# rlangefe/pygemma

Hardware: AMD Instinct MI355X
Metric: SNPs/sec (whole node) at n=10,000 c=5; K-eigendecomp wallclock (higher is better)
Workload: dtype i8x3->i32 MFMA (genotype codes exact, integer accumulation exact; U as 24-bit fixed point per eigenvector in three int8 planes) rotation + f64 Gram/sweeps (f32 rounding points of the reference)

## Files before the change

### include/pygemma_hip.h

```cpp
#ifndef PYGEMMA_HIP_H
#define PYGEMMA_HIP_H
#include <stddef.h>
#include <stdint.h>
#ifdef __cplusplus
extern "C" {
#endif

#define PG_OK 0
#define PG_EINVAL (-22)
#define PG_ENOMEM (-12)
#define PG_EHIP (-5)
#define PG_ENOTSUP (-95)
#define PG_ENODEV (-19)

#define PG_MAX_COVARIATES 30

typedef struct pg_ctx pg_ctx;

const char *pg_last_error(void);
const char *pg_version(void);
int pg_device_count(void);
int pg_ctx_create(int device, pg_ctx **out);
int pg_ctx_create_on_stream(int device, void *hip_stream, pg_ctx **out);
void pg_ctx_destroy(pg_ctx *ctx);
int pg_ctx_sync(pg_ctx *ctx);
int pg_ctx_device(const pg_ctx *ctx);

int pg_malloc(pg_ctx *ctx, size_t bytes, void **dptr);
int pg_free(pg_ctx *ctx, void *dptr);
int pg_mem_info(pg_ctx *ctx, size_t *free_bytes, size_t *total_bytes);
int pg_memcpy_h2d(pg_ctx *ctx, void *dst, const void *src, size_t bytes);
int pg_memcpy_d2h(pg_ctx *ctx, void *dst, const void *src, size_t bytes);
int pg_memset(pg_ctx *ctx, void *dst, int value, size_t bytes);
int pg_memcpy2d_h2d(pg_ctx *ctx, void *dst, size_t dpitch, const void *src, size_t spitch, size_t width, size_t height);

int pg_host_alloc(pg_ctx *ctx, size_t bytes, void **hptr);
int pg_host_free(pg_ctx *ctx, void *hptr);
int pg_host_register(pg_ctx *ctx, void *hptr, size_t bytes);
int pg_host_unregister(pg_ctx *ctx, void *hptr);
int pg_memcpy_h2d_async(pg_ctx *ctx, void *dst, const void *src, size_t bytes);
int pg_memcpy_d2h_async(pg_ctx *ctx, void *dst, const void *src, size_t bytes);
int pg_memcpy_d2d_async(pg_ctx *ctx, void *dst, const void *src, size_t bytes);
int pg_memcpy2d_h2d_async(pg_ctx *ctx, void *dst, size_t dpitch, const void *src, size_t spitch, size_t width, size_t height);
int pg_stage_rows(void *dst, size_t dpitch, const void *src, size_t spitch, size_t width, size_t height, int nthreads);

int pg_event_create(pg_ctx *ctx, void **event);
int pg_event_destroy(pg_ctx *ctx, void *event);
int pg_event_record(pg_ctx *ctx, void *event);
int pg_event_elapsed_ms(pg_ctx *ctx, void *start, void *stop, float *ms);
int pg_event_sync(pg_ctx *ctx, void *event);
int pg_stream_wait_event(pg_ctx *ctx, void *event);

typedef struct pg_comm pg_comm;
#define PG_COMM_ID_BYTES 128
int pg_comm_unique_id(void *id128);
int pg_comm_init_rank(pg_ctx *ctx, int nranks, int rank, const void *id128, pg_comm **out);
int pg_comm_init_all(int ndev, pg_ctx *const *ctxs, pg_comm **out );
int pg_comm_destroy(pg_comm *comm);
int pg_comm_size(const pg_comm *comm);
int pg_comm_rank(const pg_comm *comm);
int pg_comm_broadcast_dev(pg_comm *comm, void *buf, size_t bytes, int root);
int pg_comm_allgather_dev(pg_comm *comm, const void *send, void *recv, size_t bytes_per_rank);
int pg_comm_allreduce_f64_dev(pg_comm *comm, double *buf, size_t count, int op_max);
int pg_comm_barrier(pg_comm *comm);
int pg_comm_group_start(void);
int pg_comm_group_end(void);

int pg_assoc_dev(pg_ctx *ctx, int64_t n, int c, int64_t p, const float *d, const float *Wr, const float *yr,
                 const float *Xr, int64_t ldx, int grid, float *beta, float *se, float *tau, float *lambda,
                 double *F, double *pval, unsigned long long *stats_dev);

int pg_assoc_set_eval_trace(pg_ctx *ctx, unsigned *trace_dev);
int pg_assoc_warm(pg_ctx *ctx, int64_t n, int c);

int pg_assoc_pheno_dev(pg_ctx *ctx, int64_t n, int c, int64_t p, int t, const float *d, const float *Wr,
                       const float *Yr, int64_t ldy, const float *Xr, int64_t ldx, int grid,
                       float *beta, float *se, float *tau, float *lambda, double *F, double *pval,
                       unsigned long long *stats_dev);
int pg_assoc_pheno_warm(pg_ctx *ctx, int64_t n, int c, int t, int64_t p);

int pg_assoc_lrt_dev(pg_ctx *ctx, int64_t n, int c, int64_t p, const float *d, const float *Wr, const float *yr,
                     const float *Xr, int64_t ldx, int grid, float *beta, float *se, float *tau, float *lambda,
                     double *F, double *pval, double *l_alt, double *l_null, double *D_lrt, double *p_lrt);

int pg_score_null_dev(pg_ctx *ctx, int64_t n, int c, const float *d, const float *Wr, const float *yr, float *lambda0_dev);
int pg_score_dev(pg_ctx *ctx, int64_t n, int c, int64_t p, const float *d, const float *Wr, const float *yr, float lambda0,
                 const float *Xr, int64_t ldx, float *beta, float *se, float *tau, float *lambda, double *F, double *pval);

int pg_assoc_gxe_dev(pg_ctx *ctx, int64_t n, int c, int64_t p, const float *d, const float *Wr, const float *yr,
                     const float *xr, int64_t ldx, const float *xer, int64_t ldxe, float *beta, float *se, float *tau,
                     float *lambda, double *F, double *pval, unsigned long long *stats_dev);
int pg_assoc_gxe_warm(pg_ctx *ctx, int64_t n, int c);
int pg_gxe_scale_u_dev(pg_ctx *ctx, int64_t n, const float *U, int64_t ldU, const float *e, float *Ue);

int pg_assoc(pg_ctx *ctx, int64_t n, int c, int64_t p, const float *d, const float *Wr, const float *yr,
             const float *X_n_by_p, int grid, float *beta, float *se, float *tau, float *lambda, double *F,
             double *pval, unsigned long long *stats2);

int pg_assoc_multi(int ngpu, int64_t n, int c, int64_t p, const float *d, const float *Wr, const float *yr,
                   const float *X_n_by_p, int grid, float *beta, float *se, float *tau, float *lambda, double *F, double *pval);

int pg_fdist_sf_dev(pg_ctx *ctx, int64_t count, const double *F, double dfd, double *pval);

int pg_transpose_dev(pg_ctx *ctx, int64_t n, int64_t p, const float *X_n_by_p, int64_t ldX, float *Xr, int64_t ldx);

int pg_rotate_dev(pg_ctx *ctx, int64_t n, int64_t p, const float *U, int64_t ldU, const float *X_n_by_p, int64_t ldX,
                  float *Xr, int64_t ldx);

size_t pg_geno_prep_bytes(int64_t n);
size_t pg_geno_work_bytes(int64_t n, int64_t p);
int pg_geno_prep_dev(pg_ctx *ctx, int64_t n, const float *U, int64_t ldU, void *Uprep);
int pg_rotate_geno_dev(pg_ctx *ctx, int64_t n, int64_t p, const void *Uprep, const float *X_n_by_p, int64_t ldX, float *Xr,
                       int64_t ldx, void *work, int *is_geno);
int pg_rotate_auto_dev(pg_ctx *ctx, int64_t n, int64_t p, const float *U, int64_t ldU, const void *Uprep, const float *X_n_by_p, int64_t ldX,
                       float *Xr, int64_t ldx, void *work, int *path_dev);
int pg_rotate_auto_i8_dev(pg_ctx *ctx, int64_t n, int64_t p, const void *Uprep, const void *X8_n_by_p, int is_unsigned, int64_t ldX,
                          float *Xr, int64_t ldx, void *work, int *path_dev);
int pg_rotate_geno_i8_dev(pg_ctx *ctx, int64_t n, int64_t p, const void *Uprep, const void *X8_n_by_p, int is_unsigned, int64_t ldX,
                          float *Xr, int64_t ldx, void *work, int *is_geno);
int pg_cast_i8_f32_dev(pg_ctx *ctx, int64_t n, int64_t p, const void *X8_n_by_p, int is_unsigned, int64_t ldX, float *Xf, int64_t ldXf);
int pg_rotate_geno_f64_dev(pg_ctx *ctx, int64_t n, int64_t p, const void *Uprep, const double *X_n_by_p, int64_t ldX, float *Xr,
                           int64_t ldx, void *work, int *is_geno);
int pg_cast_f64_f32_dev(pg_ctx *ctx, int64_t n, int64_t p, const double *X_n_by_p, int64_t ldX, float *Xf, int64_t ldXf);
int pg_rotate_bed_dev(pg_ctx *ctx, int64_t n, int64_t p, const void *Uprep, const unsigned char *bed, int64_t ldb, int count_a1,
                      float *Xr, int64_t ldx, void *work);

int pg_kinship_dev(pg_ctx *ctx, int64_t n, int64_t p_k, const float *Gt, int64_t ldg, float *K);
int pg_kinship_geno_dev(pg_ctx *ctx, int64_t n, int64_t p, const float *G, int64_t ldG, int standardize, float *K);

enum { PG_DTYPE_INT8 = 0, PG_DTYPE_UINT8 = 1, PG_DTYPE_FLOAT32 = 2, PG_DTYPE_FLOAT64 = 3 };
size_t pg_kinship_acc_bytes(int64_t n, int64_t pb);
int pg_kinship_bed_acc_dev(pg_ctx *ctx, int64_t n, int64_t pb, const unsigned char *bed, int64_t ldb, int count_a1, int standardize,
                           double *acc);
int pg_kinship_x_acc_dev(pg_ctx *ctx, int64_t n, int64_t pb, const void *X, int dtype, int64_t ldX, int snp_major, int standardize,
                         double *acc);
int pg_kinship_finish_dev(pg_ctx *ctx, int64_t n, int64_t p, const double *acc, float *K);

int pg_zkzt_dev(pg_ctx *ctx, int64_t n, int64_t q, const void *Z, int z_is_f64, int64_t ldz, const void *K, int k_is_f64, int64_t ldk,
                float *out, int64_t ldo);

int pg_syevd_dev(pg_ctx *ctx, int64_t n, const float *K, float *evals, float *U, double *evals64, double *U64);

int pg_precompute_mat_dev(pg_ctx *ctx, int64_t n, int ctot, float lam, const float *d, const float *Wx, const float *y,
                          int full, float *P3, float *Q3, float *R3, float *vecs, float *scal);
int pg_newton_dev(pg_ctx *ctx, int64_t n, int ctot, float lam, float lam_min, float lam_max, const float *d,
                  const float *Wx, const float *y, float *root);
int pg_reml_scalars_dev(pg_ctx *ctx, int64_t n, int ctot, const float *args8, float *out3);
int pg_ml_scalars_dev(pg_ctx *ctx, int64_t n, const float *args7, float *out3);

int pgx_dgemm_dev(pg_ctx *ctx, int transA, int64_t M, int64_t N, int64_t K, double alpha, const double *A, int64_t lda,
                  const double *B, int64_t ldb, double beta, double *C, int64_t ldc);
int pgx_dgemm_ex_dev(pg_ctx *ctx, int flags, int kxorB, int64_t M, int64_t N, int64_t K, double alpha, const double *A, int64_t lda,
                     const double *B, int64_t ldb, double beta, double *C, int64_t ldc);
int pgx_ring_stamps(long long *out64);
int pgx_sytrd_dev(pg_ctx *ctx, int64_t n, const float *K, double *d, double *e, double *tau, double *Vall);
int pgx_stedc_dev(pg_ctx *ctx, int64_t n, const double *d_host, const double *e_host, double *evals_host, double *Z_dev);
int pgx_sb2_stage1_dev(pg_ctx *ctx, int64_t n, const float *K, double *Aband, double *Z, int *flags);
int pgx_sb2_stage2_dev(pg_ctx *ctx, int64_t n, const double *Aband, double *d, double *e, double *Z, int *flags);
int pgx_sb2_set_debug(void *host_mapped);

#ifdef __cplusplus
}
#endif
#endif
```

### pygemma_amd/_lib.py

```python
import ctypes as C
import os

import numpy as np

_HERE = os.path.dirname(os.path.abspath(__file__))
LIB_PATH = os.environ.get("PYGEMMA_HIP_LIB") or os.path.join(_HERE, "lib", "libpygemma_hip.so")
_lib = None

SYMBOLS = [
    "pg_last_error", "pg_version", "pg_device_count", "pg_ctx_create", "pg_ctx_create_on_stream",
    "pg_ctx_destroy", "pg_ctx_sync", "pg_ctx_device", "pg_mem_info", "pg_malloc", "pg_free", "pg_memcpy_h2d", "pg_memcpy_d2h",
    "pg_memset", "pg_memcpy2d_h2d", "pg_event_create", "pg_event_destroy", "pg_event_record", "pg_event_elapsed_ms",
    "pg_kinship_dev", "pg_geno_prep_bytes", "pg_geno_work_bytes", "pg_geno_prep_dev", "pg_rotate_geno_dev", "pg_assoc_dev", "pg_assoc", "pg_fdist_sf_dev", "pg_transpose_dev", "pg_rotate_dev", "pg_syevd_dev",
    "pg_precompute_mat_dev", "pg_newton_dev", "pg_reml_scalars_dev", "pg_ml_scalars_dev", "pg_rotate_bed_dev", "pg_rotate_geno_i8_dev", "pg_cast_i8_f32_dev", "pg_assoc_multi", "pg_rotate_geno_f64_dev", "pg_cast_f64_f32_dev",
    "pg_host_alloc", "pg_host_free", "pg_host_register", "pg_host_unregister", "pg_memcpy_h2d_async", "pg_memcpy_d2h_async",
    "pg_memcpy_d2d_async", "pg_memcpy2d_h2d_async", "pg_stage_rows", "pg_event_sync", "pg_stream_wait_event",
    "pg_comm_unique_id", "pg_comm_init_rank", "pg_comm_init_all", "pg_comm_destroy", "pg_comm_size", "pg_comm_rank",
    "pg_comm_broadcast_dev", "pg_comm_allgather_dev", "pg_comm_allreduce_f64_dev", "pg_comm_barrier", "pg_comm_group_start",
    "pg_comm_group_end", "pgx_dgemm_dev", "pgx_sytrd_dev", "pgx_stedc_dev", "pgx_sb2_stage1_dev", "pgx_sb2_stage2_dev", "pgx_sb2_set_debug", "pg_kinship_geno_dev", "pg_assoc_lrt_dev", "pg_rotate_auto_dev", "pg_assoc_set_eval_trace", "pg_assoc_warm", "pg_rotate_auto_i8_dev",
    "pg_zkzt_dev", "pgx_dgemm_ex_dev", "pgx_ring_stamps", "pg_assoc_pheno_dev", "pg_assoc_pheno_warm", "pg_score_null_dev", "pg_score_dev",
    "pg_kinship_acc_bytes", "pg_kinship_bed_acc_dev", "pg_kinship_x_acc_dev", "pg_kinship_finish_dev",
    "pg_assoc_gxe_dev", "pg_assoc_gxe_warm", "pg_gxe_scale_u_dev",
]


class PgError(RuntimeError):
    pass


def load():
    global _lib
    if _lib is not None:
        return _lib
    if not os.path.exists(LIB_PATH):
        raise PgError(f"{LIB_PATH} not found: build the HIP extension (python -c 'import __graft_entry__ as g; g.build()'). "
                      "pygemma_amd has no CPU fallback.")
    L = C.CDLL(LIB_PATH)
    vp, i64, i32, sz = C.c_void_p, C.c_int64, C.c_int, C.c_size_t
    L.pg_last_error.restype = C.c_char_p
    L.pg_version.restype = C.c_char_p
    L.pg_device_count.restype = i32
    L.pg_ctx_create.argtypes = [i32, C.POINTER(vp)]
    L.pg_ctx_create_on_stream.argtypes = [i32, vp, C.POINTER(vp)]
    L.pg_ctx_destroy.argtypes = [vp]
    L.pg_ctx_destroy.restype = None
    L.pg_ctx_sync.argtypes = [vp]
    L.pg_ctx_device.argtypes = [vp]
    L.pg_mem_info.argtypes = [vp, C.POINTER(C.c_size_t), C.POINTER(C.c_size_t)]
    L.pg_malloc.argtypes = [vp, sz, C.POINTER(vp)]
    L.pg_free.argtypes = [vp, vp]
    L.pg_memcpy_h2d.argtypes = [vp, vp, vp, sz]
    L.pg_memcpy_d2h.argtypes = [vp, vp, vp, sz]
    L.pg_memset.argtypes = [vp, vp, i32, sz]
    L.pg_assoc_dev.argtypes = [vp, i64, i32, i64, vp, vp, vp, vp, i64, i32, vp, vp, vp, vp, vp, vp, vp]
    L.pg_assoc.argtypes = [vp, i64, i32, i64, vp, vp, vp, vp, i32, vp, vp, vp, vp, vp, vp, vp]
    L.pg_assoc_lrt_dev.argtypes = [vp, i64, i32, i64, vp, vp, vp, vp, i64, i32] + [vp] * 10
    L.pg_assoc_lrt_dev.restype = i32
    L.pg_fdist_sf_dev.argtypes = [vp, i64, vp, C.c_double, vp]
    L.pg_assoc_multi.argtypes = [i32, i64, i32, i64, vp, vp, vp, vp, i32, vp, vp, vp, vp, vp, vp]
    L.pg_assoc_multi.restype = i32
    L.pg_transpose_dev.argtypes = [vp, i64, i64, vp, i64, vp, i64]
    L.pg_rotate_dev.argtypes = [vp, i64, i64, vp, i64, vp, i64, vp, i64]
    L.pg_kinship_dev.argtypes = [vp, i64, i64, vp, i64, vp]
    L.pg_kinship_geno_dev.argtypes = [vp, i64, i64, vp, i64, i32, vp]
    L.pg_kinship_geno_dev.restype = i32
    L.pg_kinship_acc_bytes.argtypes = [i64, i64]
    L.pg_kinship_acc_bytes.restype = sz
    L.pg_kinship_bed_acc_dev.argtypes = [vp, i64, i64, vp, i64, i32, i32, vp]
    L.pg_kinship_bed_acc_dev.restype = i32
    L.pg_kinship_x_acc_dev.argtypes = [vp, i64, i64, vp, i32, i64, i32, i32, vp]
    L.pg_kinship_x_acc_dev.restype = i32
    L.pg_kinship_finish_dev.argtypes = [vp, i64, i64, vp, vp]
    L.pg_kinship_finish_dev.restype = i32
    L.pg_geno_prep_bytes.argtypes = [i64]
    L.pg_geno_prep_bytes.restype = sz
    L.pg_geno_work_bytes.argtypes = [i64, i64]
    L.pg_geno_work_bytes.restype = sz
    L.pg_geno_prep_dev.argtypes = [vp, i64, vp, i64, vp]
    L.pg_geno_prep_dev.restype = i32
    L.pg_rotate_geno_dev.argtypes = [vp, i64, i64, vp, vp, i64, vp, i64, vp, C.POINTER(i32)]
    L.pg_rotate_geno_dev.restype = i32
    L.pg_assoc_set_eval_trace.argtypes = [vp, vp]
    L.pg_assoc_set_eval_trace.restype = i32
    L.pg_assoc_warm.argtypes = [vp, i64, i32]
    L.pg_assoc_warm.restype = i32
    L.pg_assoc_pheno_dev.argtypes = [vp, i64, i32, i64, i32, vp, vp, vp, i64, vp, i64, i32, vp, vp, vp, vp, vp, vp, vp]
    L.pg_assoc_pheno_dev.restype = i32
    L.pg_assoc_pheno_warm.argtypes = [vp, i64, i32, i32, i64]
    L.pg_assoc_pheno_warm.restype = i32
    L.pg_score_null_dev.argtypes = [vp, i64, i32, vp, vp, vp, vp]
    L.pg_score_null_dev.restype = i32
    L.pg_score_dev.argtypes = [vp, i64, i32, i64, vp, vp, vp, C.c_float, vp, i64, vp, vp, vp, vp, vp, vp]
    L.pg_score_dev.restype = i32
    L.pg_assoc_gxe_dev.argtypes = [vp, i64, i32, i64, vp, vp, vp, vp, i64, vp, i64, vp, vp, vp, vp, vp, vp, vp]
    L.pg_assoc_gxe_dev.restype = i32
    L.pg_assoc_gxe_warm.argtypes = [vp, i64, i32]
    L.pg_assoc_gxe_warm.restype = i32
    L.pg_gxe_scale_u_dev.argtypes = [vp, i64, vp, i64, vp, vp]
    L.pg_gxe_scale_u_dev.restype = i32
    L.pg_rotate_auto_i8_dev.argtypes = [vp, i64, i64, vp, vp, i32, i64, vp, i64, vp, vp]
    L.pg_rotate_auto_i8_dev.restype = i32
    L.pg_rotate_auto_dev.argtypes = [vp, i64, i64, vp, i64, vp, vp, i64, vp, i64, vp, vp]
    L.pg_rotate_auto_dev.restype = i32
    L.pg_rotate_bed_dev.argtypes = [vp, i64, i64, vp, vp, i64, i32, vp, i64, vp]
    L.pg_rotate_bed_dev.restype = i32
    L.pg_rotate_geno_i8_dev.argtypes = [vp, i64, i64, vp, vp, i32, i64, vp, i64, vp, C.POINTER(i32)]
    L.pg_rotate_geno_i8_dev.restype = i32
    L.pg_cast_i8_f32_dev.argtypes = [vp, i64, i64, vp, i32, i64, vp, i64]
    L.pg_cast_i8_f32_dev.restype = i32
    L.pg_rotate_geno_f64_dev.argtypes = [vp, i64, i64, vp, vp, i64, vp, i64, vp, C.POINTER(i32)]
    L.pg_rotate_geno_f64_dev.restype = i32
    L.pg_cast_f64_f32_dev.argtypes = [vp, i64, i64, vp, i64, vp, i64]
    L.pg_cast_f64_f32_dev.restype = i32
    L.pg_memcpy2d_h2d.argtypes = [vp, vp, sz, vp, sz, sz, sz]
    L.pg_event_create.argtypes = [vp, C.POINTER(vp)]
    L.pg_event_destroy.argtypes = [vp, vp]
    L.pg_event_record.argtypes = [vp, vp]
    L.pg_event_elapsed_ms.argtypes = [vp, vp, vp, C.POINTER(C.c_float)]
    L.pg_syevd_dev.argtypes = [vp, i64, vp, vp, vp, vp, vp]
    f32 = C.c_float
    L.pg_precompute_mat_dev.argtypes = [vp, i64, i32, f32, vp, vp, vp, i32, vp, vp, vp, vp, vp]
    L.pg_newton_dev.argtypes = [vp, i64, i32, f32, f32, f32, vp, vp, vp, vp]
    L.pg_reml_scalars_dev.argtypes = [vp, i64, i32, vp, vp]
    L.pg_ml_scalars_dev.argtypes = [vp, i64, vp, vp]
    L.pg_ml_scalars_dev.restype = i32
    L.pg_host_alloc.argtypes = [vp, sz, C.POINTER(vp)]
    L.pg_host_free.argtypes = [vp, vp]
    L.pg_host_register.argtypes = [vp, vp, sz]
    L.pg_host_unregister.argtypes = [vp, vp]
    L.pg_memcpy_h2d_async.argtypes = [vp, vp, vp, sz]
    L.pg_memcpy_d2h_async.argtypes = [vp, vp, vp, sz]
    L.pg_memcpy_d2d_async.argtypes = [vp, vp, vp, sz]
    L.pg_memcpy2d_h2d_async.argtypes = [vp, vp, sz, vp, sz, sz, sz]
    L.pg_stage_rows.argtypes = [vp, sz, vp, sz, sz, sz, i32]
    L.pg_event_sync.argtypes = [vp, vp]
    L.pg_stream_wait_event.argtypes = [vp, vp]
    L.pg_comm_unique_id.argtypes = [vp]
    L.pg_comm_init_rank.argtypes = [vp, i32, i32, vp, C.POINTER(vp)]
    L.pg_comm_init_all.argtypes = [i32, C.POINTER(vp), C.POINTER(vp)]
    L.pg_comm_destroy.argtypes = [vp]
    L.pg_comm_size.argtypes = [vp]
    L.pg_comm_rank.argtypes = [vp]
    L.pg_comm_broadcast_dev.argtypes = [vp, vp, sz, i32]
    L.pg_comm_allgather_dev.argtypes = [vp, vp, vp, sz]
    L.pg_comm_allreduce_f64_dev.argtypes = [vp, vp, sz, i32]
    L.pg_comm_barrier.argtypes = [vp]
    L.pgx_dgemm_dev.argtypes = [vp, i32, i64, i64, i64, C.c_double, vp, i64, vp, i64, C.c_double, vp, i64]
    L.pgx_dgemm_ex_dev.argtypes = [vp, i32, i32, i64, i64, i64, C.c_double, vp, i64, vp, i64, C.c_double, vp, i64]
    L.pgx_dgemm_ex_dev.restype = i32
    L.pg_zkzt_dev.argtypes = [vp, i64, i64, vp, i32, i64, vp, i32, i64, vp, i64]
    L.pg_zkzt_dev.restype = i32
    L.pgx_sytrd_dev.argtypes = [vp, i64, vp, vp, vp, vp, vp]
    L.pgx_stedc_dev.argtypes = [vp, i64, vp, vp, vp, vp]
    L.pgx_sb2_stage1_dev.argtypes = [vp, i64, vp, vp, vp, vp]
    L.pgx_sb2_stage2_dev.argtypes = [vp, i64, vp, vp, vp, vp, vp]
    L.pgx_sb2_set_debug.argtypes = [vp]
    for name in ("pg_host_alloc", "pg_host_free", "pg_host_register", "pg_host_unregister", "pg_memcpy_h2d_async", "pg_memcpy_d2h_async",
                 "pg_memcpy_d2d_async", "pg_memcpy2d_h2d_async", "pg_stage_rows", "pg_event_sync", "pg_stream_wait_event", "pg_comm_unique_id",
                 "pg_comm_init_rank", "pg_comm_init_all", "pg_comm_destroy", "pg_comm_size", "pg_comm_rank", "pg_comm_broadcast_dev",
                 "pg_comm_allgather_dev", "pg_comm_allreduce_f64_dev", "pg_comm_barrier", "pg_comm_group_start", "pg_comm_group_end",
                 "pgx_dgemm_dev", "pgx_sytrd_dev", "pgx_stedc_dev", "pgx_sb2_stage1_dev", "pgx_sb2_stage2_dev", "pgx_sb2_set_debug"):
        getattr(L, name).restype = i32
    for name in ("pg_ctx_create", "pg_ctx_create_on_stream", "pg_ctx_sync", "pg_ctx_device", "pg_malloc", "pg_free",
                 "pg_memcpy_h2d", "pg_memcpy_d2h", "pg_memset", "pg_assoc_dev", "pg_assoc", "pg_fdist_sf_dev",
                 "pg_transpose_dev", "pg_rotate_dev", "pg_syevd_dev", "pg_memcpy2d_h2d", "pg_event_create", "pg_event_destroy",
                 "pg_event_record", "pg_event_elapsed_ms", "pg_kinship_dev", "pg_precompute_mat_dev", "pg_newton_dev",
                 "pg_reml_scalars_dev"):
        getattr(L, name).restype = i32
    _lib = L
    return L


def check(rc, what=""):
    if rc != 0:
        raise PgError(f"{what} failed (code {rc}): {load().pg_last_error().decode()}")


class DeviceBuffer:

    def __init__(self, ctx, nbytes):
        self.ctx, self.nbytes = ctx, int(nbytes)
        p = C.c_void_p()
        check(load().pg_malloc(ctx.handle, self.nbytes, C.byref(p)), "pg_malloc")
        self.ptr = p.value

    def free(self):
        if self.ptr:
            load().pg_free(self.ctx.handle, self.ptr)
            self.ptr = None

    def upload(self, arr):
        arr = np.ascontiguousarray(arr)
        assert arr.nbytes <= self.nbytes
        check(load().pg_memcpy_h2d(self.ctx.handle, self.ptr, arr.ctypes.data, arr.nbytes), "pg_memcpy_h2d")
        return self

    def download(self, shape, dtype, offset=0):
        out = np.empty(shape, dtype)
        check(load().pg_memcpy_d2h(self.ctx.handle, out.ctypes.data, self.ptr + offset, out.nbytes), "pg_memcpy_d2h")
        return out


class Context:

    def __init__(self, device=0, stream=None):
        L = load()
        h = C.c_void_p()
        if stream is None:
            check(L.pg_ctx_create(int(device), C.byref(h)), "pg_ctx_create")
        else:
            check(L.pg_ctx_create_on_stream(int(device), C.c_void_p(stream), C.byref(h)), "pg_ctx_create_on_stream")
        self.handle = h
        self.device = device
        self._bufs = []

    def alloc(self, nbytes):
        b = DeviceBuffer(self, nbytes)
        self._bufs.append(b)
        return b

    def to_device(self, arr):
        arr = np.ascontiguousarray(arr)
        return self.alloc(max(arr.nbytes, 4)).upload(arr)

    def sync(self):
        check(load().pg_ctx_sync(self.handle), "pg_ctx_sync")

    def mem_info(self):
        f, t = C.c_size_t(), C.c_size_t()
        check(load().pg_mem_info(self.handle, C.byref(f), C.byref(t)), "pg_mem_info")
        return int(f.value), int(t.value)

    def close(self):
        if self.handle:
            for b in self._bufs:
                b.free()
            self._bufs = []
            load().pg_ctx_destroy(self.handle)
            self.handle = None

    def __enter__(self):
        return self

    def __exit__(self, *a):
        self.close()

    def __del__(self):
        try:
            self.close()
        except Exception:
            pass


def device_count():
    return load().pg_device_count()


_pinned = {}


class _PinnedBlock:

    def __init__(self, nbytes, device=0):
        import weakref
        self.ctx = Context(device)
        p = C.c_void_p()
        check(load().pg_host_alloc(self.ctx.handle, max(int(nbytes), 1), C.byref(p)), "pg_host_alloc")
        self.ptr, self.nbytes = p.value, int(nbytes)
        _pinned[self.ptr] = self.nbytes
        self._fin = weakref.finalize(self, _PinnedBlock._release, self.ctx, self.ptr)

    @staticmethod
    def _release(ctx, ptr):
        _pinned.pop(ptr, None)
        try:
            load().pg_host_free(ctx.handle, ptr)
            ctx.close()
        except Exception:
            pass


def pinned_empty(shape, dtype=np.float32, device=0):
    dtype = np.dtype(dtype)
    nbytes = int(np.prod(shape, dtype=np.int64)) * dtype.itemsize
    blk = _PinnedBlock(nbytes, device)
    buf = (C.c_char * max(nbytes, 1)).from_address(blk.ptr)
    arr = np.frombuffer(buf, dtype=dtype, count=nbytes // dtype.itemsize).reshape(shape)
    arr.flags.writeable = True
    buf._pg_block = blk
    return arr


def pin(arr, device=0):
    assert arr.flags.c_contiguous or arr.flags.f_contiguous
    ctx = Context(device)
    check(load().pg_host_register(ctx.handle, arr.ctypes.data, arr.nbytes), "pg_host_register")
    _pinned[arr.ctypes.data] = arr.nbytes

    class _Pin:
        def close(self_inner):
            if _pinned.pop(arr.ctypes.data, None) is not None:
                load().pg_host_unregister(ctx.handle, arr.ctypes.data)
                ctx.close()
    return _Pin()


def is_pinned(arr):
    try:
        from numpy.lib.array_utils import byte_bounds
    except ImportError:
        byte_bounds = np.byte_bounds
    lo, hi = byte_bounds(arr)
    for base, nb in list(_pinned.items()):
        if base <= lo and hi <= base + nb:
            return True
    return False
```

### pygemma_amd/csrc/assoc.hip

```cpp
#include "common.hpp"

#include <cmath>

namespace pg {

constexpr int NLAM = 11;
#ifndef PG_ASSOC_WPB
#define PG_ASSOC_WPB 2
#endif
constexpr int WPB = PG_ASSOC_WPB;
#define PG_MINV 1e-35f
#ifndef PG_FUSE_PQ_MAX
#define PG_FUSE_PQ_MAX 36
#endif
#ifndef PG_FUSE_PQR_MAX
#define PG_FUSE_PQR_MAX 28
#endif
#ifndef PG_PFD
#define PG_PFD 2
#endif
#ifndef PG_CHUNK_MIN_NP
#define PG_CHUNK_MIN_NP 80
#endif
#ifndef PG_SCAN_NV
#define PG_SCAN_NV 96
#endif
#ifndef PG_SWEEP_LDS_MIN_SLOTS
#define PG_SWEEP_LDS_MIN_SLOTS 3
#endif
#ifndef PG_PHENO_SPLIT_XE
#define PG_PHENO_SPLIT_XE 26
#endif
#ifndef PG_WAVES
#define PG_WAVES 2
#endif

__host__ __device__ constexpr size_t assoc_per_wave_bytes(int M, bool sweep_lds, size_t evalout_bytes, int n_vals)
{
    return (((sweep_lds ? (size_t)3 * M * 8 : 0) + (size_t)NLAM * 2 * M * 8 + NLAM * evalout_bytes + 2 * NLAM * 4 + (size_t)n_vals * 4) + 15) & ~(size_t)15;
}

struct AssocParams {
    int n, npad, c, niter, nu, grid, rowf;
    long long p, ldx;
    const float *xr;
    const float *fixed;
    float *htab;
    double *fixg;
    double *t1tab;
    float *ldHtab;
    float lam11[NLAM];
    float logl_c;
    const int *leaf, *node, *level, *chunk;
    int n_leaf, n_level, n_chunk, n_vals;
    float *beta, *se, *tau, *lam;
    double *F;
    unsigned long long *stats;
    unsigned *trace;
    int lrt, nhalf;
    float ml_c;
    float *lalt, *lamalt;
    const double *xbuf;
    int xe, xcol;
};

struct EvalOut { float yPy, yPPy, yPPPy, trP, trPP, ld, Pxx_c, Pyx_c, sh, shh; };

__device__ __forceinline__ float hinv_f32(float lam, float d)
{
    const float x = __fadd_rn(__fmul_rn(lam, d), 1.0f);
    const float r0 = __builtin_amdgcn_rcpf(x);
    float r = __builtin_fmaf(__builtin_fmaf(-x, r0, 1.0f), r0, r0);
    if (__builtin_expect(!(x < 0x1p126f), 0)) r = __fdiv_rn(1.0f, x);
    return r;
}

__device__ __forceinline__ float np_logf(float x)
{
    const float p1 = 9.999999999999998702752e-01f, p2 = 2.112677543073053063722e+00f,
                p3 = 1.480000633576506585156e+00f, p4 = 3.808837741388407920751e-01f,
                p5 = 2.589979117907922693523e-02f;
    const float q1 = 2.612677543073109236779e+00f, q2 = 2.453006071784736363091e+00f,
                q3 = 9.864942958519418960339e-01f, q4 = 1.546476374983906719538e-01f,
                q5 = 5.875095403124574342950e-03f;
    if (__builtin_expect(!(x > 0.0f) || x == INFINITY, 0)) return (x != x) ? x : (x < 0.0f ? NAN : (x == 0.0f ? -INFINITY : x));
    unsigned u = __float_as_uint(x);
    int e = (int)((u >> 23) & 0xff) - 126;
    float m = __uint_as_float((u & 0x007fffffu) | 0x3f000000u);
    float ef = (float)e;
    if (m <= 0.70710678118f) { m = __fadd_rn(m, m); ef = __fsub_rn(ef, 1.0f); }
    float t = __fsub_rn(m, 1.0f);
    float den = fmaf(q5, t, q4);
    den = fmaf(den, t, q3); den = fmaf(den, t, q2); den = fmaf(den, t, q1); den = fmaf(den, t, 1.0f);
    float num = fmaf(p5, t, p4);
    num = fmaf(num, t, p3); num = fmaf(num, t, p2); num = fmaf(num, t, p1); num = fmaf(num, t, 0.0f);
    float poly = __fdiv_rn(num, den);
    return fmaf(ef, 0.693147180559945309417232121458176568f, poly);
}

__device__ __forceinline__ double bfly(double v)
{
#pragma unroll
    for (int s = 1; s < 64; s <<= 1) v += __shfl_xor(v, s, 64);
    return v;
}

__device__ float device_logdet_H(const AssocParams &pr, float lam, int lane, float *vals)
{
    const int sub = lane & 7, grp = lane >> 3;
    auto elem = [&](int i) -> float {
        float d = pr.fixed[(size_t)i * pr.rowf];
        return np_logf(__fadd_rn(__fmul_rn(lam, d), 1.0f));
    };
    for (int l0 = 0; l0 < pr.n_leaf; l0 += 8) {
        const int lf = l0 + grp;
        int start = 0, len = 0;
        if (lf < pr.n_leaf) { start = pr.leaf[2 * lf]; len = pr.leaf[2 * lf + 1]; }
        float res = 0.0f;
        if (len >= 8) {
            const int body = len - (len & 7);
            float r = elem(start + sub);
            for (int i = 8; i < body; i += 8) r = __fadd_rn(r, elem(start + i + sub));
            r = __fadd_rn(r, __shfl_xor(r, 1, 64));
            r = __fadd_rn(r, __shfl_xor(r, 2, 64));
            r = __fadd_rn(r, __shfl_xor(r, 4, 64));
            res = r;
            for (int i = body; i < len; i++) res = __fadd_rn(res, elem(start + i));
        } else {
            for (int i = 0; i < len; i++) res = __fadd_rn(res, elem(start + i));
        }
        if (lf < pr.n_leaf && sub == 0) vals[lf] = res;
    }
    __builtin_amdgcn_fence(__ATOMIC_RELEASE, "wavefront");
    __builtin_amdgcn_wave_barrier();
    __builtin_amdgcn_fence(__ATOMIC_ACQUIRE, "wavefront");
    for (int h = 0; h < pr.n_level; h++) {
        const int b = pr.level[h], e = pr.level[h + 1];
        for (int k = b + lane; k < e; k += 64) {
            float a = vals[pr.node[2 * k]], c = vals[pr.node[2 * k + 1]];
            vals[pr.n_leaf + k] = __fadd_rn(a, c);
        }
        __builtin_amdgcn_fence(__ATOMIC_RELEASE, "wavefront");
        __builtin_amdgcn_wave_barrier();
        __builtin_amdgcn_fence(__ATOMIC_ACQUIRE, "wavefront");
    }
    float tot = vals[pr.chunk[0]];
    for (int k = 1; k < pr.n_chunk; k++) tot = __fadd_rn(tot, vals[pr.chunk[k]]);
    return tot;
}

__device__ __forceinline__ float logl_f(const AssocParams &pr, float yPy, float ldH, float ld)
{
    float r = pr.logl_c;
    r = (float)((double)r + (0.5 * (double)0.0f));
    r = (float)((double)r - (0.5 * (double)ldH));
    r = (float)((double)r - (0.5 * (double)ld));
    r = (float)((double)r - ((0.5 * (double)pr.nu) * log((double)yPy)));
    return r;
}
__device__ __forceinline__ float d1_f(const AssocParams &pr, float lam, float yPy, float yPPy, float trP)
{
    float yT = (PG_MINV > yPy) ? PG_MINV : yPy;
    float nc_tr = __fsub_rn((float)pr.nu, trP);
    float r = (float)(-0.5 * (double)__fdiv_rn(nc_tr, lam));
    float t = (0.0f > yPPy) ? 0.0f : yPPy;
    float g = __fdiv_rn(__fsub_rn(yT, t), lam);
    r = (float)((double)r + ((0.5 * (double)pr.nu) * (double)g) / (double)yT);
    return r;
}
__device__ __forceinline__ float d2_f(const AssocParams &pr, float lam, float yPy, float yPPy, float yPPPy,
                                      float trP, float trPP)
{
    float a = (PG_MINV > yPy) ? PG_MINV : yPy;
    float b = (PG_MINV > yPPy) ? PG_MINV : yPPy;
    float e = (PG_MINV > yPPPy) ? PG_MINV : yPPPy;
    double lam2 = (double)lam * (double)lam;
    float ae = __fadd_rn(a, e);
    float G2 = (float)(((double)ae - 2.0 * (double)b) / lam2);
    float G1 = __fdiv_rn(__fsub_rn(a, b), lam);
    float nct = __fadd_rn((float)pr.nu, trPP);
    float r = (float)((0.5 * ((double)nct - 2.0 * (double)trP)) / lam2);
    float G2a = __fmul_rn(G2, a);
    r = (float)((double)r - ((double)pr.nu * ((double)G2a - (0.5 * (double)G1) * (double)G1)) / ((double)a * (double)a));
    return r;
}

__device__ __forceinline__ float ml_logl_f(const AssocParams &pr, float yPy, float ldH)
{
    float r = pr.ml_c;
    r = __fsub_rn(r, __fmul_rn(0.5f, ldH));
    const float t = (PG_MINV > yPy) ? PG_MINV : yPy;
    r = (float)((double)r - (double)pr.nhalf * log((double)t));
    return r;
}
__device__ __forceinline__ float ml_d1_f(const AssocParams &pr, float lam, float yPy, float yPPy, float sh)
{
    float r = __fmul_rn(-0.5f, __fdiv_rn(__fsub_rn((float)pr.n, sh), lam));
    const float num = (PG_MINV > yPPy) ? PG_MINV : yPPy, den = (PG_MINV > yPy) ? PG_MINV : yPy;
    r = (float)((double)r + ((double)pr.nhalf * (1.0 - (double)__fdiv_rn(num, den))) / (double)lam);
    return r;
}
__device__ __forceinline__ float ml_d2_f(const AssocParams &pr, float lam, float yPy, float yPPy, float yPPPy, float sh, float shh)
{
    const float a = (PG_MINV > yPy) ? PG_MINV : yPy, b = (PG_MINV > yPPy) ? PG_MINV : yPPy, e = (PG_MINV > yPPPy) ? PG_MINV : yPPPy;
    const float G2 = (float)(((double)__fadd_rn(a, e) - 2.0 * (double)b) / (double)__fmul_rn(lam, lam));
    const float G1 = __fdiv_rn(__fsub_rn(a, b), lam);
    const float t = __fmul_rn(0.5f, __fsub_rn(__fadd_rn((float)pr.n, shh), __fmul_rn(2.0f, sh)));
    float r = (float)((double)t / ((double)lam * (double)lam));
    r = (float)((double)r - ((0.5 * (double)pr.n) * ((2.0 * (double)G2) - (double)__fdiv_rn(__fmul_rn(G1, G1), a))) / (double)a);
    return r;
}

template <int C> struct Shape {
    static constexpr int M = C + 2;
    static constexpr int NP = M * (M + 1) / 2;
    static constexpr int SLOTS = (NP + 63) / 64;
    static constexpr int NV0 = NP < 64 ? NP : 64, NV1 = NP > 64 ? NP - 64 : 0;
    static constexpr int slot_nv(int sl) { return (NP - 64 * sl) < 64 ? (NP - 64 * sl) : 64; }
    static constexpr bool CHUNKED = NP > PG_CHUNK_MIN_NP;
    static constexpr bool SWEEP_LDS = SLOTS >= PG_SWEEP_LDS_MIN_SLOTS;
    static constexpr int SCAN_NV = (M <= 4 && PG_SCAN_NV > 64) ? 64 : PG_SCAN_NV;
    static constexpr int G = (SCAN_NV / (2 * M)) < 1 ? 1 : ((SCAN_NV / (2 * M)) > 11 ? 11 : (SCAN_NV / (2 * M)));
    static constexpr bool FUSE_PQ = NP <= PG_FUSE_PQ_MAX, FUSE_PQR = NP <= PG_FUSE_PQR_MAX;
};
__host__ __device__ constexpr int tri(int r, int c) { return r * (r + 1) / 2 + c; }
__host__ __device__ constexpr int next_pow2(int v) { int p = 1; while (p < v) p <<= 1; return p; }

__device__ __forceinline__ double dmaxf(double a, float b) { return ((double)b > a) ? (double)b : a; }

template <int NVP>
__device__ __forceinline__ double reduce_scatter(double (&v)[NVP], int lane)
{
    static_assert(NVP >= 1 && NVP <= 64 && (NVP & (NVP - 1)) == 0, "power of two");
#pragma unroll
    for (int s = 1; s < NVP; s <<= 1) {
        const bool b = (lane & s) != 0;
#pragma unroll
        for (int m = 0; m < NVP / (2 * s); m++) {
            const double keep = b ? v[2 * m + 1] : v[2 * m];
            const double send = b ? v[2 * m] : v[2 * m + 1];
            v[m] = keep + __shfl_xor(send, s, 64);
        }
    }
    double x = v[0];
#pragma unroll
    for (int s = NVP; s < 64; s <<= 1) x += __shfl_xor(x, s, 64);
    return x;
}

template <int C, int SL = 0>
__device__ __forceinline__ void scatter_entries(const double (&acc)[Shape<C>::NP], int lane, double (&out)[Shape<C>::SLOTS])
{
    constexpr int NV = Shape<C>::slot_nv(SL), NVP = next_pow2(NV);
    double t[NVP];
#pragma unroll
    for (int k = 0; k < NVP; k++) t[k] = (k < NV) ? acc[64 * SL + k] : 0.0;
    out[SL] = reduce_scatter<NVP>(t, lane);
    if constexpr (SL + 1 < Shape<C>::SLOTS) scatter_entries<C, SL + 1>(acc, lane, out);
}

template <int C> struct Own {
    int e[Shape<C>::SLOTS], r[Shape<C>::SLOTS], c[Shape<C>::SLOTS];
    bool valid[Shape<C>::SLOTS];
    __device__ __forceinline__ void init(int lane)
    {
#pragma unroll
        for (int sl = 0; sl < Shape<C>::SLOTS; sl++) {
            const int nv = Shape<C>::slot_nv(sl), k = lane % next_pow2(nv);
            valid[sl] = k < nv;
            e[sl] = valid[sl] ? 64 * sl + k : 0;
            int rr = 0;
            while ((rr + 1) * (rr + 2) / 2 <= e[sl]) rr++;
            r[sl] = rr; c[sl] = e[sl] - rr * (rr + 1) / 2;
        }
    }
};

template <int SLOTS>
__device__ __forceinline__ double gather(const double (&X)[SLOTS], int es)
{
    double v = __shfl(X[0], es & 63, 64);
#pragma unroll
    for (int sl = 1; sl < SLOTS; sl++) { const double w = __shfl(X[sl], es & 63, 64); v = ((es >> 6) == sl) ? w : v; }
    return v;
}

__device__ __forceinline__ void wave_lds_sync();

template <int C, bool FULL>
__device__ __forceinline__ void lane_sweeps(double (&P)[Shape<C>::SLOTS], double (&Q)[Shape<C>::SLOTS], double (&R)[Shape<C>::SLOTS],
                                            const Own<C> &own, double t1, double t2, int lane, EvalOut &o, double *piv)
{
    constexpr int M = Shape<C>::M, NP = Shape<C>::NP, SLOTS = Shape<C>::SLOTS;
    constexpr bool VIA_LDS = Shape<C>::SWEEP_LDS;
    if (own.valid[0] && own.e[0] == 0) P[0] = dmaxf(P[0], PG_MINV);
    double trP = t1, trPP = t2, apiv = 1.0;
    for (int i = 1; i < M; i++) {
        const int q = i - 1, eqq = tri(q, q);
        double a, b, e = 0.0;
        double ur[SLOTS], uc[SLOTS], vr[SLOTS], vc[SLOTS], wr[SLOTS], wc[SLOTS];
        bool act[SLOTS];
        if constexpr (VIA_LDS) {
#pragma unroll
            for (int sl = 0; sl < SLOTS; sl++)
                if (own.valid[sl] && own.c[sl] == q) {
                    piv[own.r[sl]] = P[sl]; piv[M + own.r[sl]] = Q[sl];
                    if (FULL) piv[2 * M + own.r[sl]] = R[sl];
                }
            wave_lds_sync();
            a = piv[q]; b = piv[M + q];
            if (FULL) e = piv[2 * M + q];
#pragma unroll
            for (int sl = 0; sl < SLOTS; sl++) {
                act[sl] = own.valid[sl] && own.c[sl] >= i;
                const int rr = act[sl] ? own.r[sl] : q, cc = act[sl] ? own.c[sl] : q;
                ur[sl] = piv[rr]; uc[sl] = piv[cc];
                vr[sl] = piv[M + rr]; vc[sl] = piv[M + cc];
                if (FULL) { wr[sl] = piv[2 * M + rr]; wc[sl] = piv[2 * M + cc]; }
            }
            wave_lds_sync();
        } else {
            a = gather<SLOTS>(P, eqq); b = gather<SLOTS>(Q, eqq);
            e = FULL ? gather<SLOTS>(R, eqq) : 0.0;
#pragma unroll
            for (int sl = 0; sl < SLOTS; sl++) {
                act[sl] = own.valid[sl] && own.c[sl] >= i;
                const int er = act[sl] ? tri(own.r[sl], q) : 0, ec = act[sl] ? tri(own.c[sl], q) : 0;
                ur[sl] = gather<SLOTS>(P, er); uc[sl] = gather<SLOTS>(P, ec);
                vr[sl] = gather<SLOTS>(Q, er); vc[sl] = gather<SLOTS>(Q, ec);
                if (FULL) { wr[sl] = gather<SLOTS>(R, er); wc[sl] = gather<SLOTS>(R, ec); }
            }
        }
        if (lane == q) apiv = a;
        const double a2 = a * a, ia = -1.0 / a, ba2 = b / a2;
        if (FULL) {
            const double ba = b / a;
            trPP = (trPP + ba * ba) - 2 * (e / a);
            const double a3 = a2 * a, b2 = b * b;
            const double cR = (e / a2) - (b2 / a3);
#pragma unroll
            for (int sl = 0; sl < SLOTS; sl++)
                if (act[sl]) {
                    double s1 = fma(cR * uc[sl], ur[sl], R[sl]);
                    double s2 = fma(ia * uc[sl], wr[sl], 0.0); s2 = fma(ia * wc[sl], ur[sl], s2);
                    double s3 = fma(ia * vc[sl], vr[sl], 0.0);
                    double s4 = fma(ba2 * uc[sl], vr[sl], 0.0); s4 = fma(ba2 * vc[sl], ur[sl], s4);
                    double rn = ((s1 + s2) + s3) + s4;
                    if (own.r[sl] == i && own.c[sl] == i) rn = dmaxf(rn, PG_MINV);
                    R[sl] = rn;
                }
        }
        trP = trP - b / a;
#pragma unroll
        for (int sl = 0; sl < SLOTS; sl++)
            if (act[sl]) {
                double s1 = fma(ba2 * uc[sl], ur[sl], Q[sl]);
                double s2 = fma(ia * uc[sl], vr[sl], 0.0); s2 = fma(ia * vc[sl], ur[sl], s2);
                double qn = s1 + s2;
                double pn = fma(ia * uc[sl], ur[sl], P[sl]);
                if (own.r[sl] == i && own.c[sl] == i) { qn = dmaxf(qn, PG_MINV); pn = dmaxf(pn, PG_MINV); }
                Q[sl] = qn; P[sl] = pn;
            }
        if (i == M - 2) { o.Pxx_c = (float)gather<SLOTS>(P, tri(M - 2, M - 2)); o.Pyx_c = (float)gather<SLOTS>(P, tri(M - 1, M - 2)); }
    }
    const double lg = log(apiv);
    float ld = 0.0f;
    for (int q = 0; q < M - 1; q++) ld = (float)((double)ld + __shfl(lg, q, 64));
    o.yPy = (float)gather<SLOTS>(P, NP - 1);
    o.yPPy = (float)gather<SLOTS>(Q, NP - 1);
    o.yPPPy = FULL ? (float)gather<SLOTS>(R, NP - 1) : 0.0f;
    o.trP = (float)trP;
    o.trPP = FULL ? (float)trPP : 0.0f;
    o.ld = ld;
    o.sh = (float)t1;
    o.shh = FULL ? (float)t2 : 0.0f;
}

template <int C> struct Elem {
    static constexpr int S4 = (C + 2 + 3) / 4;
    float4 row[S4];
    float x;
};
template <int C, bool HASX = true>
__device__ __forceinline__ void load_elem(const AssocParams &pr, const float *xrow, int i, Elem<C> &e)
{
    const float4 *src = reinterpret_cast<const float4 *>(pr.fixed + (size_t)i * pr.rowf);
#pragma unroll
    for (int k = 0; k < Elem<C>::S4; k++) e.row[k] = src[k];
    const int ic = min(i, pr.n - 1);
    e.x = HASX ? xrow[ic] : 0.0f;
}
constexpr int PFD = PG_PFD;
template <class E, int PF = PFD, class LoadF, class BodyF>
__device__ __forceinline__ void pipelined(int niter, LoadF &&ld, BodyF &&body)
{
    E buf[PF];
#pragma unroll
    for (int d = 0; d < PF; d++) ld(buf[d], d < niter ? d : niter - 1);
    for (int it = 0; it < niter; it += PF) {
#pragma unroll
        for (int d = 0; d < PF; d++) {
            if (it + d < niter) body(buf[d], it + d);
            const int nx = it + d + PF;
            ld(buf[d], nx < niter ? nx : niter - 1);
        }
    }
}
template <int C>
__device__ __forceinline__ void unpack_elem(const AssocParams &pr, const Elem<C> &e, int i, float &d, float (&col)[C + 2])
{
    float buf[4 * Elem<C>::S4];
#pragma unroll
    for (int k = 0; k < Elem<C>::S4; k++) {
        buf[4 * k] = e.row[k].x; buf[4 * k + 1] = e.row[k].y; buf[4 * k + 2] = e.row[k].z; buf[4 * k + 3] = e.row[k].w;
    }
    d = buf[0];
#pragma unroll
    for (int j = 0; j < C; j++) col[j] = buf[1 + j];
    col[C] = e.x;
    col[C + 1] = buf[C + 1];
}
template <int C> struct WaldElem {
    using E = Elem<C>;
    using Row = const float *;
    template <bool HASX>
    static __device__ __forceinline__ void load(const AssocParams &pr, Row xrow, int i, E &e) { load_elem<C, HASX>(pr, xrow, i, e); }
    static __device__ __forceinline__ void unpack(const AssocParams &pr, const E &e, int i, float &d, float (&col)[C + 2]) { unpack_elem<C>(pr, e, i, d, col); }
};

template <int C, int MASK, bool HASX, class EL = WaldElem<C>>
__device__ __forceinline__ void gram_pass(const AssocParams &pr, typename EL::Row xrow, float lam, int lane, float *htab_out,
                                          double (&Po)[Shape<C>::SLOTS], double (&Qo)[Shape<C>::SLOTS], double (&Ro)[Shape<C>::SLOTS],
                                          double &t1, double &t2)
{
    constexpr int M = Shape<C>::M, NP = Shape<C>::NP;
    constexpr bool DP = (MASK & 1) != 0, DQ = (MASK & 2) != 0, DR = (MASK & 4) != 0;
    double P[DP ? NP : 1], Q[DQ ? NP : 1], R[DR ? NP : 1];
#pragma unroll
    for (int k = 0; k < NP; k++) { if constexpr (DP) P[k] = 0.0; if constexpr (DQ) Q[k] = 0.0; if constexpr (DR) R[k] = 0.0; }
    double s1 = 0.0, s2 = 0.0;
    using E = typename EL::E;
    pipelined<E>(pr.niter, [&](E &e, int it) { EL::template load<HASX>(pr, xrow, it * 64 + lane, e); },
                       [&](const E &cur, int it) {
        const int i = it * 64 + lane;
        float d, colf[M];
        EL::unpack(pr, cur, i, d, colf);
        const float h = hinv_f32(lam, d);
        if (htab_out) htab_out[i] = h;
        const double hd = (double)h;
        double col[M], a[M];
#pragma unroll
        for (int j = 0; j < M; j++) { col[j] = (double)colf[j]; a[j] = hd * col[j]; }
        if (DP || DQ) {
#pragma unroll
            for (int j = 0; j < M; j++)
#pragma unroll
                for (int k = 0; k <= j; k++) {
                    if constexpr (DP) P[tri(j, k)] = fma(a[j], col[k], P[tri(j, k)]);
                    if constexpr (DQ) Q[tri(j, k)] = fma(a[j], a[k], Q[tri(j, k)]);
                }
        }
        if (DP) s1 += hd;
        if constexpr (DR) {
            const double h2 = hd * hd;
#pragma unroll
            for (int j = 0; j < M; j++) {
                const double gj = h2 * col[j];
#pragma unroll
                for (int k = 0; k <= j; k++) R[tri(j, k)] = fma(gj, a[k], R[tri(j, k)]);
            }
            s2 = fma(hd, hd, s2);
        }
    });
    if constexpr (DP) { scatter_entries<C>(P, lane, Po); t1 = bfly(s1); }
    if constexpr (DQ) scatter_entries<C>(Q, lane, Qo);
    if constexpr (DR) { scatter_entries<C>(R, lane, Ro); t2 = bfly(s2); }
}

template <int C, int PW, int SL, bool HASX, class EL = WaldElem<C>>
__device__ __forceinline__ void gram_pass_slot(const AssocParams &pr, typename EL::Row xrow, float lam, int lane, float *htab_out, double &out, double &tsum)
{
    constexpr int M = Shape<C>::M, E0 = 64 * SL, NV = Shape<C>::slot_nv(SL), NVP = next_pow2(NV);
    double acc[NVP];
#pragma unroll
    for (int k = 0; k < NVP; k++) acc[k] = 0.0;
    double s = 0.0;
    using E = typename EL::E;
    pipelined<E, (M > 22 ? 1 : PFD)>(pr.niter, [&](E &e, int it) { EL::template load<HASX>(pr, xrow, it * 64 + lane, e); },
                       [&](const E &cur, int it) {
        const int i = it * 64 + lane;
        float d, colf[M];
        EL::unpack(pr, cur, i, d, colf);
        const float h = hinv_f32(lam, d);
        if (htab_out) htab_out[i] = h;
        const double hd = (double)h, h2 = hd * hd;
        double col[M], a[M], g[PW == 3 ? M : 1];
#pragma unroll
        for (int j = 0; j < M; j++) { col[j] = (double)colf[j]; a[j] = hd * col[j]; if constexpr (PW == 3) g[j] = h2 * col[j]; }
#pragma unroll
        for (int j = 0; j < M; j++)
#pragma unroll
            for (int k = 0; k <= j; k++) {
                const int e = tri(j, k);
                if (e >= E0 && e < E0 + NV) {
                    if constexpr (PW == 1) acc[e - E0] = fma(a[j], col[k], acc[e - E0]);
                    else if constexpr (PW == 2) acc[e - E0] = fma(a[j], a[k], acc[e - E0]);
                    else acc[e - E0] = fma(g[j], a[k], acc[e - E0]);
                }
            }
        if constexpr (SL == 0 && PW == 1) s += hd;
        if constexpr (SL == 0 && PW == 3) s = fma(hd, hd, s);
    });
    out = reduce_scatter<NVP>(acc, lane);
    if constexpr (SL == 0 && (PW == 1 || PW == 3)) tsum = bfly(s);
}
template <int C, int PW, bool HASX, int SL = 0, class EL = WaldElem<C>>
__device__ __forceinline__ void slot_passes(const AssocParams &pr, typename EL::Row xrow, float lam, int lane, float *htab_out,
                                            double (&X)[Shape<C>::SLOTS], double &tsum)
{
    gram_pass_slot<C, PW, SL, HASX, EL>(pr, xrow, lam, lane, SL == 0 ? htab_out : nullptr, X[SL], tsum);
    if constexpr (SL + 1 < Shape<C>::SLOTS) slot_passes<C, PW, HASX, SL + 1, EL>(pr, xrow, lam, lane, htab_out, X, tsum);
}

template <int C, bool FULL, class EL = WaldElem<C>>
__device__ __forceinline__ void eval_specific(const AssocParams &pr, typename EL::Row xrow, float lam, int lane, const Own<C> &own, EvalOut &o,
                                              double *piv)
{
    constexpr int SLOTS = Shape<C>::SLOTS;
    double P[SLOTS], Q[SLOTS], R[SLOTS], t1 = 0.0, t2 = 0.0;
#pragma unroll
    for (int sl = 0; sl < SLOTS; sl++) R[sl] = 0.0;
    if constexpr (Shape<C>::CHUNKED) {
        double tq = 0.0;
        slot_passes<C, 1, true, 0, EL>(pr, xrow, lam, lane, nullptr, P, t1);
        slot_passes<C, 2, true, 0, EL>(pr, xrow, lam, lane, nullptr, Q, tq);
        if (FULL) slot_passes<C, 3, true, 0, EL>(pr, xrow, lam, lane, nullptr, R, t2);
    } else if constexpr (FULL && Shape<C>::FUSE_PQR) {
        gram_pass<C, 7, true, EL>(pr, xrow, lam, lane, nullptr, P, Q, R, t1, t2);
    } else if constexpr (Shape<C>::FUSE_PQ) {
        gram_pass<C, 3, true, EL>(pr, xrow, lam, lane, nullptr, P, Q, R, t1, t2);
        if (FULL) gram_pass<C, 4, true, EL>(pr, xrow, lam, lane, nullptr, P, Q, R, t1, t2);
    } else {
        gram_pass<C, 1, true, EL>(pr, xrow, lam, lane, nullptr, P, Q, R, t1, t2);
        gram_pass<C, 2, true, EL>(pr, xrow, lam, lane, nullptr, P, Q, R, t1, t2);
        if (FULL) gram_pass<C, 4, true, EL>(pr, xrow, lam, lane, nullptr, P, Q, R, t1, t2);
    }
    lane_sweeps<C, FULL>(P, Q, R, own, t1, t2, lane, o, piv);
}

template <int C>
__global__ __launch_bounds__(64) void setup_tabs_kernel(AssocParams pr)
{
    constexpr int NP = Shape<C>::NP, SLOTS = Shape<C>::SLOTS;
    extern __shared__ float smem_f[];
    const int t = blockIdx.x, lane = threadIdx.x;
    const float lam = pr.lam11[t];
    Own<C> own;
    own.init(lane);
    double P[SLOTS], Q[SLOTS], R[SLOTS], t1 = 0.0, t2 = 0.0;
    if constexpr (Shape<C>::CHUNKED) {
        double tq = 0.0;
        slot_passes<C, 1, false>(pr, nullptr, lam, lane, pr.htab + (size_t)t * pr.npad, P, t1);
        slot_passes<C, 2, false>(pr, nullptr, lam, lane, nullptr, Q, tq);
    } else if constexpr (Shape<C>::FUSE_PQ) {
        gram_pass<C, 3, false>(pr, nullptr, lam, lane, pr.htab + (size_t)t * pr.npad, P, Q, R, t1, t2);
    } else {
        gram_pass<C, 1, false>(pr, nullptr, lam, lane, pr.htab + (size_t)t * pr.npad, P, Q, R, t1, t2);
        gram_pass<C, 2, false>(pr, nullptr, lam, lane, nullptr, P, Q, R, t1, t2);
    }
#pragma unroll
    for (int sl = 0; sl < SLOTS; sl++)
        if (own.valid[sl]) {
            pr.fixg[((size_t)t * 2 + 0) * NP + own.e[sl]] = P[sl];
            pr.fixg[((size_t)t * 2 + 1) * NP + own.e[sl]] = Q[sl];
        }
    float ldH = device_logdet_H(pr, lam, lane, smem_f);
    if (lane == 0) { pr.t1tab[t] = t1; pr.ldHtab[t] = ldH; }
}

template <int C, int GG>
__device__ __forceinline__ void scan_accumulate(const AssocParams &pr, const float *xrow, int t0, int lane, double *xent)
{
    constexpr int M = Shape<C>::M, NV = GG * 2 * M;
    constexpr int NV0 = NV < 64 ? NV : 64, NV1 = NV > 64 ? NV - 64 : 0;
    constexpr int NVP0 = next_pow2(NV0), NVP1 = next_pow2(NV1 > 0 ? NV1 : 1);
    static_assert(NV <= 128, "scan group too large");
    double acc[NV0 == 64 ? 64 + NVP1 : NVP0];
#pragma unroll
    for (int k = 0; k < (NV0 == 64 ? 64 + NVP1 : NVP0); k++) acc[k] = 0.0;
    struct SE { Elem<C> e; float h[GG]; };
    pipelined<SE>(pr.niter, [&](SE &q, int it) {
        const int i = it * 64 + lane;
        load_elem<C>(pr, xrow, i, q.e);
#pragma unroll
        for (int g = 0; g < GG; g++) q.h[g] = pr.htab[(size_t)(t0 + g) * pr.npad + i];
    }, [&](const SE &q, int it) {
        const int i = it * 64 + lane;
        float d, colf[M];
        unpack_elem<C>(pr, q.e, i, d, colf);
        const double xd = (double)colf[C];
        double z[M];
#pragma unroll
        for (int k = 0; k <= C; k++) z[k] = xd * (double)colf[k];
        z[C + 1] = (double)colf[C + 1] * xd;
#pragma unroll
        for (int g = 0; g < GG; g++) {
            const double hd = (double)q.h[g];
            const double h2 = hd * hd;
#pragma unroll
            for (int k = 0; k <= C + 1; k++) {
                acc[g * 2 * M + k] = fma(hd, z[k], acc[g * 2 * M + k]);
                acc[g * 2 * M + M + k] = fma(h2, z[k], acc[g * 2 * M + M + k]);
            }
        }
    });
    {
        double t[NVP0];
#pragma unroll
        for (int k = 0; k < NVP0; k++) t[k] = acc[k];
        const double tot = reduce_scatter<NVP0>(t, lane);
        const int idx = lane % NVP0;
        if (idx < NV0 && lane < NVP0) xent[t0 * 2 * M + idx] = tot;
    }
    if constexpr (NV1 > 0) {
        double t[NVP1];
#pragma unroll
        for (int k = 0; k < NVP1; k++) t[k] = acc[64 + k];
        const double tot = reduce_scatter<NVP1>(t, lane);
        const int idx = lane % NVP1;
        if (idx < NV1 && lane < NVP1) xent[t0 * 2 * M + 64 + idx] = tot;
    }
}
template <int C, int T0>
__device__ __forceinline__ void scan_all(const AssocParams &pr, const float *xrow, int lane, double *xent)
{
    constexpr int G = Shape<C>::G;
    if constexpr (T0 < NLAM) {
        constexpr int GG = (NLAM - T0) < G ? (NLAM - T0) : G;
        scan_accumulate<C, GG>(pr, xrow, T0, lane, xent);
        scan_all<C, T0 + GG>(pr, xrow, lane, xent);
    }
}

template <int C, int TC, int GG, int PWS, int PW0>
__device__ __forceinline__ void scan_pheno_accumulate(const AssocParams &pr, const float *xrow, const float *Y, long long ldy, int tcn,
                                                      int t0, int lane, double *out)
{
    constexpr int M = Shape<C>::M, XE = C + 1 + TC, NV = GG * PWS * XE;
    auto dest = [&](int v) { const int gg = v / (PWS * XE), r = v - gg * PWS * XE; return (t0 + gg) * 2 * XE + PW0 * XE + r; };
    constexpr int NV0 = NV < 64 ? NV : 64, NV1 = NV > 64 ? NV - 64 : 0;
    constexpr int NVP0 = next_pow2(NV0), NVP1 = next_pow2(NV1 > 0 ? NV1 : 1);
    static_assert(NV <= 128, "scan group too large");
    double acc[NV0 == 64 ? 64 + NVP1 : NVP0];
#pragma unroll
    for (int k = 0; k < (NV0 == 64 ? 64 + NVP1 : NVP0); k++) acc[k] = 0.0;
    struct SE { Elem<C> e; float y[TC]; float h[GG]; };
    pipelined<SE>(pr.niter, [&](SE &q, int it) {
        const int i = it * 64 + lane;
        load_elem<C>(pr, xrow, i, q.e);
#pragma unroll
        for (int j = 0; j < TC; j++) q.y[j] = (i < pr.n && j < tcn) ? Y[(size_t)j * ldy + i] : 0.0f;
#pragma unroll
        for (int g = 0; g < GG; g++) q.h[g] = pr.htab[(size_t)(t0 + g) * pr.npad + i];
    }, [&](const SE &q, int it) {
        const int i = it * 64 + lane;
        float d, colf[M];
        unpack_elem<C>(pr, q.e, i, d, colf);
        const double xd = (double)colf[C];
        double z[XE];
#pragma unroll
        for (int k = 0; k <= C; k++) z[k] = xd * (double)colf[k];
#pragma unroll
        for (int j = 0; j < TC; j++) z[C + 1 + j] = (double)q.y[j] * xd;
#pragma unroll
        for (int g = 0; g < GG; g++) {
            const double hd = (double)q.h[g];
            const double h2 = hd * hd;
#pragma unroll
            for (int k = 0; k < XE; k++) {
                if constexpr (PWS == 2) {
                    acc[g * 2 * XE + k] = fma(hd, z[k], acc[g * 2 * XE + k]);
                    acc[g * 2 * XE + XE + k] = fma(h2, z[k], acc[g * 2 * XE + XE + k]);
                } else {
                    acc[g * XE + k] = fma(PW0 == 0 ? hd : h2, z[k], acc[g * XE + k]);
                }
            }
        }
    });
    {
        double t[NVP0];
#pragma unroll
        for (int k = 0; k < NVP0; k++) t[k] = acc[k];
        const double tot = reduce_scatter<NVP0>(t, lane);
        const int idx = lane % NVP0;
        if (idx < NV0 && lane < NVP0) out[dest(idx)] = tot;
    }
    if constexpr (NV1 > 0) {
        double t[NVP1];
#pragma unroll
        for (int k = 0; k < NVP1; k++) t[k] = acc[64 + k];
        const double tot = reduce_scatter<NVP1>(t, lane);
        const int idx = lane % NVP1;
        if (idx < NV1 && lane < NVP1) out[dest(64 + idx)] = tot;
    }
}
template <int C, int TC, int T0>
__device__ __forceinline__ void scan_pheno_all(const AssocParams &pr, const float *xrow, const float *Y, long long ldy, int tcn, int lane,
                                               double *out)
{
    constexpr int XE = C + 1 + TC, PWS = XE > PG_PHENO_SPLIT_XE ? 1 : 2;
    constexpr int G0 = PWS == 1 ? 1 : (Shape<C>::SCAN_NV - XE) / (PWS * XE), G = G0 < 1 ? 1 : (G0 > NLAM ? NLAM : G0);
    if constexpr (T0 < NLAM) {
        constexpr int GG = (NLAM - T0) < G ? (NLAM - T0) : G;
        if constexpr (PWS == 2) {
            scan_pheno_accumulate<C, TC, GG, 2, 0>(pr, xrow, Y, ldy, tcn, T0, lane, out);
        } else {
            scan_pheno_accumulate<C, TC, GG, 1, 0>(pr, xrow, Y, ldy, tcn, T0, lane, out);
            scan_pheno_accumulate<C, TC, GG, 1, 1>(pr, xrow, Y, ldy, tcn, T0, lane, out);
        }
        scan_pheno_all<C, TC, T0 + GG>(pr, xrow, Y, ldy, tcn, lane, out);
    }
}
constexpr int SCAN_WPB = 4;
template <int C, int TC>
__global__ __launch_bounds__(64 * SCAN_WPB, PG_WAVES) void scan_pheno_kernel(AssocParams pr, const float *Y, long long ldy, int tcn, double *xbuf)
{
    const int wave = threadIdx.x >> 6, lane = threadIdx.x & 63;
    const long long g = (long long)blockIdx.x * SCAN_WPB + wave;
    if (g >= pr.p) return;
    scan_pheno_all<C, TC, 0>(pr, pr.xr + (size_t)g * pr.ldx, Y, ldy, tcn, lane, xbuf + (size_t)g * NLAM * 2 * (C + 1 + TC));
}

__device__ __forceinline__ void wave_lds_sync()
{
    __builtin_amdgcn_fence(__ATOMIC_RELEASE, "wavefront");
    __builtin_amdgcn_wave_barrier();
    __builtin_amdgcn_fence(__ATOMIC_ACQUIRE, "wavefront");
}

template <class Fn>
__device__ __forceinline__ double brentq_dev(Fn &&f, double xa, double xb, double fa, double fb, int maxiter = 100)
{
    const double xtol = 2e-12, rtol = 0.1;
    double xpre = xa, xcur = xb, xblk = 0., fpre = fa, fcur = fb, fblk = 0., spre = 0., scur = 0., sbis, delta, stry, dpre, dblk;
    if (fpre == 0) return xpre;
    if (fcur == 0) return xcur;
    for (int i = 0; i < maxiter; i++) {
        if (fpre != 0 && fcur != 0 && (__builtin_signbit(fpre) != __builtin_signbit(fcur))) {
            xblk = xpre; fblk = fpre; spre = scur = xcur - xpre;
        }
        if (fabs(fblk) < fabs(fcur)) {
            xpre = xcur; xcur = xblk; xblk = xpre;
            fpre = fcur; fcur = fblk; fblk = fpre;
        }
        delta = (xtol + rtol * fabs(xcur)) / 2;
        sbis = (xblk - xcur) / 2;
        if (fcur == 0 || fabs(sbis) < delta) return xcur;
        if (fabs(spre) > delta && fabs(fcur) < fabs(fpre)) {
            if (xpre == xblk) {
                stry = -fcur * (xcur - xpre) / (fcur - fpre);
            } else {
                dpre = (fpre - fcur) / (xpre - xcur);
                dblk = (fblk - fcur) / (xblk - xcur);
                stry = -fcur * (fblk * dblk - fpre * dpre) / (dblk * dpre * (fblk - fpre));
            }
            double lim = 3 * fabs(sbis) - delta;
            double mn = fabs(spre) < lim ? fabs(spre) : lim;
            if (2 * fabs(stry) < mn) { spre = scur; scur = stry; }
            else { spre = sbis; scur = sbis; }
        } else { spre = sbis; scur = sbis; }
        xpre = xcur; fpre = fcur;
        if (fabs(scur) > delta) xcur += scur;
        else xcur += (sbis > 0 ? delta : -delta);
        fcur = f(xcur);
    }
    return xcur;
}

template <class Eval>
__device__ __forceinline__ float newton_dev(const AssocParams &pr, float lroot, float l0, float l1, Eval &&eval)
{
    int iteration = 0;
    for (;;) {
        EvalOut e;
        eval(lroot, e);
        const float d1 = d1_f(pr, lroot, e.yPy, e.yPPy, e.trP);
        const float d2 = d2_f(pr, lroot, e.yPy, e.yPPy, e.yPPPy, e.trP, e.trPP);
        const float ratio = __fdiv_rn(d1, d2);
        const bool any_nan = (ratio != ratio) || (d1 != d1) || (d2 != d2);
        const float sr = (float)((ratio > 0) - (ratio < 0)), s1 = (float)((d1 > 0) - (d1 < 0)), s2 = (float)((d2 > 0) - (d2 < 0));
        if (!any_nan && sr * s1 * s2 <= 0.0f) break;
        const float lnew = __fsub_rn(lroot, ratio);
        const float r_eps = (float)(fabs((double)__fsub_rn(lnew, lroot)) / fabs((double)lroot));
        if (lnew < l0) break;
        if (lnew > l1) break;
        if (isnan(lnew) || isinf(lnew)) break;
        lroot = lnew;
        if ((double)r_eps < 1e-5 || iteration > 100) break;
        iteration++;
    }
    return lroot;
}

template <int C, bool LRT, bool PHENO = false>
__global__ __launch_bounds__(64 * WPB, PG_WAVES) void assoc_kernel(AssocParams pr)
{
    constexpr int M = Shape<C>::M, NP = Shape<C>::NP, SLOTS = Shape<C>::SLOTS;
    extern __shared__ unsigned char smem[];
    const int wave = threadIdx.x >> 6, lane = threadIdx.x & 63;
    static_assert(!(PHENO && LRT), "the multi-phenotype search has no LRT");
    const long long g = (long long)blockIdx.x * WPB + wave;
    if (g >= pr.p) return;
    constexpr size_t piv_bytes = Shape<C>::SWEEP_LDS ? (size_t)3 * M * 8 : 0;
    unsigned char *base = smem + (size_t)wave * assoc_per_wave_bytes(M, Shape<C>::SWEEP_LDS, sizeof(EvalOut), pr.n_vals);
    double *piv = reinterpret_cast<double *>(base);
    base += piv_bytes;
    double *xent = reinterpret_cast<double *>(base);
    EvalOut *evs = reinterpret_cast<EvalOut *>(base + (size_t)NLAM * 2 * M * 8);
    float *d1s = reinterpret_cast<float *>(evs + NLAM);
    float *lls = d1s + NLAM;
    float *vals = lls + NLAM;
    const float *xrow = pr.xr + (size_t)g * pr.ldx;

    Own<C> own;
    own.init(lane);
    if constexpr (PHENO) {
        const double *src = pr.xbuf + (size_t)g * NLAM * 2 * pr.xe;
        for (int j = lane; j < NLAM * 2 * M; j += 64) {
            const int tp = j / M, k = j - tp * M;
            xent[j] = src[(size_t)tp * pr.xe + (k <= C ? k : pr.xcol)];
        }
    } else {
        scan_all<C, 0>(pr, xrow, lane, xent);
    }
    wave_lds_sync();
    for (int t = 0; t < NLAM; t++) {
        double P[SLOTS], Q[SLOTS], R[SLOTS];
        const double *fp = pr.fixg + ((size_t)t * 2 + 0) * NP, *fq = pr.fixg + ((size_t)t * 2 + 1) * NP;
        const double *xe = xent + t * 2 * M;
#pragma unroll
        for (int sl = 0; sl < SLOTS; sl++) {
            const int r = own.r[sl], c = own.c[sl];
            const bool isx = (r == C) || (r == C + 1 && c == C);
            const int k = (r == C) ? c : C + 1;
            P[sl] = isx ? xe[k] : fp[own.e[sl]];
            Q[sl] = isx ? xe[M + k] : fq[own.e[sl]];
            R[sl] = 0.0;
        }
        EvalOut e;
        lane_sweeps<C, false>(P, Q, R, own, pr.t1tab[t], 0.0, lane, e, piv);
        if (lane == 0) {
            evs[t] = e;
            d1s[t] = d1_f(pr, pr.lam11[t], e.yPy, e.yPPy, e.trP);
            lls[t] = logl_f(pr, e.yPy, pr.ldHtab[t], e.ld);
        }
    }
    wave_lds_sync();
    float best_l = lls[0], best_lambda;
    EvalOut best_e;
    if (best_l < lls[NLAM - 1]) { best_l = lls[NLAM - 1]; best_lambda = pr.lam11[NLAM - 1]; best_e = evs[NLAM - 1]; }
    else { best_lambda = pr.lam11[0]; best_e = evs[0]; }
    unsigned n_fast = 0, n_full = 0;
    if (pr.grid) {
        for (int t = 0; t < NLAM - 1; t++)
            if (lls[t] > best_l) { best_l = lls[t]; best_lambda = pr.lam11[t]; best_e = evs[t]; }
    } else {
        for (int k = 0; k < NLAM - 1; k++) {
            const float f0 = d1s[k], f1 = d1s[k + 1];
            if (__builtin_signbit(f0) == __builtin_signbit(f1)) continue;
            const float l0 = pr.lam11[k], l1 = pr.lam11[k + 1];
            double root = brentq_dev(
                [&](double x) -> double {
                    EvalOut e;
                    const float lf = (float)x;
                    eval_specific<C, false>(pr, xrow, lf, lane, own, e, piv);
                    n_fast++;
                    return (double)d1_f(pr, lf, e.yPy, e.yPPy, e.trP);
                },
                (double)l0, (double)l1, (double)f0, (double)f1);
            const float lroot = newton_dev(pr, (float)root, l0, l1, [&](float lf, EvalOut &e) {
                eval_specific<C, true>(pr, xrow, lf, lane, own, e, piv);
                n_full++;
            });
            EvalOut e;
            eval_specific<C, false>(pr, xrow, lroot, lane, own, e, piv);
            n_fast++;
            const float ldH = device_logdet_H(pr, lroot, lane, vals);
            const float ll = logl_f(pr, e.yPy, ldH, e.ld);
            if (ll > best_l) { best_l = ll; best_lambda = lroot; best_e = e; }
        }
    }
    if constexpr (LRT) {
        float ml_l = ml_logl_f(pr, evs[0].yPy, pr.ldHtab[0]), ml_lam = pr.lam11[0];
        {
            const float l1 = ml_logl_f(pr, evs[NLAM - 1].yPy, pr.ldHtab[NLAM - 1]);
            if (ml_l == ml_l && (l1 != l1 || l1 > ml_l)) { ml_l = l1; ml_lam = pr.lam11[NLAM - 1]; }
        }
        for (int k = 0; k < NLAM - 1; k++) {
            const float f0 = ml_d1_f(pr, pr.lam11[k], evs[k].yPy, evs[k].yPPy, evs[k].sh);
            const float f1 = ml_d1_f(pr, pr.lam11[k + 1], evs[k + 1].yPy, evs[k + 1].yPPy, evs[k + 1].sh);
            if (f0 != f0 || f1 != f1) continue;
            const float s0 = (float)((f0 > 0) - (f0 < 0)), s1 = (float)((f1 > 0) - (f1 < 0));
            if (!(s0 * s1 < 0.0f)) continue;
            double p0 = brentq_dev(
                [&](double x) -> double {
                    EvalOut e;
                    const float lf = (float)x;
                    eval_specific<C, false>(pr, xrow, lf, lane, own, e, piv);
                    n_fast++;
                    return (double)ml_d1_f(pr, lf, e.yPy, e.yPPy, e.sh);
                },
                (double)pr.lam11[k], (double)pr.lam11[k + 1], (double)f0, (double)f1, 5000);
            double pn = p0;
            for (int itr = 0; itr < 10; itr++) {
                EvalOut e;
                const float lf = (float)p0;
                eval_specific<C, true>(pr, xrow, lf, lane, own, e, piv);
                n_full++;
                const float fval = ml_d1_f(pr, lf, e.yPy, e.yPPy, e.sh);
                if (fval == 0.0f) { pn = p0; break; }
                const float fder = ml_d2_f(pr, lf, e.yPy, e.yPPy, e.yPPPy, e.sh, e.shh);
                if (fder == 0.0f) { pn = p0; break; }
                pn = p0 - (double)__fdiv_rn(fval, fder);
                if (fabs(pn - p0) <= 1.48e-8 + 1e-5 * fabs(p0)) break;
                p0 = pn;
            }
            if (ml_l == ml_l) {
                EvalOut e;
                const float lf = (float)pn;
                eval_specific<C, false>(pr, xrow, lf, lane, own, e, piv);
                n_fast++;
                const float l = ml_logl_f(pr, e.yPy, device_logdet_H(pr, lf, lane, vals));
                if (l != l || l > ml_l) { ml_l = l; ml_lam = lf; }
            }
        }
        if (lane == 0) { pr.lalt[g] = ml_l; pr.lamalt[g] = ml_lam; }
    }
    if (lane == 0) {
        const float b = __fdiv_rn(best_e.Pyx_c, best_e.Pxx_c);
        const float pxx = (PG_MINV > best_e.Pxx_c) ? PG_MINV : best_e.Pxx_c;
        const float sb = (float)(__dsqrt_rn((double)best_e.yPy) / ((double)sqrtf(pxx) * __dsqrt_rn((double)(pr.nu))));
        const float ta = __fdiv_rn((float)pr.nu, best_e.yPy);
        const double t = (double)__fdiv_rn(b, sb);
        pr.beta[g] = b; pr.se[g] = sb; pr.tau[g] = ta; pr.lam[g] = best_lambda; pr.F[g] = t * t;
        if (pr.stats) { atomicAdd(&pr.stats[0], (unsigned long long)n_fast); atomicAdd(&pr.stats[1], (unsigned long long)n_full); }
        if (pr.trace) pr.trace[g] = n_fast | (n_full << 16);
    }
}

#if defined(PG_ASSOC_PART) && (PG_ASSOC_PART == 6 || PG_ASSOC_PART == 7)
struct GxeRows { const float *x, *xe; };
template <int CS> struct GxeVals {
    static constexpr int S4 = (CS + 2 + 3) / 4;
    float4 row[S4];
    float x, xe;
};
template <int C> struct GxeElem {
    static constexpr int CS = C - 1;
    using E = GxeVals<CS>;
    using Row = GxeRows;
    template <bool HASX>
    static __device__ __forceinline__ void load(const AssocParams &pr, Row r, int i, E &e)
    {
        const float4 *src = reinterpret_cast<const float4 *>(pr.fixed + (size_t)i * pr.rowf);
#pragma unroll
        for (int k = 0; k < E::S4; k++) e.row[k] = src[k];
        const int ic = min(i, pr.n - 1);
        e.x = r.x[ic];
        e.xe = r.xe[ic];
    }
    static __device__ __forceinline__ void unpack(const AssocParams &pr, const E &e, int i, float &d, float (&col)[C + 2])
    {
        float buf[4 * E::S4];
#pragma unroll
        for (int k = 0; k < E::S4; k++) {
            buf[4 * k] = e.row[k].x; buf[4 * k + 1] = e.row[k].y; buf[4 * k + 2] = e.row[k].z; buf[4 * k + 3] = e.row[k].w;
        }
        d = buf[0];
#pragma unroll
        for (int j = 0; j < CS; j++) col[j] = buf[1 + j];
        col[CS] = e.x;
        col[CS + 1] = e.xe;
        col[CS + 2] = buf[CS + 1];
    }
};
template <int CS> struct GxeShape {
    static constexpr int C = CS + 1, NE = 2 * CS + 5;
    static constexpr int PWS = NE > PG_PHENO_SPLIT_XE ? 1 : 2;
    static constexpr int G0 = (Shape<C>::SCAN_NV - NE) / (PWS * NE), G = G0 < 1 ? 1 : (G0 > NLAM ? NLAM : G0);
};
__host__ __device__ constexpr size_t gxe_per_wave_bytes(int M, bool sweep_lds, int NE, size_t evalout_bytes, int n_vals)
{
    return (((sweep_lds ? (size_t)3 * M * 8 : 0) + (size_t)NLAM * 2 * NE * 8 + NLAM * evalout_bytes + 2 * NLAM * 4 + (size_t)n_vals * 4) + 15) & ~(size_t)15;
}

template <int CS, int GG, int PWS, int PW0>
__device__ __forceinline__ void gxe_scan_accumulate(const AssocParams &pr, GxeRows xr, int t0, int lane, double *out)
{
    using EL = GxeElem<CS + 1>;
    constexpr int M = CS + 3, NE = GxeShape<CS>::NE, NV = GG * PWS * NE;
    auto dest = [&](int v) { const int gg = v / (PWS * NE), r = v - gg * PWS * NE; return (t0 + gg) * 2 * NE + PW0 * NE + r; };
    constexpr int NV0 = NV < 64 ? NV : 64, NV1 = NV > 64 ? NV - 64 : 0;
    constexpr int NVP0 = next_pow2(NV0), NVP1 = next_pow2(NV1 > 0 ? NV1 : 1);
    static_assert(NV <= 128, "scan group too large");
    double acc[NV0 == 64 ? 64 + NVP1 : NVP0];
#pragma unroll
    for (int k = 0; k < (NV0 == 64 ? 64 + NVP1 : NVP0); k++) acc[k] = 0.0;
    struct SE { typename EL::E e; float h[GG]; };
    pipelined<SE>(pr.niter, [&](SE &q, int it) {
        const int i = it * 64 + lane;
        EL::template load<true>(pr, xr, i, q.e);
#pragma unroll
        for (int g = 0; g < GG; g++) q.h[g] = pr.htab[(size_t)(t0 + g) * pr.npad + i];
    }, [&](const SE &q, int it) {
        const int i = it * 64 + lane;
        float d, colf[M];
        EL::unpack(pr, q.e, i, d, colf);
        const double xd = (double)colf[CS], ed = (double)colf[CS + 1], yd = (double)colf[CS + 2];
        double z[NE];
#pragma unroll
        for (int k = 0; k < CS; k++) { z[k] = xd * (double)colf[k]; z[CS + 1 + k] = ed * (double)colf[k]; }
        z[CS] = xd * xd;
        z[2 * CS + 1] = ed * xd;
        z[2 * CS + 2] = ed * ed;
        z[2 * CS + 3] = yd * xd;
        z[2 * CS + 4] = yd * ed;
#pragma unroll
        for (int g = 0; g < GG; g++) {
            const double hd = (double)q.h[g];
            const double h2 = hd * hd;
#pragma unroll
            for (int k = 0; k < NE; k++) {
                if constexpr (PWS == 2) {
                    acc[g * 2 * NE + k] = fma(hd, z[k], acc[g * 2 * NE + k]);
                    acc[g * 2 * NE + NE + k] = fma(h2, z[k], acc[g * 2 * NE + NE + k]);
                } else {
                    acc[g * NE + k] = fma(PW0 == 0 ? hd : h2, z[k], acc[g * NE + k]);
                }
            }
        }
    });
    {
        double t[NVP0];
#pragma unroll
        for (int k = 0; k < NVP0; k++) t[k] = acc[k];
        const double tot = reduce_scatter<NVP0>(t, lane);
        const int idx = lane % NVP0;
        if (idx < NV0 && lane < NVP0) out[dest(idx)] = tot;
    }
    if constexpr (NV1 > 0) {
        double t[NVP1];
#pragma unroll
        for (int k = 0; k < NVP1; k++) t[k] = acc[64 + k];
        const double tot = reduce_scatter<NVP1>(t, lane);
        const int idx = lane % NVP1;
        if (idx < NV1 && lane < NVP1) out[dest(64 + idx)] = tot;
    }
}
template <int CS, int T0>
__device__ __forceinline__ void gxe_scan_all(const AssocParams &pr, GxeRows xr, int lane, double *xent)
{
    constexpr int G = GxeShape<CS>::G;
    if constexpr (T0 < NLAM) {
        constexpr int GG = (NLAM - T0) < G ? (NLAM - T0) : G;
        if constexpr (GxeShape<CS>::PWS == 2) {
            gxe_scan_accumulate<CS, GG, 2, 0>(pr, xr, T0, lane, xent);
        } else {
            gxe_scan_accumulate<CS, GG, 1, 0>(pr, xr, T0, lane, xent);
            gxe_scan_accumulate<CS, GG, 1, 1>(pr, xr, T0, lane, xent);
        }
        gxe_scan_all<CS, T0 + GG>(pr, xr, lane, xent);
    }
}

template <int CS>
__global__ __launch_bounds__(64 * WPB, PG_WAVES) void assoc_gxe_kernel(AssocParams pr, const float *xer, long long ldxe)
{
    constexpr int C = CS + 1, M = Shape<C>::M, SLOTS = Shape<C>::SLOTS, NE = GxeShape<CS>::NE, NPS = Shape<CS>::NP;
    using EL = GxeElem<C>;
    extern __shared__ unsigned char smem[];
    const int wave = threadIdx.x >> 6, lane = threadIdx.x & 63;
    const long long g = (long long)blockIdx.x * WPB + wave;
    if (g >= pr.p) return;
    constexpr size_t piv_bytes = Shape<C>::SWEEP_LDS ? (size_t)3 * M * 8 : 0;
    unsigned char *base = smem + (size_t)wave * gxe_per_wave_bytes(M, Shape<C>::SWEEP_LDS, NE, sizeof(EvalOut), pr.n_vals);
    double *piv = reinterpret_cast<double *>(base);
    base += piv_bytes;
    double *xent = reinterpret_cast<double *>(base);
    EvalOut *evs = reinterpret_cast<EvalOut *>(base + (size_t)NLAM * 2 * NE * 8);
    float *d1s = reinterpret_cast<float *>(evs + NLAM);
    float *lls = d1s + NLAM;
    float *vals = lls + NLAM;
    const GxeRows xr{pr.xr + (size_t)g * pr.ldx, xer + (size_t)g * ldxe};

    Own<C> own;
    own.init(lane);
    gxe_scan_all<CS, 0>(pr, xr, lane, xent);
    wave_lds_sync();
    for (int t = 0; t < NLAM; t++) {
        double P[SLOTS], Q[SLOTS], R[SLOTS];
        const double *fp = pr.fixg + ((size_t)t * 2 + 0) * NPS, *fq = pr.fixg + ((size_t)t * 2 + 1) * NPS;
        const double *xe = xent + t * 2 * NE;
#pragma unroll
        for (int sl = 0; sl < SLOTS; sl++) {
            const int r = own.r[sl], c = own.c[sl];
            const int k = (r == CS) ? c : (r == CS + 1) ? CS + 1 + c : (r == CS + 2 && c == CS) ? 2 * CS + 3 : (r == CS + 2 && c == CS + 1) ? 2 * CS + 4 : -1;
            const int f = (r < CS) ? tri(r, c) : tri(CS + 1, c < CS ? c : CS + 1);
            const int kk = k >= 0 ? k : 0;
            P[sl] = k >= 0 ? xe[kk] : fp[f];
            Q[sl] = k >= 0 ? xe[NE + kk] : fq[f];
            R[sl] = 0.0;
        }
        EvalOut e;
        lane_sweeps<C, false>(P, Q, R, own, pr.t1tab[t], 0.0, lane, e, piv);
        if (lane == 0) {
            evs[t] = e;
            d1s[t] = d1_f(pr, pr.lam11[t], e.yPy, e.yPPy, e.trP);
            lls[t] = logl_f(pr, e.yPy, pr.ldHtab[t], e.ld);
        }
    }
    wave_lds_sync();
    float best_l = lls[0], best_lambda;
    EvalOut best_e;
    if (best_l < lls[NLAM - 1]) { best_l = lls[NLAM - 1]; best_lambda = pr.lam11[NLAM - 1]; best_e = evs[NLAM - 1]; }
    else { best_lambda = pr.lam11[0]; best_e = evs[0]; }
    unsigned n_fast = 0, n_full = 0;
    for (int k = 0; k < NLAM - 1; k++) {
        const float f0 = d1s[k], f1 = d1s[k + 1];
        if (__builtin_signbit(f0) == __builtin_signbit(f1)) continue;
        const float l0 = pr.lam11[k], l1 = pr.lam11[k + 1];
        double root = brentq_dev(
            [&](double x) -> double {
                EvalOut e;
                const float lf = (float)x;
                eval_specific<C, false, EL>(pr, xr, lf, lane, own, e, piv);
                n_fast++;
                return (double)d1_f(pr, lf, e.yPy, e.yPPy, e.trP);
            },
            (double)l0, (double)l1, (double)f0, (double)f1);
        const float lroot = newton_dev(pr, (float)root, l0, l1, [&](float lf, EvalOut &e) {
            eval_specific<C, true, EL>(pr, xr, lf, lane, own, e, piv);
            n_full++;
        });
        EvalOut e;
        eval_specific<C, false, EL>(pr, xr, lroot, lane, own, e, piv);
        n_fast++;
        const float ldH = device_logdet_H(pr, lroot, lane, vals);
        const float ll = logl_f(pr, e.yPy, ldH, e.ld);
        if (ll > best_l) { best_l = ll; best_lambda = lroot; best_e = e; }
    }
    if (lane == 0) {
        const float b = __fdiv_rn(best_e.Pyx_c, best_e.Pxx_c);
        const float pxx = (PG_MINV > best_e.Pxx_c) ? PG_MINV : best_e.Pxx_c;
        const float sb = (float)(__dsqrt_rn((double)best_e.yPy) / ((double)sqrtf(pxx) * __dsqrt_rn((double)(pr.nu))));
        const float ta = __fdiv_rn((float)pr.nu, best_e.yPy);
        const double t = (double)__fdiv_rn(b, sb);
        pr.beta[g] = b; pr.se[g] = sb; pr.tau[g] = ta; pr.lam[g] = best_lambda; pr.F[g] = t * t;
        if (pr.stats) { atomicAdd(&pr.stats[0], (unsigned long long)n_fast); atomicAdd(&pr.stats[1], (unsigned long long)n_full); }
    }
}

template <int CS>
static int launch_gxe(pg_ctx *ctx, AssocParams &pr, const float *xer, long long ldxe)
{
    constexpr int C = CS + 1;
    const size_t lds = (size_t)WPB * gxe_per_wave_bytes(Shape<C>::M, Shape<C>::SWEEP_LDS, GxeShape<CS>::NE, sizeof(EvalOut), pr.n_vals);
    PG_REQUIRE(pr.n_vals >= 0 && lds <= 160 * 1024, "assoc_gxe: c = %d, n_vals = %d need %zu bytes of LDS per workgroup", CS, pr.n_vals, lds);
    setup_tabs_kernel<CS><<<NLAM, 64, (size_t)pr.n_vals * 4 + 16, ctx->stream>>>(pr);
    PG_HIP(hipGetLastError());
    if (lds > 64 * 1024)
        PG_HIP(hipFuncSetAttribute(reinterpret_cast<const void *>(&assoc_gxe_kernel<CS>), hipFuncAttributeMaxDynamicSharedMemorySize, (int)lds));
    const long long nblk = (pr.p + WPB - 1) / WPB;
    assoc_gxe_kernel<CS><<<dim3((unsigned)nblk), 64 * WPB, lds, ctx->stream>>>(pr, xer, ldxe);
    PG_HIP(hipGetLastError());
    return PG_OK;
}
#endif

template <int C, bool LRT = false>
static int launch_assoc(pg_ctx *ctx, AssocParams &pr)
{
    const size_t lds = (size_t)WPB * assoc_per_wave_bytes(Shape<C>::M, Shape<C>::SWEEP_LDS, sizeof(EvalOut), pr.n_vals);
    static_assert(Shape<C>::M == C + 2, "Shape<C>::M");
    PG_REQUIRE(pr.n_vals >= 0 && lds <= 160 * 1024, "assoc: c = %d, n_vals = %d need %zu bytes of LDS per workgroup", C, pr.n_vals, lds);
    setup_tabs_kernel<C><<<NLAM, 64, (size_t)pr.n_vals * 4 + 16, ctx->stream>>>(pr);
    PG_HIP(hipGetLastError());
    if (lds > 64 * 1024)
        PG_HIP(hipFuncSetAttribute(reinterpret_cast<const void *>(&assoc_kernel<C, LRT>), hipFuncAttributeMaxDynamicSharedMemorySize, (int)lds));
    const long long nblk = (pr.p + WPB - 1) / WPB;
    assoc_kernel<C, LRT><<<dim3((unsigned)nblk), 64 * WPB, lds, ctx->stream>>>(pr);
    PG_HIP(hipGetLastError());
    return PG_OK;
}

struct PhenoLaunch {
    enum { SETUP, SCAN, SEARCH } phase;
    const float *Y; long long ldy;
    int tcn, tpad;
    double *xbuf;
};
constexpr int PHENO_CHUNK = 8;
template <int C>
static int launch_pheno(pg_ctx *ctx, AssocParams &pr, const PhenoLaunch &pl)
{
    if (pl.phase == PhenoLaunch::SETUP) {
        setup_tabs_kernel<C><<<NLAM, 64, (size_t)pr.n_vals * 4 + 16, ctx->stream>>>(pr);
    } else if (pl.phase == PhenoLaunch::SCAN) {
        const unsigned nblk = (unsigned)((pr.p + SCAN_WPB - 1) / SCAN_WPB);
        switch (pl.tpad) {
            case 1: scan_pheno_kernel<C, 1><<<nblk, 64 * SCAN_WPB, 0, ctx->stream>>>(pr, pl.Y, pl.ldy, pl.tcn, pl.xbuf); break;
            case 2: scan_pheno_kernel<C, 2><<<nblk, 64 * SCAN_WPB, 0, ctx->stream>>>(pr, pl.Y, pl.ldy, pl.tcn, pl.xbuf); break;
            case 4: scan_pheno_kernel<C, 4><<<nblk, 64 * SCAN_WPB, 0, ctx->stream>>>(pr, pl.Y, pl.ldy, pl.tcn, pl.xbuf); break;
            case 8: scan_pheno_kernel<C, 8><<<nblk, 64 * SCAN_WPB, 0, ctx->stream>>>(pr, pl.Y, pl.ldy, pl.tcn, pl.xbuf); break;
            default: set_error("assoc_pheno: chunk width %d", pl.tpad); return PG_EINVAL;
        }
    } else {
        const size_t lds = (size_t)WPB * assoc_per_wave_bytes(Shape<C>::M, Shape<C>::SWEEP_LDS, sizeof(EvalOut), pr.n_vals);
        PG_REQUIRE(pr.n_vals >= 0 && lds <= 160 * 1024, "assoc_pheno: c = %d, n_vals = %d need %zu bytes of LDS per workgroup", C, pr.n_vals, lds);
        if (lds > 64 * 1024)
            PG_HIP(hipFuncSetAttribute(reinterpret_cast<const void *>(&assoc_kernel<C, false, true>), hipFuncAttributeMaxDynamicSharedMemorySize, (int)lds));
        const long long nblk = (pr.p + WPB - 1) / WPB;
        assoc_kernel<C, false, true><<<dim3((unsigned)nblk), 64 * WPB, lds, ctx->stream>>>(pr);
    }
    PG_HIP(hipGetLastError());
    return PG_OK;
}


int launch_assoc_hi(pg_ctx *ctx, AssocParams &pr);
int launch_assoc_lrt(pg_ctx *ctx, AssocParams &pr);
int launch_assoc_lrt_hi(pg_ctx *ctx, AssocParams &pr);
int launch_assoc_pheno(pg_ctx *ctx, AssocParams &pr, const PhenoLaunch &pl);
int launch_assoc_pheno_hi(pg_ctx *ctx, AssocParams &pr, const PhenoLaunch &pl);
int launch_assoc_gxe(pg_ctx *ctx, AssocParams &pr, const float *xer, long long ldxe);
int launch_assoc_gxe_hi(pg_ctx *ctx, AssocParams &pr, const float *xer, long long ldxe);
#define PG_CASE(CC) case CC: return launch_assoc<CC, PG_CASE_LRT>(ctx, pr);
#define PG_PCASE(CC) case CC: return launch_pheno<CC>(ctx, pr, pl);
#define PG_GCASE(CC) case CC: return launch_gxe<CC>(ctx, pr, xer, ldxe);
#if defined(PG_ASSOC_PART) && PG_ASSOC_PART == 6
int launch_assoc_gxe(pg_ctx *ctx, AssocParams &pr, const float *xer, long long ldxe)
{
    switch (pr.c) {
        PG_GCASE(1) PG_GCASE(2) PG_GCASE(3) PG_GCASE(4) PG_GCASE(5) PG_GCASE(6) PG_GCASE(7) PG_GCASE(8) PG_GCASE(9) PG_GCASE(10)
        PG_GCASE(11) PG_GCASE(12) PG_GCASE(13) PG_GCASE(14) PG_GCASE(15)
        default: return launch_assoc_gxe_hi(ctx, pr, xer, ldxe);
    }
}
__global__ __launch_bounds__(256) void gxe_scale_u_kernel(long long n, const float *U, long long ldU, const float *e, float *Ue)
{
    const long long i = blockIdx.y, k = (long long)blockIdx.x * 256 + threadIdx.x;
    if (i < n && k < n) Ue[i * n + k] = __fmul_rn(e[i], U[i * ldU + k]);
}
extern "C" int pg_gxe_scale_u_dev(pg_ctx *ctx, int64_t n, const float *U, int64_t ldU, const float *e, float *Ue)
{
    PG_REQUIRE(ctx && U && e && Ue, "pg_gxe_scale_u_dev: NULL argument");
    PG_REQUIRE(n >= 1 && n < (1LL << 30) && ldU >= n, "pg_gxe_scale_u_dev: bad shape n=%lld ldU=%lld", (long long)n, (long long)ldU);
    PG_HIP(hipSetDevice(ctx->device));
    gxe_scale_u_kernel<<<dim3((unsigned)((n + 255) / 256), (unsigned)n), 256, 0, ctx->stream>>>(n, U, ldU, e, Ue);
    PG_HIP(hipGetLastError());
    return PG_OK;
}
#elif defined(PG_ASSOC_PART) && PG_ASSOC_PART == 7
int launch_assoc_gxe_hi(pg_ctx *ctx, AssocParams &pr, const float *xer, long long ldxe)
{
    switch (pr.c) {
        PG_GCASE(16) PG_GCASE(17) PG_GCASE(18) PG_GCASE(19) PG_GCASE(20) PG_GCASE(21) PG_GCASE(22) PG_GCASE(23) PG_GCASE(24) PG_GCASE(25)
        PG_GCASE(26) PG_GCASE(27) PG_GCASE(28) PG_GCASE(29)
        default: return PG_ENOTSUP;
    }
}
#elif defined(PG_ASSOC_PART) && PG_ASSOC_PART == 4
int launch_assoc_pheno(pg_ctx *ctx, AssocParams &pr, const PhenoLaunch &pl)
{
    switch (pr.c) {
        PG_PCASE(1) PG_PCASE(2) PG_PCASE(3) PG_PCASE(4) PG_PCASE(5) PG_PCASE(6) PG_PCASE(7) PG_PCASE(8) PG_PCASE(9) PG_PCASE(10)
        PG_PCASE(11) PG_PCASE(12) PG_PCASE(13) PG_PCASE(14) PG_PCASE(15)
        default: return launch_assoc_pheno_hi(ctx, pr, pl);
    }
}
#elif defined(PG_ASSOC_PART) && PG_ASSOC_PART == 5
int launch_assoc_pheno_hi(pg_ctx *ctx, AssocParams &pr, const PhenoLaunch &pl)
{
    switch (pr.c) {
        PG_PCASE(16) PG_PCASE(17) PG_PCASE(18) PG_PCASE(19) PG_PCASE(20) PG_PCASE(21) PG_PCASE(22) PG_PCASE(23) PG_PCASE(24) PG_PCASE(25)
        PG_PCASE(26) PG_PCASE(27) PG_PCASE(28) PG_PCASE(29) PG_PCASE(30)
        default: return PG_ENOTSUP;
    }
}
#elif defined(PG_ASSOC_PART) && PG_ASSOC_PART == 1
#define PG_CASE_LRT false
int launch_assoc_hi(pg_ctx *ctx, AssocParams &pr)
{
    switch (pr.c) {
        PG_CASE(16) PG_CASE(17) PG_CASE(18) PG_CASE(19) PG_CASE(20) PG_CASE(21) PG_CASE(22) PG_CASE(23) PG_CASE(24) PG_CASE(25)
        PG_CASE(26) PG_CASE(27) PG_CASE(28) PG_CASE(29) PG_CASE(30)
        default: return PG_ENOTSUP;
    }
}
#elif defined(PG_ASSOC_PART) && PG_ASSOC_PART == 2
#define PG_CASE_LRT true
int launch_assoc_lrt(pg_ctx *ctx, AssocParams &pr)
{
    switch (pr.c) {
        PG_CASE(0) PG_CASE(1) PG_CASE(2) PG_CASE(3) PG_CASE(4) PG_CASE(5) PG_CASE(6) PG_CASE(7) PG_CASE(8) PG_CASE(9) PG_CASE(10)
        PG_CASE(11) PG_CASE(12) PG_CASE(13) PG_CASE(14) PG_CASE(15)
        default: return launch_assoc_lrt_hi(ctx, pr);
    }
}
#elif defined(PG_ASSOC_PART) && PG_ASSOC_PART == 3
#define PG_CASE_LRT true
int launch_assoc_lrt_hi(pg_ctx *ctx, AssocParams &pr)
{
    switch (pr.c) {
        PG_CASE(16) PG_CASE(17) PG_CASE(18) PG_CASE(19) PG_CASE(20) PG_CASE(21) PG_CASE(22) PG_CASE(23) PG_CASE(24) PG_CASE(25)
        PG_CASE(26) PG_CASE(27) PG_CASE(28) PG_CASE(29) PG_CASE(30)
        default: return PG_ENOTSUP;
    }
}
#else
#define PG_CASE_LRT false
static int launch_assoc_any(pg_ctx *ctx, AssocParams &pr)
{
    if (pr.lrt) return launch_assoc_lrt(ctx, pr);
    switch (pr.c) {
#ifdef PG_ONLY_C
        PG_CASE(PG_ONLY_C)
#else
        PG_CASE(1) PG_CASE(2) PG_CASE(3) PG_CASE(4) PG_CASE(5) PG_CASE(6) PG_CASE(7) PG_CASE(8) PG_CASE(9) PG_CASE(10)
        PG_CASE(11) PG_CASE(12) PG_CASE(13) PG_CASE(14) PG_CASE(15)
#endif
        default: return launch_assoc_hi(ctx, pr);
    }
}
#ifdef PG_ONLY_C
#undef PG_CASE_LRT
#define PG_CASE_LRT true
int launch_assoc_lrt(pg_ctx *ctx, AssocParams &pr)
{
    switch (pr.c) { PG_CASE(PG_ONLY_C) case PG_ONLY_C - 1: return launch_assoc<PG_ONLY_C - 1, true>(ctx, pr); default: return PG_ENOTSUP; }
}
int launch_assoc_hi(pg_ctx *, AssocParams &) { return PG_ENOTSUP; }
int launch_assoc_pheno(pg_ctx *, AssocParams &, const PhenoLaunch &) { return PG_ENOTSUP; }
#endif
#endif
#undef PG_CASE
#undef PG_PCASE
#undef PG_GCASE

#ifndef PG_ASSOC_PART
__device__ double betacf_dev(double a, double b, double x)
{
    const double FPMIN = 1e-300, EPS = 1e-16;
    double qab = a + b, qap = a + 1.0, qam = a - 1.0, c = 1.0, dd = 1.0 - qab * x / qap, h;
    if (fabs(dd) < FPMIN) dd = FPMIN;
    dd = 1.0 / dd; h = dd;
    for (int m = 1; m <= 2000; m++) {
        int m2 = 2 * m;
        double aa = m * (b - m) * x / ((qam + m2) * (a + m2));
        dd = 1.0 + aa * dd; if (fabs(dd) < FPMIN) dd = FPMIN;
        c = 1.0 + aa / c; if (fabs(c) < FPMIN) c = FPMIN;
        dd = 1.0 / dd; h *= dd * c;
        aa = -(a + m) * (qab + m) * x / ((a + m2) * (qap + m2));
        dd = 1.0 + aa * dd; if (fabs(dd) < FPMIN) dd = FPMIN;
        c = 1.0 + aa / c; if (fabs(c) < FPMIN) c = FPMIN;
        dd = 1.0 / dd;
        double del = dd * c;
        h *= del;
        if (fabs(del - 1.0) < EPS) break;
    }
    return h;
}
__global__ void fdist_sf_kernel(long long count, const double *F, double dfd, double *pval)
{
    long long g = (long long)blockIdx.x * blockDim.x + threadIdx.x;
    if (g >= count) return;
    double f = F[g], r;
    if (f != f) r = f;
    else if (f <= 0.0) r = 1.0;
    else if (isinf(f)) r = 0.0;
    else {
        double a = 0.5 * dfd, b = 0.5;
        double x = dfd / (dfd + f), omx = 1.0 - x;
        double lbeta = lgamma(a) + lgamma(b) - lgamma(a + b);
        double lbt = a * log(x) + b * log(omx) - lbeta;
        if (x < (a + 1.0) / (a + b + 2.0)) r = exp(lbt) * betacf_dev(a, b, x) / a;
        else r = 1.0 - exp(lbt) * betacf_dev(b, a, omx) / b;
    }
    pval[g] = r;
}

__global__ void build_fixed_kernel(int n, int npad, int c, int ldw, int rowf, const float *d, const float *Wr, const float *yr, float *fixed)
{
    int i = blockIdx.x * blockDim.x + threadIdx.x;
    if (i >= npad) return;
    float *row = fixed + (size_t)i * rowf;
    for (int k = 0; k < rowf; k++) row[k] = 0.0f;
    if (i >= n) row[0] = INFINITY;
    if (i < n) {
        row[0] = d[i];
        for (int j = 0; j < c; j++) row[1 + j] = Wr[(size_t)i * ldw + j];
        row[c + 1] = yr[i];
    }
}

__global__ __launch_bounds__(256) void transpose_kernel(long long n, long long p, const float *X, long long ldX, float *Xr, long long ldx)
{
    __shared__ float tile[32][33];
    const long long g0 = (long long)blockIdx.x * 32, i0 = (long long)blockIdx.y * 32;
    const int tx = threadIdx.x & 31, ty = threadIdx.x >> 5;
    for (int r = ty; r < 32; r += 8) {
        long long i = i0 + r, g = g0 + tx;
        tile[r][tx] = (i < n && g < p) ? X[(size_t)i * ldX + g] : 0.0f;
    }
    __syncthreads();
    for (int r = ty; r < 32; r += 8) {
        long long g = g0 + r, i = i0 + tx;
        if (g < p && i < ldx) Xr[(size_t)g * ldx + i] = tile[tx][r];
    }
}

constexpr int IM = PG_MAX_COVARIATES + 2;

struct InspectParams {
    AssocParams pr;
    int ctot, m, full;
    float lam, lam_min, lam_max;
    const float *d, *Wx, *y;
    float *P3, *Q3, *R3;
    float *vecs;
    float *scal;
    float *out;
};

__device__ __forceinline__ float inspect_col(const InspectParams &ip, int j, int i)
{
    return (j < ip.ctot) ? ip.Wx[(size_t)i * ip.ctot + j] : ip.y[i];
}

__device__ void inspect_gram0(const InspectParams &ip, float lam, bool full, int lane, double (*G)[IM][IM], double *tr)
{
    const int n = ip.pr.n, m = ip.m;
    for (int j = 0; j < m; j++)
        for (int k = 0; k <= j; k++) {
            double P = 0.0, Q = 0.0, R = 0.0;
            for (int i = lane; i < n; i += 64) {
                const double hd = (double)hinv_f32(lam, ip.d[i]);
                const double cj = (double)inspect_col(ip, j, i), ck = (double)inspect_col(ip, k, i);
                const double aj = hd * cj, ak = hd * ck;
                P = fma(aj, ck, P);
                Q = fma(aj, ak, Q);
                if (full) { const double gj = (hd * hd) * cj; R = fma(gj, ak, R); }
            }
            P = bfly(P); Q = bfly(Q); R = bfly(R);
            if (lane == 0) { G[0][j][k] = P; G[1][j][k] = Q; G[2][j][k] = full ? R : 0.0; }
        }
    double s1 = 0.0, s2 = 0.0;
    for (int i = lane; i < n; i += 64) {
        const double hd = (double)hinv_f32(lam, ip.d[i]);
        s1 += hd;
        s2 = fma(hd, hd, s2);
    }
    s1 = bfly(s1); s2 = bfly(s2);
    if (lane == 0) { tr[0] = s1; tr[1] = full ? s2 : 0.0; }
    wave_lds_sync();
}

__device__ void inspect_sweeps(const InspectParams &ip, bool full, double (*G)[IM][IM], const double *tr, bool exp, EvalOut &o)
{
    const int m = ip.m;
    double (*P)[IM] = G[0], (*Q)[IM] = G[1], (*R)[IM] = G[2];
    double trP = tr[0], trPP = tr[1];
    float ld = 0.0f;
    P[0][0] = dmaxf(P[0][0], PG_MINV);
    auto level_out = [&](int lv) {
        if (!exp) return;
        for (int r = lv; r < m; r++)
            for (int c = lv; c <= r; c++) {
                const size_t idx = ((size_t)r * m + lv) * m + c;
                ip.P3[idx] = (float)P[r][c]; ip.Q3[idx] = (float)Q[r][c];
                if (full) ip.R3[idx] = (float)R[r][c];
            }
        ip.vecs[0 * m + lv] = (float)P[m - 1][m - 1];
        ip.vecs[1 * m + lv] = (float)Q[m - 1][m - 1];
        if (full) ip.vecs[2 * m + lv] = (float)R[m - 1][m - 1];
        ip.vecs[3 * m + lv] = (float)trP;
        ip.vecs[4 * m + lv] = (float)trPP;
    };
    level_out(0);
    for (int i = 1; i < m; i++) {
        const int q = i - 1;
        const double a = P[q][q], b = Q[q][q], e = R[q][q];
        double u[IM], v[IM], w[IM];
        for (int r = i; r < m; r++) { u[r] = P[r][q]; v[r] = Q[r][q]; w[r] = R[r][q]; }
        if (full) {
            const double ba = b / a;
            trPP = trPP + ba * ba - 2 * (e / a);
            const double a2 = a * a, a3 = a2 * a, b2 = b * b;
            const double cR = (e / a2) - (b2 / a3), ia = -1.0 / a, ba2 = b / a2;
            for (int r = i; r < m; r++)
                for (int c = i; c <= r; c++) {
                    const double t1 = fma(cR * u[c], u[r], R[r][c]);
                    double t2 = fma(ia * u[c], w[r], 0.0); t2 = fma(ia * w[c], u[r], t2);
                    const double t3 = fma(ia * v[c], v[r], 0.0);
                    double t4 = fma(ba2 * u[c], v[r], 0.0); t4 = fma(ba2 * v[c], u[r], t4);
                    R[r][c] = ((t1 + t2) + t3) + t4;
                }
            R[i][i] = dmaxf(R[i][i], PG_MINV);
        }
        trP = trP - b / a;
        {
            const double a2 = a * a, al1 = b / a2, ia = -1.0 / a;
            for (int r = i; r < m; r++)
                for (int c = i; c <= r; c++) {
                    const double t1 = fma(al1 * u[c], u[r], Q[r][c]);
                    double t2 = fma(ia * u[c], v[r], 0.0); t2 = fma(ia * v[c], u[r], t2);
                    Q[r][c] = t1 + t2;
                }
            Q[i][i] = dmaxf(Q[i][i], PG_MINV);
        }
        ld = (float)((double)ld + log(a));
        {
            const double ia = -1.0 / a;
            for (int r = i; r < m; r++)
                for (int c = i; c <= r; c++) P[r][c] = fma(ia * u[c], u[r], P[r][c]);
            P[i][i] = dmaxf(P[i][i], PG_MINV);
        }
        if (!full) trPP = 0.0;
        level_out(i);
    }
    o.yPy = (float)P[m - 1][m - 1]; o.yPPy = (float)Q[m - 1][m - 1]; o.yPPPy = (float)R[m - 1][m - 1];
    o.trP = (float)trP; o.trPP = (float)trPP; o.ld = ld;
    o.Pxx_c = (m >= 2) ? (float)P[m - 2][m - 2] : 0.0f; o.Pyx_c = (m >= 2) ? (float)P[m - 1][m - 2] : 0.0f;
}

__global__ __launch_bounds__(64) void precompute_kernel(InspectParams ip)
{
    __shared__ double G[3][IM][IM];
    __shared__ double tr[2];
    __shared__ EvalOut eo;
    extern __shared__ float vals_dyn[];
    const int lane = threadIdx.x, m = ip.m;
    for (int idx = lane; idx < m * m * m; idx += 64) { ip.P3[idx] = NAN; ip.Q3[idx] = NAN; ip.R3[idx] = NAN; }
    for (int idx = lane; idx < 5 * m; idx += 64) ip.vecs[idx] = NAN;
    for (int idx = lane; idx < 3 * IM * IM; idx += 64) (&G[0][0][0])[idx] = 0.0;
    wave_lds_sync();
    inspect_gram0(ip, ip.lam, ip.full != 0, lane, G, tr);
    if (lane == 0) inspect_sweeps(ip, ip.full != 0, G, tr, true, eo);
    wave_lds_sync();
    const float ldH = device_logdet_H(ip.pr, ip.lam, lane, vals_dyn);
    if (lane == 0) {
        ip.scal[0] = eo.ld; ip.scal[1] = ldH;
        ip.scal[2] = d1_f(ip.pr, ip.lam, eo.yPy, eo.yPPy, eo.trP);
        ip.scal[3] = ip.full ? d2_f(ip.pr, ip.lam, eo.yPy, eo.yPPy, eo.yPPPy, eo.trP, eo.trPP) : NAN;
        ip.scal[4] = logl_f(ip.pr, eo.yPy, ldH, eo.ld);
        ip.scal[5] = (float)tr[0];
        ip.scal[6] = ip.full ? (float)tr[1] : NAN;
    }
}

__global__ __launch_bounds__(64) void newton_kernel(InspectParams ip)
{
    __shared__ double G[3][IM][IM];
    __shared__ double tr[2];
    __shared__ EvalOut eo;
    const int lane = threadIdx.x;
    const float root = newton_dev(ip.pr, ip.lam, ip.lam_min, ip.lam_max, [&](float lf, EvalOut &e) {
        for (int idx = lane; idx < 3 * IM * IM; idx += 64) (&G[0][0][0])[idx] = 0.0;
        wave_lds_sync();
        inspect_gram0(ip, lf, true, lane, G, tr);
        if (lane == 0) inspect_sweeps(ip, true, G, tr, false, eo);
        wave_lds_sync();
        e = eo;
        wave_lds_sync();
    });
    if (lane == 0) ip.out[0] = root;
}

__global__ void reml_scalars_kernel(AssocParams pr, const float *a, float *out)
{
    if (threadIdx.x != 0 || blockIdx.x != 0) return;
    out[0] = logl_f(pr, a[1], a[6], a[7]);
    out[1] = d1_f(pr, a[0], a[1], a[2], a[4]);
    out[2] = d2_f(pr, a[0], a[1], a[2], a[3], a[4], a[5]);
}

}

using namespace pg;

extern "C" int pg_fdist_sf_dev(pg_ctx *ctx, int64_t count, const double *F, double dfd, double *pval)
{
    PG_REQUIRE(ctx && F && pval && count >= 0, "pg_fdist_sf_dev: bad arguments");
    if (count == 0) return PG_OK;
    PG_HIP(hipSetDevice(ctx->device));
    fdist_sf_kernel<<<(unsigned)((count + 255) / 256), 256, 0, ctx->stream>>>(count, F, dfd, pval);
    PG_HIP(hipGetLastError());
    return PG_OK;
}

extern "C" int pg_transpose_dev(pg_ctx *ctx, int64_t n, int64_t p, const float *X, int64_t ldX, float *Xr, int64_t ldx)
{
    PG_REQUIRE(ctx && X && Xr && n > 0 && p > 0 && ldx >= n && ldX >= p, "pg_transpose_dev: bad arguments");
    PG_HIP(hipSetDevice(ctx->device));
    dim3 grid((unsigned)((p + 31) / 32), (unsigned)((ldx + 31) / 32));
    transpose_kernel<<<grid, 256, 0, ctx->stream>>>(n, p, X, ldX, Xr, ldx);
    PG_HIP(hipGetLastError());
    return PG_OK;
}

static void fill_params(pg_ctx *ctx, int64_t n, int c, int grid, AssocParams &pr)
{
    pr.n = (int)n; pr.npad = (int)((n + 63) / 64 * 64); pr.c = c; pr.niter = pr.npad / 64;
    pr.nu = (int)(n - c - 1); pr.grid = grid ? 1 : 0; pr.rowf = ((c + 2 + 3) / 4) * 4;
    for (int k = -5; k <= 5; k++) pr.lam11[k + 5] = (float)pow(10.0, (double)(float)k);
    {
        const int ctot = c + 1;
        float r = (float)((0.5 * (double)(n - ctot)) * std::log(0.5 * (double)(n - ctot) / M_PI));
        r = (float)((double)r - (0.5 * (double)(n - ctot)));
        pr.logl_c = r;
    }
    pr.nhalf = (int)(n / 2);
    {
        float r = (float)((double)(n / 2) * std::log((double)n / (2.0 * M_PI)));
        pr.ml_c = r - (float)(n / 2);
    }
    pr.leaf = ctx->plan.d_leaf; pr.node = ctx->plan.d_node; pr.level = ctx->plan.d_level; pr.chunk = ctx->plan.d_chunk;
    pr.n_leaf = ctx->plan.n_leaf; pr.n_level = ctx->plan.n_level; pr.n_chunk = ctx->plan.n_chunk;
    pr.n_vals = ctx->plan.n_leaf + ctx->plan.n_node;
}

static int assoc_run(pg_ctx *ctx, int64_t n, int c, int64_t p, const float *d, const float *Wr, int64_t ldw, const float *yr,
                     const float *Xr, int64_t ldx, int grid, float *beta, float *se, float *tau, float *lambda, double *F,
                     unsigned long long *stats_dev, bool lrt, float *lalt, float *lamalt)
{
    PG_HIP(hipSetDevice(ctx->device));
    int rc = build_npsum_plan(ctx, n);
    if (rc) return rc;

    AssocParams pr{};
    fill_params(ctx, n, c, grid, pr);
    pr.p = p; pr.ldx = ldx; pr.xr = Xr;
    const int M = c + 2, NP = M * (M + 1) / 2;
    rc = ensure(ctx, &ctx->fixed, &ctx->fixed_bytes, (size_t)pr.npad * pr.rowf * 4);
    if (rc) return rc;
    const size_t off_fixg = ((size_t)NLAM * pr.npad * 4 + 255) & ~(size_t)255;
    const size_t off_t1 = off_fixg + (size_t)NLAM * 2 * NP * 8;
    const size_t off_ldh = off_t1 + NLAM * 8;
    rc = ensure(ctx, &ctx->tabs, &ctx->tabs_bytes, off_ldh + NLAM * 4 + 256);
    if (rc) return rc;
    if (!ctx->stats) PG_HIP(hipMalloc(&ctx->stats, 16));
    pr.fixed = (const float *)ctx->fixed;
    pr.htab = (float *)ctx->tabs;
    pr.fixg = (double *)((char *)ctx->tabs + off_fixg);
    pr.t1tab = (double *)((char *)ctx->tabs + off_t1);
    pr.ldHtab = (float *)((char *)ctx->tabs + off_ldh);
    pr.lrt = lrt ? 1 : 0;
    pr.lalt = lalt; pr.lamalt = lamalt;
    pr.beta = beta; pr.se = se; pr.tau = tau; pr.lam = lambda; pr.F = F;
    pr.stats = stats_dev;
    pr.trace = lrt ? nullptr : ctx->eval_trace;

    build_fixed_kernel<<<(pr.npad + 255) / 256, 256, 0, ctx->stream>>>(pr.n, pr.npad, c, (int)ldw, pr.rowf, d, Wr, yr, (float *)ctx->fixed);
    PG_HIP(hipGetLastError());
    return launch_assoc_any(ctx, pr);
}

extern "C" int pg_assoc_dev(pg_ctx *ctx, int64_t n, int c, int64_t p, const float *d, const float *Wr, const float *yr,
                            const float *Xr, int64_t ldx, int grid, float *beta, float *se, float *tau, float *lambda,
                            double *F, double *pval, unsigned long long *stats_dev)
{
    PG_REQUIRE(ctx && d && Wr && yr && Xr && beta && se && tau && lambda && F, "pg_assoc_dev: NULL argument");
    PG_REQUIRE(n >= 2 && n < (1LL << 30) && p >= 0 && ldx >= n, "pg_assoc_dev: bad shape n=%lld p=%lld ldx=%lld", (long long)n, (long long)p, (long long)ldx);
    if (c < 1 || c > PG_MAX_COVARIATES) {
        set_error("pg_assoc_dev: c=%d covariates not supported by this build (1..%d)", c, PG_MAX_COVARIATES);
        return PG_ENOTSUP;
    }
    PG_REQUIRE(n - c - 1 > 0, "pg_assoc_dev: n - c - 1 must be positive");
    if (p == 0) return PG_OK;
    int rc = assoc_run(ctx, n, c, p, d, Wr, c, yr, Xr, ldx, grid, beta, se, tau, lambda, F, stats_dev, false, nullptr, nullptr);
    if (rc) return rc;
    if (pval) return pg_fdist_sf_dev(ctx, p, F, (double)(n - c - 1), pval);
    return PG_OK;
}

extern "C" int pg_assoc_warm(pg_ctx *ctx, int64_t n, int c)
{
    PG_REQUIRE(ctx && n >= 2 && n < (1LL << 30), "pg_assoc_warm: bad arguments");
    if (c < 1 || c > PG_MAX_COVARIATES) {
        set_error("pg_assoc_warm: c=%d covariates not supported by this build (1..%d)", c, PG_MAX_COVARIATES);
        return PG_ENOTSUP;
    }
    PG_HIP(hipSetDevice(ctx->device));
    int rc = build_npsum_plan(ctx, n);
    if (rc) return rc;
    const int npad = (int)((n + 63) / 64 * 64), rowf = ((c + 2 + 3) / 4) * 4, M = c + 2, NP = M * (M + 1) / 2;
    rc = ensure(ctx, &ctx->fixed, &ctx->fixed_bytes, (size_t)npad * rowf * 4);
    if (rc) return rc;
    const size_t off_fixg = ((size_t)NLAM * npad * 4 + 255) & ~(size_t)255;
    rc = ensure(ctx, &ctx->tabs, &ctx->tabs_bytes, off_fixg + (size_t)NLAM * 2 * NP * 8 + NLAM * 8 + NLAM * 4 + 256);
    if (rc) return rc;
    if (!ctx->stats) PG_HIP(hipMalloc(&ctx->stats, 16));
    return PG_OK;
}

extern "C" int pg_assoc_set_eval_trace(pg_ctx *ctx, unsigned *trace_dev)
{
    PG_REQUIRE(ctx, "pg_assoc_set_eval_trace: NULL ctx");
    ctx->eval_trace = trace_dev;
    return PG_OK;
}

struct PhenoLayout {
    int npad, rowf, NP, tpad_max;
    long long ptile;
    size_t off_htab, off_fixg, off_t1, off_ldh, off_xbuf, bytes;
};
static PhenoLayout pheno_layout(int64_t n, int c, int t, int64_t p)
{
    PhenoLayout L{};
    auto up = [](size_t v) { return (v + 255) & ~(size_t)255; };
    L.npad = (int)((n + 63) / 64 * 64); L.rowf = ((c + 2 + 3) / 4) * 4; L.NP = (c + 2) * (c + 3) / 2;
    const int tc = t < PHENO_CHUNK ? t : PHENO_CHUNK;
    L.tpad_max = 1;
    while (L.tpad_max < tc) L.tpad_max <<= 1;
    const size_t per_snp = (size_t)NLAM * 2 * (c + 1 + L.tpad_max) * 8;
    const long long cap = (long long)((256u << 20) / per_snp);
    L.ptile = p < cap ? p : (cap < 1024 ? 1024 : cap);
    if (L.ptile > p) L.ptile = p;
    L.off_htab = up((size_t)PHENO_CHUNK * L.npad * L.rowf * 4);
    L.off_fixg = L.off_htab + up((size_t)NLAM * L.npad * 4);
    L.off_t1 = L.off_fixg + up((size_t)PHENO_CHUNK * NLAM * 2 * L.NP * 8);
    L.off_ldh = L.off_t1 + up(NLAM * 8);
    L.off_xbuf = L.off_ldh + up(NLAM * 4);
    L.bytes = L.off_xbuf + up((size_t)L.ptile * per_snp);
    return L;
}

extern "C" int pg_assoc_pheno_dev(pg_ctx *ctx, int64_t n, int c, int64_t p, int t, const float *d, const float *Wr,
                                  const float *Yr, int64_t ldy, const float *Xr, int64_t ldx, int grid,
                                  float *beta, float *se, float *tau, float *lambda, double *F, double *pval,
                                  unsigned long long *stats_dev)
{
    PG_REQUIRE(ctx && d && Wr && Yr && Xr && beta && se && tau && lambda && F, "pg_assoc_pheno_dev: NULL argument");
    PG_REQUIRE(n >= 2 && n < (1LL << 30) && p >= 0 && ldx >= n, "pg_assoc_pheno_dev: bad shape n=%lld p=%lld ldx=%lld",
               (long long)n, (long long)p, (long long)ldx);
    if (c < 1 || c > PG_MAX_COVARIATES) {
        set_error("pg_assoc_pheno_dev: c=%d covariates not supported by this build (1..%d)", c, PG_MAX_COVARIATES);
        return PG_ENOTSUP;
    }
    PG_REQUIRE(n - c - 1 > 0, "pg_assoc_pheno_dev: n - c - 1 must be positive");
    PG_REQUIRE(t >= 1 && ldy >= n, "pg_assoc_pheno_dev: bad phenotypes t=%d ldy=%lld (n=%lld)", t, (long long)ldy, (long long)n);
    if (p == 0) return PG_OK;
    PG_HIP(hipSetDevice(ctx->device));
    int rc = build_npsum_plan(ctx, n);
    if (rc) return rc;
    const PhenoLayout L = pheno_layout(n, c, t, p);
    rc = ensure(ctx, &ctx->pheno, &ctx->pheno_bytes, L.bytes);
    if (rc) return rc;
    char *base = (char *)ctx->pheno;
    float *fixed = (float *)base;
    double *fixg = (double *)(base + L.off_fixg), *xbuf = (double *)(base + L.off_xbuf);

    AssocParams pr{};
    fill_params(ctx, n, c, grid, pr);
    pr.ldx = ldx;
    pr.htab = (float *)(base + L.off_htab);
    pr.t1tab = (double *)(base + L.off_t1);
    pr.ldHtab = (float *)(base + L.off_ldh);
    pr.stats = stats_dev;
    const size_t fixed_stride = (size_t)L.npad * L.rowf, fixg_stride = (size_t)NLAM * 2 * L.NP;
    for (int k0 = 0; k0 < t; k0 += PHENO_CHUNK) {
        const int tcn = (t - k0) < PHENO_CHUNK ? (t - k0) : PHENO_CHUNK;
        int tpad = 1;
        while (tpad < tcn) tpad <<= 1;
        for (int j = 0; j < tcn; j++) {
            pr.fixed = fixed + j * fixed_stride;
            pr.fixg = fixg + j * fixg_stride;
            build_fixed_kernel<<<(L.npad + 255) / 256, 256, 0, ctx->stream>>>(pr.n, L.npad, c, c, L.rowf, d, Wr, Yr + (size_t)(k0 + j) * ldy,
                                                                             (float *)pr.fixed);
            PG_HIP(hipGetLastError());
            rc = launch_assoc_pheno(ctx, pr, PhenoLaunch{PhenoLaunch::SETUP, nullptr, 0, 0, 0, nullptr});
            if (rc) return rc;
        }
        pr.xe = c + 1 + tpad; pr.xbuf = xbuf;
        for (int64_t s0 = 0; s0 < p; s0 += L.ptile) {
            pr.p = (p - s0) < L.ptile ? (p - s0) : L.ptile;
            pr.xr = Xr + (size_t)s0 * ldx;
            rc = launch_assoc_pheno(ctx, pr, PhenoLaunch{PhenoLaunch::SCAN, Yr + (size_t)k0 * ldy, ldy, tcn, tpad, xbuf});
            if (rc) return rc;
            for (int j = 0; j < tcn; j++) {
                const size_t o = (size_t)(k0 + j) * p + s0;
                pr.fixed = fixed + j * fixed_stride; pr.fixg = fixg + j * fixg_stride; pr.xcol = c + 1 + j;
                pr.beta = beta + o; pr.se = se + o; pr.tau = tau + o; pr.lam = lambda + o; pr.F = F + o;
                rc = launch_assoc_pheno(ctx, pr, PhenoLaunch{PhenoLaunch::SEARCH, nullptr, 0, tcn, tpad, xbuf});
                if (rc) return rc;
            }
        }
    }
    if (pval) return pg_fdist_sf_dev(ctx, (int64_t)t * p, F, (double)(n - c - 1), pval);
    return PG_OK;
}

extern "C" int pg_assoc_pheno_warm(pg_ctx *ctx, int64_t n, int c, int t, int64_t p)
{
    PG_REQUIRE(ctx && n >= 2 && n < (1LL << 30) && t >= 1 && p >= 1, "pg_assoc_pheno_warm: bad arguments");
    if (c < 1 || c > PG_MAX_COVARIATES) {
        set_error("pg_assoc_pheno_warm: c=%d covariates not supported by this build (1..%d)", c, PG_MAX_COVARIATES);
        return PG_ENOTSUP;
    }
    PG_HIP(hipSetDevice(ctx->device));
    int rc = build_npsum_plan(ctx, n);
    if (rc) return rc;
    return ensure(ctx, &ctx->pheno, &ctx->pheno_bytes, pheno_layout(n, c, t, p).bytes);
}

extern "C" int pg_assoc_gxe_dev(pg_ctx *ctx, int64_t n, int c, int64_t p, const float *d, const float *Wr, const float *yr,
                                const float *xr, int64_t ldx, const float *xer, int64_t ldxe, float *beta, float *se, float *tau,
                                float *lambda, double *F, double *pval, unsigned long long *stats_dev)
{
    PG_REQUIRE(ctx && d && Wr && yr && xr && xer && beta && se && tau && lambda && F, "pg_assoc_gxe_dev: NULL argument");
    PG_REQUIRE(n >= 2 && n < (1LL << 30) && p >= 0 && ldx >= n && ldxe >= n, "pg_assoc_gxe_dev: bad shape n=%lld p=%lld ldx=%lld ldxe=%lld",
               (long long)n, (long long)p, (long long)ldx, (long long)ldxe);
    if (c < 1 || c + 1 > PG_MAX_COVARIATES) {
        set_error("pg_assoc_gxe_dev: c=%d shared covariates not supported by this build (1..%d)", c, PG_MAX_COVARIATES - 1);
        return PG_ENOTSUP;
    }
    PG_REQUIRE(n - c - 2 > 0, "pg_assoc_gxe_dev: n - c - 2 must be positive");
    if (p == 0) return PG_OK;
    PG_HIP(hipSetDevice(ctx->device));
    int rc = build_npsum_plan(ctx, n);
    if (rc) return rc;
    AssocParams pr{};
    fill_params(ctx, n, c + 1, 0, pr);
    pr.c = c; pr.rowf = ((c + 2 + 3) / 4) * 4;
    pr.p = p; pr.ldx = ldx; pr.xr = xr;
    const int NP = (c + 2) * (c + 3) / 2;
    rc = ensure(ctx, &ctx->fixed, &ctx->fixed_bytes, (size_t)pr.npad * pr.rowf * 4);
    if (rc) return rc;
    const size_t off_fixg = ((size_t)NLAM * pr.npad * 4 + 255) & ~(size_t)255;
    const size_t off_t1 = off_fixg + (size_t)NLAM * 2 * NP * 8;
    const size_t off_ldh = off_t1 + NLAM * 8;
    rc = ensure(ctx, &ctx->tabs, &ctx->tabs_bytes, off_ldh + NLAM * 4 + 256);
    if (rc) return rc;
    pr.fixed = (const float *)ctx->fixed;
    pr.htab = (float *)ctx->tabs;
    pr.fixg = (double *)((char *)ctx->tabs + off_fixg);
    pr.t1tab = (double *)((char *)ctx->tabs + off_t1);
    pr.ldHtab = (float *)((char *)ctx->tabs + off_ldh);
    pr.beta = beta; pr.se = se; pr.tau = tau; pr.lam = lambda; pr.F = F;
    pr.stats = stats_dev;
    build_fixed_kernel<<<(pr.npad + 255) / 256, 256, 0, ctx->stream>>>(pr.n, pr.npad, c, c, pr.rowf, d, Wr, yr, (float *)ctx->fixed);
    PG_HIP(hipGetLastError());
    rc = launch_assoc_gxe(ctx, pr, xer, ldxe);
    if (rc) return rc;
    if (pval) return pg_fdist_sf_dev(ctx, p, F, (double)(n - c - 2), pval);
    return PG_OK;
}

extern "C" int pg_assoc_gxe_warm(pg_ctx *ctx, int64_t n, int c)
{
    PG_REQUIRE(ctx && n >= 2 && n < (1LL << 30), "pg_assoc_gxe_warm: bad arguments");
    if (c < 1 || c + 1 > PG_MAX_COVARIATES) {
        set_error("pg_assoc_gxe_warm: c=%d shared covariates not supported by this build (1..%d)", c, PG_MAX_COVARIATES - 1);
        return PG_ENOTSUP;
    }
    return pg_assoc_warm(ctx, n, c);
}

namespace pg {
__global__ void gather_col_kernel(int n, int npad, const float *W, int ldw, int col, float *out)
{
    const int i = blockIdx.x * blockDim.x + threadIdx.x;
    if (i < npad) out[i] = (i < n) ? W[(size_t)i * ldw + col] : 0.0f;
}
__global__ void lrt_finish_kernel(long long p, const float *lalt, const float *lnull, double *o_lalt, double *o_lnull, double *o_D, double *o_p)
{
    const long long g = (long long)blockIdx.x * blockDim.x + threadIdx.x;
    if (g >= p) return;
    const float la = lalt[g], ln = lnull[0];
    const float D = __fmul_rn(2.0f, __fsub_rn(la, ln));
    const double Dd = (double)D;
    o_lalt[g] = (double)la; o_lnull[g] = (double)ln; o_D[g] = Dd;
    o_p[g] = (Dd != Dd) ? Dd : (Dd <= 0.0 ? 1.0 : erfc(sqrt(0.5 * Dd)));
}
}

extern "C" int pg_assoc_lrt_dev(pg_ctx *ctx, int64_t n, int c, int64_t p, const float *d, const float *Wr, const float *yr,
                                const float *Xr, int64_t ldx, int grid, float *beta, float *se, float *tau, float *lambda,
                                double *F, double *pval, double *l_alt, double *l_null, double *D_lrt, double *p_lrt)
{
    PG_REQUIRE(ctx && d && Wr && yr && Xr && beta && se && tau && lambda && F && l_alt && l_null && D_lrt && p_lrt, "pg_assoc_lrt_dev: NULL argument");
    PG_REQUIRE(n >= 2 && n < (1LL << 30) && p >= 0 && ldx >= n, "pg_assoc_lrt_dev: bad shape");
    if (c < 1 || c > PG_MAX_COVARIATES) {
        set_error("pg_assoc_lrt_dev: c=%d covariates not supported by this build (1..%d)", c, PG_MAX_COVARIATES);
        return PG_ENOTSUP;
    }
    PG_REQUIRE(n - c - 1 > 0, "pg_assoc_lrt_dev: n - c - 1 must be positive");
    if (p == 0) return PG_OK;
    PG_HIP(hipSetDevice(ctx->device));
    const int64_t npad = (n + 63) / 64 * 64;
    const size_t off_out = (size_t)npad * 4, off_la = off_out + 64, need = off_la + (size_t)p * 8 + 64;
    int rc = ensure(ctx, &ctx->scratch, &ctx->scratch_bytes, need);
    if (rc) return rc;
    char *sc = (char *)ctx->scratch;
    float *xnull = (float *)sc, *nb = (float *)(sc + off_out), *lnull = nb + 8, *lamnull = nb + 9;
    double *nF = (double *)(sc + off_out + 16);
    float *lalt = (float *)(sc + off_la), *lamalt = lalt + p;
    gather_col_kernel<<<(unsigned)((npad + 255) / 256), 256, 0, ctx->stream>>>((int)n, (int)npad, Wr, c, c - 1, xnull);
    PG_HIP(hipGetLastError());
    rc = assoc_run(ctx, n, c - 1, 1, d, Wr, c, yr, xnull, npad, grid, nb, nb + 1, nb + 2, nb + 3, nF, nullptr, true, lnull, lamnull);
    if (rc) return rc;
    rc = assoc_run(ctx, n, c, p, d, Wr, c, yr, Xr, ldx, grid, beta, se, tau, lambda, F, nullptr, true, lalt, lamalt);
    if (rc) return rc;
    lrt_finish_kernel<<<(unsigned)((p + 255) / 256), 256, 0, ctx->stream>>>(p, lalt, lnull, l_alt, l_null, D_lrt, p_lrt);
    PG_HIP(hipGetLastError());
    if (pval) return pg_fdist_sf_dev(ctx, p, F, (double)(n - c - 1), pval);
    return PG_OK;
}

extern "C" int pg_score_null_dev(pg_ctx *ctx, int64_t n, int c, const float *d, const float *Wr, const float *yr, float *lambda0_dev)
{
    PG_REQUIRE(ctx && d && Wr && yr && lambda0_dev, "pg_score_null_dev: NULL argument");
    PG_REQUIRE(n >= 2 && n < (1LL << 30), "pg_score_null_dev: bad shape n=%lld", (long long)n);
    if (c < 1 || c > PG_MAX_COVARIATES) {
        set_error("pg_score_null_dev: c=%d covariates not supported by this build (1..%d)", c, PG_MAX_COVARIATES);
        return PG_ENOTSUP;
    }
    PG_REQUIRE(n - c - 1 > 0, "pg_score_null_dev: n - c - 1 must be positive");
    PG_HIP(hipSetDevice(ctx->device));
    const int64_t npad = (n + 63) / 64 * 64;
    const size_t off_out = (size_t)npad * 4;
    int rc = ensure(ctx, &ctx->scratch, &ctx->scratch_bytes, off_out + 64);
    if (rc) return rc;
    char *sc = (char *)ctx->scratch;
    float *xnull = (float *)sc, *nb = (float *)(sc + off_out), *lnull = nb + 8;
    double *nF = (double *)(sc + off_out + 16);
    gather_col_kernel<<<(unsigned)((npad + 255) / 256), 256, 0, ctx->stream>>>((int)n, (int)npad, Wr, c, c - 1, xnull);
    PG_HIP(hipGetLastError());
    return assoc_run(ctx, n, c - 1, 1, d, Wr, c, yr, xnull, npad, 0, nb, nb + 1, nb + 2, nb + 3, nF, nullptr, true, lnull, lambda0_dev);
}

static int inspect_params(pg_ctx *ctx, int64_t n, int ctot, InspectParams &ip, const float *d)
{
    PG_REQUIRE(n >= 2 && n < (1LL << 30), "inspect: bad n");
    if (ctot < 1 || ctot > PG_MAX_COVARIATES + 1) {
        set_error("inspect: %d columns not supported by this build (1..%d)", ctot, PG_MAX_COVARIATES + 1);
        return PG_ENOTSUP;
    }
    PG_REQUIRE(n - ctot > 0, "inspect: n - c must be positive");
    PG_HIP(hipSetDevice(ctx->device));
    int rc = build_npsum_plan(ctx, n);
    if (rc) return rc;
    AssocParams &pr = ip.pr;
    pr.n = (int)n; pr.npad = (int)((n + 63) / 64 * 64); pr.c = ctot - 1; pr.niter = pr.npad / 64;
    pr.nu = (int)(n - ctot); pr.rowf = 1; pr.fixed = d;
    {
        float r = (float)((0.5 * (double)(n - ctot)) * std::log(0.5 * (double)(n - ctot) / M_PI));
        r = (float)((double)r - (0.5 * (double)(n - ctot)));
        pr.logl_c = r;
    }
    pr.leaf = ctx->plan.d_leaf; pr.node = ctx->plan.d_node; pr.level = ctx->plan.d_level; pr.chunk = ctx->plan.d_chunk;
    pr.n_leaf = ctx->plan.n_leaf; pr.n_level = ctx->plan.n_level; pr.n_chunk = ctx->plan.n_chunk;
    pr.n_vals = ctx->plan.n_leaf + ctx->plan.n_node;
    ip.ctot = ctot; ip.m = ctot + 1; ip.d = d;
    return PG_OK;
}

extern "C" int pg_precompute_mat_dev(pg_ctx *ctx, int64_t n, int ctot, float lam, const float *d, const float *Wx, const float *y,
                                     int full, float *P3, float *Q3, float *R3, float *vecs, float *scal)
{
    PG_REQUIRE(ctx && d && Wx && y && P3 && Q3 && R3 && vecs && scal, "pg_precompute_mat_dev: NULL argument");
    InspectParams ip{};
    int rc = inspect_params(ctx, n, ctot, ip, d);
    if (rc) return rc;
    ip.full = full ? 1 : 0; ip.lam = lam; ip.Wx = Wx; ip.y = y;
    ip.P3 = P3; ip.Q3 = Q3; ip.R3 = R3; ip.vecs = vecs; ip.scal = scal;
    precompute_kernel<<<1, 64, (size_t)ip.pr.n_vals * 4 + 16, ctx->stream>>>(ip);
    PG_HIP(hipGetLastError());
    return PG_OK;
}

extern "C" int pg_newton_dev(pg_ctx *ctx, int64_t n, int ctot, float lam, float lam_min, float lam_max, const float *d,
                             const float *Wx, const float *y, float *root)
{
    PG_REQUIRE(ctx && d && Wx && y && root, "pg_newton_dev: NULL argument");
    InspectParams ip{};
    int rc = inspect_params(ctx, n, ctot, ip, d);
    if (rc) return rc;
    ip.full = 1; ip.lam = lam; ip.lam_min = lam_min; ip.lam_max = lam_max; ip.Wx = Wx; ip.y = y; ip.out = root;
    newton_kernel<<<1, 64, 0, ctx->stream>>>(ip);
    PG_HIP(hipGetLastError());
    return PG_OK;
}

extern "C" int pg_reml_scalars_dev(pg_ctx *ctx, int64_t n, int ctot, const float *args8, float *out3)
{
    PG_REQUIRE(ctx && args8 && out3 && n - ctot > 0, "pg_reml_scalars_dev: bad arguments");
    PG_HIP(hipSetDevice(ctx->device));
    AssocParams pr{};
    pr.n = (int)n; pr.nu = (int)(n - ctot);
    {
        float r = (float)((0.5 * (double)(n - ctot)) * std::log(0.5 * (double)(n - ctot) / M_PI));
        r = (float)((double)r - (0.5 * (double)(n - ctot)));
        pr.logl_c = r;
    }
    reml_scalars_kernel<<<1, 1, 0, ctx->stream>>>(pr, args8, out3);
    PG_HIP(hipGetLastError());
    return PG_OK;
}

__global__ void ml_scalars_kernel(AssocParams pr, const float *a, float *out)
{
    if (threadIdx.x != 0 || blockIdx.x != 0) return;
    out[0] = ml_logl_f(pr, a[1], a[6]);
    out[1] = ml_d1_f(pr, a[0], a[1], a[2], a[4]);
    out[2] = ml_d2_f(pr, a[0], a[1], a[2], a[3], a[4], a[5]);
}
extern "C" int pg_ml_scalars_dev(pg_ctx *ctx, int64_t n, const float *args7, float *out3)
{
    PG_REQUIRE(ctx && args7 && out3 && n >= 2 && n < (1LL << 30), "pg_ml_scalars_dev: bad arguments");
    PG_HIP(hipSetDevice(ctx->device));
    AssocParams pr{};
    pr.n = (int)n;
    pr.nhalf = (int)(n / 2);
    {
        float r = (float)((double)(n / 2) * std::log((double)n / (2.0 * M_PI)));
        pr.ml_c = r - (float)(n / 2);
    }
    ml_scalars_kernel<<<1, 1, 0, ctx->stream>>>(pr, args7, out3);
    PG_HIP(hipGetLastError());
    return PG_OK;
}
#else
}
#endif
```

### pygemma_amd/csrc/common.hpp

```cpp
#pragma once
#include <hip/hip_runtime.h>
#include <cstdarg>
#include <cstdint>
#include <cstdio>
#include <cstring>
#include <vector>

#include "../../include/pygemma_hip.h"

namespace pg {

void set_error(const char *fmt, ...);

#define PG_HIP(call)                                                                             \
    do {                                                                                         \
        hipError_t _e = (call);                                                                  \
        if (_e != hipSuccess) {                                                                  \
            pg::set_error("%s failed: %s (%s:%d)", #call, hipGetErrorString(_e), __FILE__, __LINE__); \
            return PG_EHIP;                                                                      \
        }                                                                                        \
    } while (0)

#define PG_REQUIRE(cond, ...)            \
    do {                                 \
        if (!(cond)) {                   \
            pg::set_error(__VA_ARGS__);  \
            return PG_EINVAL;            \
        }                                \
    } while (0)

struct NpSumPlan {
    int64_t n = -1;
    int n_leaf = 0, n_node = 0, n_level = 0, n_chunk = 0;
    int *d_leaf = nullptr;
    int *d_node = nullptr;
    int *d_level = nullptr;
    int *d_chunk = nullptr;
};

}

struct pg_ctx {
    int device = 0;
    hipStream_t stream = nullptr;
    bool own_stream = true;
    int num_cu = 256;
    void *fixed = nullptr; size_t fixed_bytes = 0;
    void *tabs = nullptr;  size_t tabs_bytes = 0;
    unsigned long long *stats = nullptr;
    unsigned *eval_trace = nullptr;
    pg::NpSumPlan plan;
    void *pheno = nullptr; size_t pheno_bytes = 0;
    void *score = nullptr; size_t score_bytes = 0;
    void *scratch = nullptr; size_t scratch_bytes = 0;
    void *arena = nullptr; size_t arena_bytes = 0;
    void *hpin = nullptr; size_t hpin_bytes = 0;
};

namespace pg {
int ensure(pg_ctx *ctx, void **ptr, size_t *have, size_t need);
int build_npsum_plan(pg_ctx *ctx, int64_t n);
}
```

### pygemma_amd/ops.py

```python
import ctypes as C

import numpy as np

from . import _lib


def _f32(a):
    return np.ascontiguousarray(a, dtype=np.float32)


def assoc(d, Wr, yr, Xr, grid=False, ctx=None, want_p=True, return_stats=False):
    L = _lib.load()
    own = ctx is None
    ctx = ctx or _lib.Context(0)
    try:
        d, Wr, yr, Xr = _f32(d), _f32(Wr), _f32(np.asarray(yr).reshape(-1)), _f32(Xr)
        n, c = Wr.shape
        p = Xr.shape[1]
        assert d.shape == (n,) and yr.shape == (n,) and Xr.shape[0] == n
        beta, se, tau, lam = (np.empty(p, np.float32) for _ in range(4))
        F, pv = np.empty(p, np.float64), np.empty(p, np.float64)
        stats = np.zeros(2, np.uint64)
        vp = lambda a: a.ctypes.data_as(C.c_void_p)
        _lib.check(L.pg_assoc(ctx.handle, n, c, p, vp(d), vp(Wr), vp(yr), vp(Xr), int(bool(grid)), vp(beta), vp(se),
                              vp(tau), vp(lam), vp(F), vp(pv) if want_p else None, vp(stats)), "pg_assoc")
        out = {"beta": beta, "se_beta": se, "tau": tau, "lambda": lam.astype(np.float64), "F_wald": F,
               "p_wald": pv if want_p else None}
        if return_stats:
            out["n_evals"] = stats.astype(np.int64)
        return out
    finally:
        if own:
            ctx.close()


def score(d, Wr, yr, Xr, lam0=None, ctx=None):
    L = _lib.load()
    own = ctx is None
    ctx = ctx or _lib.Context(0)
    try:
        d, Wr, yr, Xr = _f32(d), _f32(Wr), _f32(np.asarray(yr).reshape(-1)), _f32(Xr)
        n, c = Wr.shape
        p = Xr.shape[1]
        assert d.shape == (n,) and yr.shape == (n,) and Xr.shape[0] == n
        dd, dW, dy = ctx.to_device(d), ctx.to_device(Wr), ctx.to_device(yr)
        if lam0 is None:
            dl = ctx.alloc(4)
            _lib.check(L.pg_score_null_dev(ctx.handle, n, c, dd.ptr, dW.ptr, dy.ptr, dl.ptr), "pg_score_null_dev")
            ctx.sync()
            lam0 = dl.download((1,), np.float32)[0]
            dl.free()
        lam0 = np.float32(lam0)
        dX = ctx.to_device(Xr)
        dXr = ctx.alloc(max(p, 1) * n * 4)
        out = [ctx.alloc(max(p, 1) * 4) for _ in range(4)] + [ctx.alloc(max(p, 1) * 8) for _ in range(2)]
        if p:
            _lib.check(L.pg_transpose_dev(ctx.handle, n, p, dX.ptr, p, dXr.ptr, n), "pg_transpose_dev")
        _lib.check(L.pg_score_dev(ctx.handle, n, c, p, dd.ptr, dW.ptr, dy.ptr, float(lam0), dXr.ptr, n, *[b.ptr for b in out]),
                   "pg_score_dev")
        ctx.sync()
        res = {col: b.download((p,), np.float32 if k < 4 else np.float64)
               for k, (col, b) in enumerate(zip(("beta", "se_beta", "tau", "lambda", "F_score", "p_score"), out))}
        res["lambda"] = res["lambda"].astype(np.float64)
        res["lambda_null"] = float(lam0)
        for b in (dd, dW, dy, dX, dXr, *out):
            b.free()
        return res
    finally:
        if own:
            ctx.close()


def gxe(d, Wr, yr, Xr, XEr, ctx=None, want_p=True, return_stats=False):
    L = _lib.load()
    own = ctx is None
    ctx = ctx or _lib.Context(0)
    try:
        d, Wr, yr, Xr, XEr = _f32(d), _f32(Wr), _f32(np.asarray(yr).reshape(-1)), _f32(Xr), _f32(XEr)
        n, c = Wr.shape
        p = Xr.shape[1]
        assert d.shape == (n,) and yr.shape == (n,) and Xr.shape == (n, p) and XEr.shape == (n, p)
        dd, dW, dy = ctx.to_device(d), ctx.to_device(Wr), ctx.to_device(yr)
        dX, dXE = ctx.to_device(Xr), ctx.to_device(XEr)
        dXr, dXEr = ctx.alloc(max(p, 1) * n * 4), ctx.alloc(max(p, 1) * n * 4)
        out = [ctx.alloc(max(p, 1) * 4) for _ in range(4)] + [ctx.alloc(max(p, 1) * 8) for _ in range(2)]
        dst = ctx.alloc(16)
        _lib.check(L.pg_memset(ctx.handle, dst.ptr, 0, 16), "pg_memset")
        if p:
            _lib.check(L.pg_transpose_dev(ctx.handle, n, p, dX.ptr, p, dXr.ptr, n), "pg_transpose_dev")
            _lib.check(L.pg_transpose_dev(ctx.handle, n, p, dXE.ptr, p, dXEr.ptr, n), "pg_transpose_dev")
        _lib.check(L.pg_assoc_gxe_dev(ctx.handle, n, c, p, dd.ptr, dW.ptr, dy.ptr, dXr.ptr, n, dXEr.ptr, n,
                                      *[b.ptr for b in out[:5]], out[5].ptr if want_p else None, dst.ptr), "pg_assoc_gxe_dev")
        ctx.sync()
        res = {col: b.download((p,), np.float32 if k < 4 else np.float64)
               for k, (col, b) in enumerate(zip(("beta", "se_beta", "tau", "lambda", "F_wald", "p_wald"), out))}
        res["lambda"] = res["lambda"].astype(np.float64)
        if not want_p:
            res["p_wald"] = None
        if return_stats:
            res["n_evals"] = dst.download((2,), np.uint64).astype(np.int64)
        for b in (dd, dW, dy, dX, dXE, dXr, dXEr, dst, *out):
            b.free()
        return res
    finally:
        if own:
            ctx.close()


def fdist_sf(F, dfd, ctx=None):
    L = _lib.load()
    own = ctx is None
    ctx = ctx or _lib.Context(0)
    try:
        F = np.ascontiguousarray(F, np.float64).ravel()
        dF = ctx.to_device(F)
        dP = ctx.alloc(F.nbytes)
        _lib.check(L.pg_fdist_sf_dev(ctx.handle, F.size, dF.ptr, float(dfd), dP.ptr), "pg_fdist_sf_dev")
        ctx.sync()
        return dP.download(F.shape, np.float64)
    finally:
        if own:
            ctx.close()


def rotate(U, X, ctx=None, ldx=None):
    L = _lib.load()
    own = ctx is None
    ctx = ctx or _lib.Context(0)
    try:
        U, X = _f32(U), _f32(X)
        n, p = X.shape
        ldx = ldx or (n + 63) // 64 * 64
        dU, dX = ctx.to_device(U), ctx.to_device(X)
        dXr = ctx.alloc(p * ldx * 4)
        _lib.check(L.pg_rotate_dev(ctx.handle, n, p, dU.ptr, n, dX.ptr, p, dXr.ptr, ldx), "pg_rotate_dev")
        ctx.sync()
        out = dXr.download((p, ldx), np.float32)
        for b in (dU, dX, dXr):
            b.free()
        return out
    finally:
        if own:
            ctx.close()


def syevd(K, ctx=None, want64=False):
    L = _lib.load()
    own = ctx is None
    ctx = ctx or _lib.Context(0)
    try:
        K = _f32(K)
        n = K.shape[0]
        assert K.shape == (n, n)
        dK = ctx.to_device(K)
        dev, dU = ctx.alloc(n * 4), ctx.alloc(n * n * 4)
        d64 = ctx.alloc(n * 8) if want64 else None
        U64 = ctx.alloc(n * n * 8) if want64 else None
        _lib.check(L.pg_syevd_dev(ctx.handle, n, dK.ptr, dev.ptr, dU.ptr, d64.ptr if want64 else None,
                                  U64.ptr if want64 else None), "pg_syevd_dev")
        ctx.sync()
        out = [dev.download((n,), np.float32), dU.download((n, n), np.float32)]
        if want64:
            out += [d64.download((n,), np.float64), U64.download((n, n), np.float64)]
        for b in (dK, dev, dU, d64, U64):
            if b is not None:
                b.free()
        return tuple(out)
    finally:
        if own:
            ctx.close()


def rotate_geno(U, X, ctx=None, ldx=None):
    L = _lib.load()
    own = ctx is None
    ctx = ctx or _lib.Context(0)
    try:
        U, X = _f32(U), _f32(X)
        n, p = X.shape
        ldx = ldx or (n + 63) // 64 * 64
        dU, dX = ctx.to_device(U), ctx.to_device(X)
        dprep = ctx.alloc(L.pg_geno_prep_bytes(n))
        dwork = ctx.alloc(L.pg_geno_work_bytes(n, p))
        dXr = ctx.alloc(p * ldx * 4)
        _lib.check(L.pg_geno_prep_dev(ctx.handle, n, dU.ptr, n, dprep.ptr), "pg_geno_prep_dev")
        ok = C.c_int(0)
        _lib.check(L.pg_rotate_geno_dev(ctx.handle, n, p, dprep.ptr, dX.ptr, p, dXr.ptr, ldx, dwork.ptr, C.byref(ok)), "pg_rotate_geno_dev")
        ctx.sync()
        out = dXr.download((p, ldx), np.float32) if ok.value else None
        for b in (dU, dX, dprep, dwork, dXr):
            b.free()
        return out, int(ok.value)
    finally:
        if own:
            ctx.close()


def rotate_auto(U, X, ctx=None):
    L = _lib.load()
    own = ctx is None
    ctx = ctx or _lib.Context(0)
    try:
        U, X = _f32(U), _f32(X)
        n, p = X.shape
        ldx = (n + 63) // 64 * 64
        dU, dX = ctx.to_device(U), ctx.to_device(X)
        dprep, dwork = ctx.alloc(L.pg_geno_prep_bytes(n)), ctx.alloc(L.pg_geno_work_bytes(n, p))
        dXr, dpath = ctx.alloc(p * ldx * 4), ctx.alloc(4)
        _lib.check(L.pg_geno_prep_dev(ctx.handle, n, dU.ptr, n, dprep.ptr), "pg_geno_prep_dev")
        _lib.check(L.pg_rotate_auto_dev(ctx.handle, n, p, dU.ptr, n, dprep.ptr, dX.ptr, p, dXr.ptr, ldx, dwork.ptr, dpath.ptr),
                   "pg_rotate_auto_dev")
        ctx.sync()
        out = dXr.download((p, ldx), np.float32), int(dpath.download((1,), np.int32)[0])
        for b in (dU, dX, dprep, dwork, dXr, dpath):
            b.free()
        return out
    finally:
        if own:
            ctx.close()
```

Before: 1.763 million.

## Reuse cached Gram P/Q passes across Brent, Newton and final evaluations

Adds a small per-wave LDS ring that stores the P/Q Gram pass results (and t1) for recent lambda evaluations from the Brent root search. The first Newton step and the final evaluation can then reuse cached results, the level-0 endpoint results, or the last full evaluation instead of recomputing the Gram passes. This targets redundant per-SNP Gram work but uses more LDS per wave, which may lower occupancy, and adds LDS syncs and best-value tracking through LDS. It also adds an optional pass-trace counter exposed to Python.

```diff
diff --git a/include/pygemma_hip.h b/include/pygemma_hip.h
--- a/include/pygemma_hip.h
+++ b/include/pygemma_hip.h
@@ -71,6 +71,7 @@
                  double *F, double *pval, unsigned long long *stats_dev);
 
 int pg_assoc_set_eval_trace(pg_ctx *ctx, unsigned *trace_dev);
+int pg_assoc_set_pass_trace(pg_ctx *ctx, unsigned *trace_dev);
 int pg_assoc_warm(pg_ctx *ctx, int64_t n, int c);
 
 int pg_assoc_pheno_dev(pg_ctx *ctx, int64_t n, int c, int64_t p, int t, const float *d, const float *Wr,
diff --git a/pygemma_amd/_lib.py b/pygemma_amd/_lib.py
--- a/pygemma_amd/_lib.py
+++ b/pygemma_amd/_lib.py
@@ -20,7 +20,7 @@
     "pg_comm_group_end", "pgx_dgemm_dev", "pgx_sytrd_dev", "pgx_stedc_dev", "pgx_sb2_stage1_dev", "pgx_sb2_stage2_dev", "pgx_sb2_set_debug", "pg_kinship_geno_dev", "pg_assoc_lrt_dev", "pg_rotate_auto_dev", "pg_assoc_set_eval_trace", "pg_assoc_warm", "pg_rotate_auto_i8_dev",
     "pg_zkzt_dev", "pgx_dgemm_ex_dev", "pgx_ring_stamps", "pg_assoc_pheno_dev", "pg_assoc_pheno_warm", "pg_score_null_dev", "pg_score_dev",
     "pg_kinship_acc_bytes", "pg_kinship_bed_acc_dev", "pg_kinship_x_acc_dev", "pg_kinship_finish_dev",
-    "pg_assoc_gxe_dev", "pg_assoc_gxe_warm", "pg_gxe_scale_u_dev",
+    "pg_assoc_gxe_dev", "pg_assoc_gxe_warm", "pg_gxe_scale_u_dev", "pg_assoc_set_pass_trace",
 ]
 
 
@@ -82,6 +82,8 @@
     L.pg_rotate_geno_dev.restype = i32
     L.pg_assoc_set_eval_trace.argtypes = [vp, vp]
     L.pg_assoc_set_eval_trace.restype = i32
+    L.pg_assoc_set_pass_trace.argtypes = [vp, vp]
+    L.pg_assoc_set_pass_trace.restype = i32
     L.pg_assoc_warm.argtypes = [vp, i64, i32]
     L.pg_assoc_warm.restype = i32
     L.pg_assoc_pheno_dev.argtypes = [vp, i64, i32, i64, i32, vp, vp, vp, i64, vp, i64, i32, vp, vp, vp, vp, vp, vp, vp]
diff --git a/pygemma_amd/csrc/assoc.hip b/pygemma_amd/csrc/assoc.hip
--- a/pygemma_amd/csrc/assoc.hip
+++ b/pygemma_amd/csrc/assoc.hip
@@ -1,6 +1,7 @@
 #include "common.hpp"
 
 #include <cmath>
+#include <cstdlib>
 
 namespace pg {
 
@@ -35,9 +36,21 @@
 #define PG_WAVES 2
 #endif
 
-__host__ __device__ constexpr size_t assoc_per_wave_bytes(int M, bool sweep_lds, size_t evalout_bytes, int n_vals)
-{
-    return (((sweep_lds ? (size_t)3 * M * 8 : 0) + (size_t)NLAM * 2 * M * 8 + NLAM * evalout_bytes + 2 * NLAM * 4 + (size_t)n_vals * 4) + 15) & ~(size_t)15;
+constexpr int REUSE_MAX_DEPTH = 4;
+constexpr size_t REUSE_HDR_BYTES = 144;
+constexpr size_t REUSE_WAVE_BUDGET = 160 * 1024 / 8;
+__host__ __device__ constexpr size_t reuse_entry_bytes(int slots) { return (size_t)2 * slots * 64 * 8; }
+__host__ __device__ constexpr size_t reuse_bytes(int slots, int depth) { return REUSE_HDR_BYTES + (size_t)depth * reuse_entry_bytes(slots); }
+
+__host__ __device__ constexpr size_t assoc_per_wave_bytes(int M, bool sweep_lds, size_t evalout_bytes, int n_vals, size_t reuse_b)
+{
+    return ((reuse_b + (sweep_lds ? (size_t)3 * M * 8 : 0) + (size_t)NLAM * 2 * M * 8 + NLAM * evalout_bytes + 2 * NLAM * 4 + (size_t)n_vals * 4) + 15) & ~(size_t)15;
+}
+inline int reuse_fit_depth(int req, int slots, size_t base_bytes)
+{
+    int d = req < 0 ? 0 : (req > REUSE_MAX_DEPTH ? REUSE_MAX_DEPTH : req);
+    while (d > 0 && base_bytes + (size_t)d * reuse_entry_bytes(slots) > REUSE_WAVE_BUDGET) d--;
+    return d;
 }
 
 struct AssocParams {
@@ -57,6 +70,8 @@
     double *F;
     unsigned long long *stats;
     unsigned *trace;
+    int reuse, reuse_req, reuse_depth;
+    unsigned *ptrace;
     int lrt, nhalf;
     float ml_c;
     float *lalt, *lamalt;
@@ -522,9 +537,74 @@
     if constexpr (SL + 1 < Shape<C>::SLOTS) slot_passes<C, PW, HASX, SL + 1, EL>(pr, xrow, lam, lane, htab_out, X, tsum);
 }
 
-template <int C, bool FULL, class EL = WaldElem<C>>
+__device__ __forceinline__ double *reuse_t1(unsigned *rw) { return reinterpret_cast<double *>(rw + 8); }
+__device__ __forceinline__ EvalOut *reuse_last(unsigned *rw) { return reinterpret_cast<EvalOut *>(rw + 16); }
+__device__ __forceinline__ float *reuse_best(unsigned *rw) { return reinterpret_cast<float *>(rw + 26); }
+__device__ __forceinline__ void reuse_set_best(unsigned *rw, float lam, const EvalOut &e, float l, int lane)
+{
+    if (lane == 0) { float *b = reuse_best(rw); b[0] = e.Pyx_c; b[1] = e.Pxx_c; b[2] = e.yPy; b[3] = lam; b[4] = l; }
+    wave_lds_sync();
+}
+__device__ __forceinline__ double *reuse_pq(unsigned *rw) { return reinterpret_cast<double *>(rw + REUSE_HDR_BYTES / 4); }
+enum { REUSE_MISS = 0, REUSE_RING = 1, REUSE_END = 2, REUSE_SKIP = 3 };
+__device__ __forceinline__ void reuse_count(unsigned *rw, int how, int lane)
+{
+    if (lane == 0) rw[1] += 1u << (how == REUSE_RING ? 0 : how == REUSE_END ? 8 : how == REUSE_MISS ? 16 : 24);
+}
+__device__ __forceinline__ void reuse_bump(unsigned *rw, int word, int lane) { if (lane == 0) rw[word] += 1u; }
+__device__ __forceinline__ void reuse_init(unsigned *rw, int lane)
+{
+    if (lane < 8) rw[lane] = (lane < 2) ? 0u : 0xffffffffu;
+    if (lane >= 32 && lane < 34) rw[lane] = 0u;
+    wave_lds_sync();
+}
+template <int C>
+__device__ __forceinline__ void reuse_put(const AssocParams &pr, unsigned *rw, float lam, double t1, const double (&P)[Shape<C>::SLOTS],
+                                          const double (&Q)[Shape<C>::SLOTS], int lane)
+{
+    constexpr int SLOTS = Shape<C>::SLOTS;
+    if (pr.reuse_depth == 0) return;
+    const unsigned pos = (unsigned)__builtin_amdgcn_readfirstlane((int)rw[0]);
+    double *e = reuse_pq(rw) + (size_t)pos * 2 * SLOTS * 64;
+#pragma unroll
+    for (int sl = 0; sl < SLOTS; sl++) { e[sl * 64 + lane] = P[sl]; e[(SLOTS + sl) * 64 + lane] = Q[sl]; }
+    if (lane == 0) {
+        rw[4 + pos] = __float_as_uint(lam);
+        reuse_t1(rw)[pos] = t1;
+        rw[0] = (pos + 1 == (unsigned)pr.reuse_depth) ? 0u : pos + 1;
+    }
+    wave_lds_sync();
+}
+template <int C, class EndF>
+__device__ __forceinline__ int reuse_get(const AssocParams &pr, unsigned *rw, float lam, int k, double (&P)[Shape<C>::SLOTS],
+                                         double (&Q)[Shape<C>::SLOTS], double &t1, int lane, EndF &&endpoint)
+{
+    constexpr int SLOTS = Shape<C>::SLOTS;
+    if (!pr.reuse) return REUSE_MISS;
+    const unsigned lb = __float_as_uint(lam);
+    int hit = -1;
+#pragma unroll
+    for (int j = 0; j < REUSE_MAX_DEPTH; j++) if (j < pr.reuse_depth && rw[4 + j] == lb) hit = j;
+    hit = __builtin_amdgcn_readfirstlane(hit);
+    if (hit >= 0) {
+        const double *e = reuse_pq(rw) + (size_t)hit * 2 * SLOTS * 64;
+#pragma unroll
+        for (int sl = 0; sl < SLOTS; sl++) { P[sl] = e[sl * 64 + lane]; Q[sl] = e[(SLOTS + sl) * 64 + lane]; }
+        t1 = reuse_t1(rw)[hit];
+        return REUSE_RING;
+    }
+    const int t = (lb == __float_as_uint(pr.lam11[k])) ? k : (lb == __float_as_uint(pr.lam11[k + 1])) ? k + 1 : -1;
+    if (t >= 0) {
+        endpoint(t, P, Q);
+        t1 = pr.t1tab[t];
+        return REUSE_END;
+    }
+    return REUSE_MISS;
+}
+
+template <int C, bool FULL, class EL = WaldElem<C>, bool KEEP = false>
 __device__ __forceinline__ void eval_specific(const AssocParams &pr, typename EL::Row xrow, float lam, int lane, const Own<C> &own, EvalOut &o,
-                                              double *piv)
+                                              double *piv, unsigned *rw = nullptr)
 {
     constexpr int SLOTS = Shape<C>::SLOTS;
     double P[SLOTS], Q[SLOTS], R[SLOTS], t1 = 0.0, t2 = 0.0;
@@ -545,7 +625,60 @@
         gram_pass<C, 2, true, EL>(pr, xrow, lam, lane, nullptr, P, Q, R, t1, t2);
         if (FULL) gram_pass<C, 4, true, EL>(pr, xrow, lam, lane, nullptr, P, Q, R, t1, t2);
     }
+    if constexpr (!FULL && KEEP) reuse_put<C>(pr, rw, lam, t1, P, Q, lane);
     lane_sweeps<C, FULL>(P, Q, R, own, t1, t2, lane, o, piv);
+}
+
+template <int C, class EL = WaldElem<C>, class EndF>
+__device__ __forceinline__ void eval_specific_full_reusing(const AssocParams &pr, typename EL::Row xrow, float lam, int lane, const Own<C> &own,
+                                                           EvalOut &o, double *piv, unsigned *rw, bool try_reuse, int k, EndF &&endpoint)
+{
+    constexpr int SLOTS = Shape<C>::SLOTS;
+    constexpr bool FUSED = !Shape<C>::CHUNKED && Shape<C>::FUSE_PQR;
+    double P[SLOTS], Q[SLOTS], R[SLOTS], t1 = 0.0, t2 = 0.0;
+#pragma unroll
+    for (int sl = 0; sl < SLOTS; sl++) R[sl] = 0.0;
+    int how = REUSE_MISS;
+    if (try_reuse) {
+        how = reuse_get<C>(pr, rw, lam, k, P, Q, t1, lane, endpoint);
+        reuse_count(rw, how, lane);
+    }
+    if (how == REUSE_MISS) {
+        if constexpr (Shape<C>::CHUNKED) {
+            double tq = 0.0;
+            slot_passes<C, 1, true, 0, EL>(pr, xrow, lam, lane, nullptr, P, t1);
+            slot_passes<C, 2, true, 0, EL>(pr, xrow, lam, lane, nullptr, Q, tq);
+        } else if constexpr (FUSED) {
+            gram_pass<C, 7, true, EL>(pr, xrow, lam, lane, nullptr, P, Q, R, t1, t2);
+        } else if constexpr (Shape<C>::FUSE_PQ) {
+            gram_pass<C, 3, true, EL>(pr, xrow, lam, lane, nullptr, P, Q, R, t1, t2);
+        } else {
+            gram_pass<C, 1, true, EL>(pr, xrow, lam, lane, nullptr, P, Q, R, t1, t2);
+            gram_pass<C, 2, true, EL>(pr, xrow, lam, lane, nullptr, P, Q, R, t1, t2);
+        }
+    }
+    if (!FUSED || how != REUSE_MISS) {
+        if constexpr (Shape<C>::CHUNKED) slot_passes<C, 3, true, 0, EL>(pr, xrow, lam, lane, nullptr, R, t2);
+        else gram_pass<C, 4, true, EL>(pr, xrow, lam, lane, nullptr, P, Q, R, t1, t2);
+    }
+    lane_sweeps<C, true>(P, Q, R, own, t1, t2, lane, o, piv);
+    if (pr.reuse) {
+        if (lane == 0) { *reuse_last(rw) = o; rw[2] = __float_as_uint(lam); }
+        wave_lds_sync();
+    }
+}
+template <int C, class EL = WaldElem<C>>
+__device__ __forceinline__ void reuse_final(const AssocParams &pr, typename EL::Row xrow, float lroot, int lane, const Own<C> &own, EvalOut &o,
+                                            double *piv, unsigned *rw)
+{
+    if (pr.reuse && __builtin_amdgcn_readfirstlane((int)rw[2]) == (int)__float_as_uint(lroot)) {
+        o = *reuse_last(rw);
+        o.yPPPy = 0.0f; o.trPP = 0.0f; o.shh = 0.0f;
+        reuse_count(rw, REUSE_SKIP, lane);
+        wave_lds_sync();
+        return;
+    }
+    eval_specific<C, false, EL>(pr, xrow, lroot, lane, own, o, piv);
 }
 
 template <int C>
@@ -783,7 +916,7 @@
     int iteration = 0;
     for (;;) {
         EvalOut e;
-        eval(lroot, e);
+        eval(lroot, e, iteration == 0);
         const float d1 = d1_f(pr, lroot, e.yPy, e.yPPy, e.trP);
         const float d2 = d2_f(pr, lroot, e.yPy, e.yPPy, e.yPPPy, e.trP, e.trPP);
         const float ratio = __fdiv_rn(d1, d2);
@@ -802,17 +935,37 @@
     return lroot;
 }
 
+template <int C>
+__device__ __forceinline__ void scan_level0(const AssocParams &pr, const Own<C> &own, const double *xent, int t,
+                                            double (&P)[Shape<C>::SLOTS], double (&Q)[Shape<C>::SLOTS])
+{
+    constexpr int M = Shape<C>::M, NP = Shape<C>::NP, SLOTS = Shape<C>::SLOTS;
+    const double *fp = pr.fixg + ((size_t)t * 2 + 0) * NP, *fq = pr.fixg + ((size_t)t * 2 + 1) * NP;
+    const double *xe = xent + t * 2 * M;
+#pragma unroll
+    for (int sl = 0; sl < SLOTS; sl++) {
+        const int r = own.r[sl], c = own.c[sl];
+        const bool isx = (r == C) || (r == C + 1 && c == C);
+        const int k = (r == C) ? c : C + 1;
+        P[sl] = isx ? xe[k] : fp[own.e[sl]];
+        Q[sl] = isx ? xe[M + k] : fq[own.e[sl]];
+    }
+}
+
 template <int C, bool LRT, bool PHENO = false>
 __global__ __launch_bounds__(64 * WPB, PG_WAVES) void assoc_kernel(AssocParams pr)
 {
     constexpr int M = Shape<C>::M, NP = Shape<C>::NP, SLOTS = Shape<C>::SLOTS;
     extern __shared__ unsigned char smem[];
-    const int wave = threadIdx.x >> 6, lane = threadIdx.x & 63;
+    const int wave = __builtin_amdgcn_readfirstlane((int)(threadIdx.x >> 6)), lane = threadIdx.x & 63;
     static_assert(!(PHENO && LRT), "the multi-phenotype search has no LRT");
     const long long g = (long long)blockIdx.x * WPB + wave;
     if (g >= pr.p) return;
     constexpr size_t piv_bytes = Shape<C>::SWEEP_LDS ? (size_t)3 * M * 8 : 0;
-    unsigned char *base = smem + (size_t)wave * assoc_per_wave_bytes(M, Shape<C>::SWEEP_LDS, sizeof(EvalOut), pr.n_vals);
+    const size_t reuse_b = reuse_bytes(SLOTS, pr.reuse_depth);
+    unsigned char *base = smem + (size_t)wave * assoc_per_wave_bytes(M, Shape<C>::SWEEP_LDS, sizeof(EvalOut), pr.n_vals, reuse_b);
+    unsigned *rw = reinterpret_cast<unsigned *>(base);
+    base += reuse_b;
     double *piv = reinterpret_cast<double *>(base);
     base += piv_bytes;
     double *xent = reinterpret_cast<double *>(base);
@@ -824,6 +977,7 @@
 
     Own<C> own;
     own.init(lane);
+    reuse_init(rw, lane);
     if constexpr (PHENO) {
         const double *src = pr.xbuf + (size_t)g * NLAM * 2 * pr.xe;
         for (int j = lane; j < NLAM * 2 * M; j += 64) {
@@ -836,17 +990,9 @@
     wave_lds_sync();
     for (int t = 0; t < NLAM; t++) {
         double P[SLOTS], Q[SLOTS], R[SLOTS];
-        const double *fp = pr.fixg + ((size_t)t * 2 + 0) * NP, *fq = pr.fixg + ((size_t)t * 2 + 1) * NP;
-        const double *xe = xent + t * 2 * M;
-#pragma unroll
-        for (int sl = 0; sl < SLOTS; sl++) {
-            const int r = own.r[sl], c = own.c[sl];
-            const bool isx = (r == C) || (r == C + 1 && c == C);
-            const int k = (r == C) ? c : C + 1;
-            P[sl] = isx ? xe[k] : fp[own.e[sl]];
-            Q[sl] = isx ? xe[M + k] : fq[own.e[sl]];
-            R[sl] = 0.0;
-        }
+        scan_level0<C>(pr, own, xent, t, P, Q);
+#pragma unroll
+        for (int sl = 0; sl < SLOTS; sl++) R[sl] = 0.0;
         EvalOut e;
         lane_sweeps<C, false>(P, Q, R, own, pr.t1tab[t], 0.0, lane, e, piv);
         if (lane == 0) {
@@ -856,14 +1002,12 @@
         }
     }
     wave_lds_sync();
-    float best_l = lls[0], best_lambda;
-    EvalOut best_e;
-    if (best_l < lls[NLAM - 1]) { best_l = lls[NLAM - 1]; best_lambda = pr.lam11[NLAM - 1]; best_e = evs[NLAM - 1]; }
-    else { best_lambda = pr.lam11[0]; best_e = evs[0]; }
-    unsigned n_fast = 0, n_full = 0;
+    if (lls[0] < lls[NLAM - 1]) reuse_set_best(rw, pr.lam11[NLAM - 1], evs[NLAM - 1], lls[NLAM - 1], lane);
+    else reuse_set_best(rw, pr.lam11[0], evs[0], lls[0], lane);
+    auto endpoint = [&](int t, double (&P)[SLOTS], double (&Q)[SLOTS]) { scan_level0<C>(pr, own, xent, t, P, Q); };
     if (pr.grid) {
         for (int t = 0; t < NLAM - 1; t++)
-            if (lls[t] > best_l) { best_l = lls[t]; best_lambda = pr.lam11[t]; best_e = evs[t]; }
+            if (lls[t] > reuse_best(rw)[4]) reuse_set_best(rw, pr.lam11[t], evs[t], lls[t], lane);
     } else {
         for (int k = 0; k < NLAM - 1; k++) {
             const float f0 = d1s[k], f1 = d1s[k + 1];
@@ -873,21 +1017,21 @@
                 [&](double x) -> double {
                     EvalOut e;
                     const float lf = (float)x;
-                    eval_specific<C, false>(pr, xrow, lf, lane, own, e, piv);
-                    n_fast++;
+                    eval_specific<C, false, WaldElem<C>, true>(pr, xrow, lf, lane, own, e, piv, rw);
+                    reuse_bump(rw, 32, lane);
                     return (double)d1_f(pr, lf, e.yPy, e.yPPy, e.trP);
                 },
                 (double)l0, (double)l1, (double)f0, (double)f1);
-            const float lroot = newton_dev(pr, (float)root, l0, l1, [&](float lf, EvalOut &e) {
-                eval_specific<C, true>(pr, xrow, lf, lane, own, e, piv);
-                n_full++;
+            const float lroot = newton_dev(pr, (float)root, l0, l1, [&](float lf, EvalOut &e, bool first) {
+                eval_specific_full_reusing<C>(pr, xrow, lf, lane, own, e, piv, rw, first, k, endpoint);
+                reuse_bump(rw, 33, lane);
             });
             EvalOut e;
-            eval_specific<C, false>(pr, xrow, lroot, lane, own, e, piv);
-            n_fast++;
+            reuse_final<C>(pr, xrow, lroot, lane, own, e, piv, rw);
+            reuse_bump(rw, 32, lane);
             const float ldH = device_logdet_H(pr, lroot, lane, vals);
             const float ll = logl_f(pr, e.yPy, ldH, e.ld);
-            if (ll > best_l) { best_l = ll; best_lambda = lroot; best_e = e; }
+            if (ll > reuse_best(rw)[4]) reuse_set_best(rw, lroot, e, ll, lane);
         }
     }
     if constexpr (LRT) {
@@ -906,8 +1050,8 @@
                 [&](double x) -> double {
                     EvalOut e;
                     const float lf = (float)x;
-                    eval_specific<C, false>(pr, xrow, lf, lane, own, e, piv);
-                    n_fast++;
+                    eval_specific<C, false, WaldElem<C>, true>(pr, xrow, lf, lane, own, e, piv, rw);
+                    reuse_bump(rw, 32, lane);
                     return (double)ml_d1_f(pr, lf, e.yPy, e.yPPy, e.sh);
                 },
                 (double)pr.lam11[k], (double)pr.lam11[k + 1], (double)f0, (double)f1, 5000);
@@ -915,8 +1059,8 @@
             for (int itr = 0; itr < 10; itr++) {
                 EvalOut e;
                 const float lf = (float)p0;
-                eval_specific<C, true>(pr, xrow, lf, lane, own, e, piv);
-                n_full++;
+                eval_specific_full_reusing<C>(pr, xrow, lf, lane, own, e, piv, rw, itr == 0, k, endpoint);
+                reuse_bump(rw, 33, lane);
                 const float fval = ml_d1_f(pr, lf, e.yPy, e.yPPy, e.sh);
                 if (fval == 0.0f) { pn = p0; break; }
                 const float fder = ml_d2_f(pr, lf, e.yPy, e.yPPy, e.yPPPy, e.sh, e.shh);
@@ -929,7 +1073,7 @@
                 EvalOut e;
                 const float lf = (float)pn;
                 eval_specific<C, false>(pr, xrow, lf, lane, own, e, piv);
-                n_fast++;
+                reuse_bump(rw, 32, lane);
                 const float l = ml_logl_f(pr, e.yPy, device_logdet_H(pr, lf, lane, vals));
                 if (l != l || l > ml_l) { ml_l = l; ml_lam = lf; }
             }
@@ -937,14 +1081,18 @@
         if (lane == 0) { pr.lalt[g] = ml_l; pr.lamalt[g] = ml_lam; }
     }
     if (lane == 0) {
-        const float b = __fdiv_rn(best_e.Pyx_c, best_e.Pxx_c);
-        const float pxx = (PG_MINV > best_e.Pxx_c) ? PG_MINV : best_e.Pxx_c;
-        const float sb = (float)(__dsqrt_rn((double)best_e.yPy) / ((double)sqrtf(pxx) * __dsqrt_rn((double)(pr.nu))));
-        const float ta = __fdiv_rn((float)pr.nu, best_e.yPy);
+        const float *best = reuse_best(rw);
+        const float best_Pyx = best[0], best_Pxx = best[1], best_yPy = best[2], best_lambda = best[3];
+        const float b = __fdiv_rn(best_Pyx, best_Pxx);
+        const float pxx = (PG_MINV > best_Pxx) ? PG_MINV : best_Pxx;
+        const float sb = (float)(__dsqrt_rn((double)best_yPy) / ((double)sqrtf(pxx) * __dsqrt_rn((double)(pr.nu))));
+        const float ta = __fdiv_rn((float)pr.nu, best_yPy);
         const double t = (double)__fdiv_rn(b, sb);
         pr.beta[g] = b; pr.se[g] = sb; pr.tau[g] = ta; pr.lam[g] = best_lambda; pr.F[g] = t * t;
+        const unsigned n_fast = rw[32], n_full = rw[33];
         if (pr.stats) { atomicAdd(&pr.stats[0], (unsigned long long)n_fast); atomicAdd(&pr.stats[1], (unsigned long long)n_full); }
         if (pr.trace) pr.trace[g] = n_fast | (n_full << 16);
+        if (pr.ptrace) pr.ptrace[g] = rw[1];
     }
 }
 
@@ -989,9 +1137,9 @@
     static constexpr int PWS = NE > PG_PHENO_SPLIT_XE ? 1 : 2;
     static constexpr int G0 = (Shape<C>::SCAN_NV - NE) / (PWS * NE), G = G0 < 1 ? 1 : (G0 > NLAM ? NLAM : G0);
 };
-__host__ __device__ constexpr size_t gxe_per_wave_bytes(int M, bool sweep_lds, int NE, size_t evalout_bytes, int n_vals)
-{
-    return (((sweep_lds ? (size_t)3 * M * 8 : 0) + (size_t)NLAM * 2 * NE * 8 + NLAM * evalout_bytes + 2 * NLAM * 4 + (size_t)n_vals * 4) + 15) & ~(size_t)15;
+__host__ __device__ constexpr size_t gxe_per_wave_bytes(int M, bool sweep_lds, int NE, size_t evalout_bytes, int n_vals, size_t reuse_b)
+{
+    return ((reuse_b + (sweep_lds ? (size_t)3 * M * 8 : 0) + (size_t)NLAM * 2 * NE * 8 + NLAM * evalout_bytes + 2 * NLAM * 4 + (size_t)n_vals * 4) + 15) & ~(size_t)15;
 }
 
 template <int CS, int GG, int PWS, int PW0>
@@ -1074,16 +1222,37 @@
 }
 
 template <int CS>
+__device__ __forceinline__ void gxe_scan_level0(const AssocParams &pr, const Own<CS + 1> &own, const double *xent, int t,
+                                                double (&P)[Shape<CS + 1>::SLOTS], double (&Q)[Shape<CS + 1>::SLOTS])
+{
+    constexpr int SLOTS = Shape<CS + 1>::SLOTS, NE = GxeShape<CS>::NE, NPS = Shape<CS>::NP;
+    const double *fp = pr.fixg + ((size_t)t * 2 + 0) * NPS, *fq = pr.fixg + ((size_t)t * 2 + 1) * NPS;
+    const double *xe = xent + t * 2 * NE;
+#pragma unroll
+    for (int sl = 0; sl < SLOTS; sl++) {
+        const int r = own.r[sl], c = own.c[sl];
+        const int k = (r == CS) ? c : (r == CS + 1) ? CS + 1 + c : (r == CS + 2 && c == CS) ? 2 * CS + 3 : (r == CS + 2 && c == CS + 1) ? 2 * CS + 4 : -1;
+        const int f = (r < CS) ? tri(r, c) : tri(CS + 1, c < CS ? c : CS + 1);
+        const int kk = k >= 0 ? k : 0;
+        P[sl] = k >= 0 ? xe[kk] : fp[f];
+        Q[sl] = k >= 0 ? xe[NE + kk] : fq[f];
+    }
+}
+
+template <int CS>
 __global__ __launch_bounds__(64 * WPB, PG_WAVES) void assoc_gxe_kernel(AssocParams pr, const float *xer, long long ldxe)
 {
     constexpr int C = CS + 1, M = Shape<C>::M, SLOTS = Shape<C>::SLOTS, NE = GxeShape<CS>::NE, NPS = Shape<CS>::NP;
     using EL = GxeElem<C>;
     extern __shared__ unsigned char smem[];
-    const int wave = threadIdx.x >> 6, lane = threadIdx.x & 63;
+    const int wave = __builtin_amdgcn_readfirstlane((int)(threadIdx.x >> 6)), lane = threadIdx.x & 63;
     const long long g = (long long)blockIdx.x * WPB + wave;
     if (g >= pr.p) return;
     constexpr size_t piv_bytes = Shape<C>::SWEEP_LDS ? (size_t)3 * M * 8 : 0;
-    unsigned char *base = smem + (size_t)wave * gxe_per_wave_bytes(M, Shape<C>::SWEEP_LDS, NE, sizeof(EvalOut), pr.n_vals);
+    const size_t reuse_b = reuse_bytes(SLOTS, pr.reuse_depth);
+    unsigned char *base = smem + (size_t)wave * gxe_per_wave_bytes(M, Shape<C>::SWEEP_LDS, NE, sizeof(EvalOut), pr.n_vals, reuse_b);
+    unsigned *rw = reinterpret_cast<unsigned *>(base);
+    base += reuse_b;
     double *piv = reinterpret_cast<double *>(base);
     base += piv_bytes;
     double *xent = reinterpret_cast<double *>(base);
@@ -1095,22 +1264,14 @@
 
     Own<C> own;
     own.init(lane);
+    reuse_init(rw, lane);
     gxe_scan_all<CS, 0>(pr, xr, lane, xent);
     wave_lds_sync();
     for (int t = 0; t < NLAM; t++) {
         double P[SLOTS], Q[SLOTS], R[SLOTS];
-        const double *fp = pr.fixg + ((size_t)t * 2 + 0) * NPS, *fq = pr.fixg + ((size_t)t * 2 + 1) * NPS;
-        const double *xe = xent + t * 2 * NE;
-#pragma unroll
-        for (int sl = 0; sl < SLOTS; sl++) {
-            const int r = own.r[sl], c = own.c[sl];
-            const int k = (r == CS) ? c : (r == CS + 1) ? CS + 1 + c : (r == CS + 2 && c == CS) ? 2 * CS + 3 : (r == CS + 2 && c == CS + 1) ? 2 * CS + 4 : -1;
-            const int f = (r < CS) ? tri(r, c) : tri(CS + 1, c < CS ? c : CS + 1);
-            const int kk = k >= 0 ? k : 0;
-            P[sl] = k >= 0 ? xe[kk] : fp[f];
-            Q[sl] = k >= 0 ? xe[NE + kk] : fq[f];
-            R[sl] = 0.0;
-        }
+        gxe_scan_level0<CS>(pr, own, xent, t, P, Q);
+#pragma unroll
+        for (int sl = 0; sl < SLOTS; sl++) R[sl] = 0.0;
         EvalOut e;
         lane_sweeps<C, false>(P, Q, R, own, pr.t1tab[t], 0.0, lane, e, piv);
         if (lane == 0) {
@@ -1120,11 +1281,9 @@
         }
     }
     wave_lds_sync();
-    float best_l = lls[0], best_lambda;
-    EvalOut best_e;
-    if (best_l < lls[NLAM - 1]) { best_l = lls[NLAM - 1]; best_lambda = pr.lam11[NLAM - 1]; best_e = evs[NLAM - 1]; }
-    else { best_lambda = pr.lam11[0]; best_e = evs[0]; }
-    unsigned n_fast = 0, n_full = 0;
+    if (lls[0] < lls[NLAM - 1]) reuse_set_best(rw, pr.lam11[NLAM - 1], evs[NLAM - 1], lls[NLAM - 1], lane);
+    else reuse_set_best(rw, pr.lam11[0], evs[0], lls[0], lane);
+    auto endpoint = [&](int t, double (&P)[SLOTS], double (&Q)[SLOTS]) { gxe_scan_level0<CS>(pr, own, xent, t, P, Q); };
     for (int k = 0; k < NLAM - 1; k++) {
         const float f0 = d1s[k], f1 = d1s[k + 1];
         if (__builtin_signbit(f0) == __builtin_signbit(f1)) continue;
@@ -1133,30 +1292,34 @@
             [&](double x) -> double {
                 EvalOut e;
                 const float lf = (float)x;
-                eval_specific<C, false, EL>(pr, xr, lf, lane, own, e, piv);
-                n_fast++;
+                eval_specific<C, false, EL, true>(pr, xr, lf, lane, own, e, piv, rw);
+                reuse_bump(rw, 32, lane);
                 return (double)d1_f(pr, lf, e.yPy, e.yPPy, e.trP);
             },
             (double)l0, (double)l1, (double)f0, (double)f1);
-        const float lroot = newton_dev(pr, (float)root, l0, l1, [&](float lf, EvalOut &e) {
-            eval_specific<C, true, EL>(pr, xr, lf, lane, own, e, piv);
-            n_full++;
+        const float lroot = newton_dev(pr, (float)root, l0, l1, [&](float lf, EvalOut &e, bool first) {
+            eval_specific_full_reusing<C, EL>(pr, xr, lf, lane, own, e, piv, rw, first, k, endpoint);
+            reuse_bump(rw, 33, lane);
         });
         EvalOut e;
-        eval_specific<C, false, EL>(pr, xr, lroot, lane, own, e, piv);
-        n_fast++;
+        reuse_final<C, EL>(pr, xr, lroot, lane, own, e, piv, rw);
+        reuse_bump(rw, 32, lane);
         const float ldH = device_logdet_H(pr, lroot, lane, vals);
         const float ll = logl_f(pr, e.yPy, ldH, e.ld);
-        if (ll > best_l) { best_l = ll; best_lambda = lroot; best_e = e; }
+        if (ll > reuse_best(rw)[4]) reuse_set_best(rw, lroot, e, ll, lane);
     }
     if (lane == 0) {
-        const float b = __fdiv_rn(best_e.Pyx_c, best_e.Pxx_c);
-        const float pxx = (PG_MINV > best_e.Pxx_c) ? PG_MINV : best_e.Pxx_c;
-        const float sb = (float)(__dsqrt_rn((double)best_e.yPy) / ((double)sqrtf(pxx) * __dsqrt_rn((double)(pr.nu))));
-        const float ta = __fdiv_rn((float)pr.nu, best_e.yPy);
+        const float *best = reuse_best(rw);
+        const float best_Pyx = best[0], best_Pxx = best[1], best_yPy = best[2], best_lambda = best[3];
+        const float b = __fdiv_rn(best_Pyx, best_Pxx);
+        const float pxx = (PG_MINV > best_Pxx) ? PG_MINV : best_Pxx;
+        const float sb = (float)(__dsqrt_rn((double)best_yPy) / ((double)sqrtf(pxx) * __dsqrt_rn((double)(pr.nu))));
+        const float ta = __fdiv_rn((float)pr.nu, best_yPy);
         const double t = (double)__fdiv_rn(b, sb);
         pr.beta[g] = b; pr.se[g] = sb; pr.tau[g] = ta; pr.lam[g] = best_lambda; pr.F[g] = t * t;
+        const unsigned n_fast = rw[32], n_full = rw[33];
         if (pr.stats) { atomicAdd(&pr.stats[0], (unsigned long long)n_fast); atomicAdd(&pr.stats[1], (unsigned long long)n_full); }
+        if (pr.ptrace) pr.ptrace[g] = rw[1];
     }
 }
 
@@ -1164,7 +1327,10 @@
 static int launch_gxe(pg_ctx *ctx, AssocParams &pr, const float *xer, long long ldxe)
 {
     constexpr int C = CS + 1;
-    const size_t lds = (size_t)WPB * gxe_per_wave_bytes(Shape<C>::M, Shape<C>::SWEEP_LDS, GxeShape<CS>::NE, sizeof(EvalOut), pr.n_vals);
+    pr.reuse_depth = reuse_fit_depth(pr.reuse_req, Shape<C>::SLOTS,
+                                     gxe_per_wave_bytes(Shape<C>::M, Shape<C>::SWEEP_LDS, GxeShape<CS>::NE, sizeof(EvalOut), pr.n_vals, reuse_bytes(Shape<C>::SLOTS, 0)));
+    const size_t lds = (size_t)WPB * gxe_per_wave_bytes(Shape<C>::M, Shape<C>::SWEEP_LDS, GxeShape<CS>::NE, sizeof(EvalOut), pr.n_vals,
+                                                        reuse_bytes(Shape<C>::SLOTS, pr.reuse_depth));
     PG_REQUIRE(pr.n_vals >= 0 && lds <= 160 * 1024, "assoc_gxe: c = %d, n_vals = %d need %zu bytes of LDS per workgroup", CS, pr.n_vals, lds);
     setup_tabs_kernel<CS><<<NLAM, 64, (size_t)pr.n_vals * 4 + 16, ctx->stream>>>(pr);
     PG_HIP(hipGetLastError());
@@ -1180,7 +1346,10 @@
 template <int C, bool LRT = false>
 static int launch_assoc(pg_ctx *ctx, AssocParams &pr)
 {
-    const size_t lds = (size_t)WPB * assoc_per_wave_bytes(Shape<C>::M, Shape<C>::SWEEP_LDS, sizeof(EvalOut), pr.n_vals);
+    pr.reuse_depth = reuse_fit_depth(pr.reuse_req, Shape<C>::SLOTS,
+                                     assoc_per_wave_bytes(Shape<C>::M, Shape<C>::SWEEP_LDS, sizeof(EvalOut), pr.n_vals, reuse_bytes(Shape<C>::SLOTS, 0)));
+    const size_t lds = (size_t)WPB * assoc_per_wave_bytes(Shape<C>::M, Shape<C>::SWEEP_LDS, sizeof(EvalOut), pr.n_vals,
+                                                          reuse_bytes(Shape<C>::SLOTS, pr.reuse_depth));
     static_assert(Shape<C>::M == C + 2, "Shape<C>::M");
     PG_REQUIRE(pr.n_vals >= 0 && lds <= 160 * 1024, "assoc: c = %d, n_vals = %d need %zu bytes of LDS per workgroup", C, pr.n_vals, lds);
     setup_tabs_kernel<C><<<NLAM, 64, (size_t)pr.n_vals * 4 + 16, ctx->stream>>>(pr);
@@ -1215,7 +1384,10 @@
             default: set_error("assoc_pheno: chunk width %d", pl.tpad); return PG_EINVAL;
         }
     } else {
-        const size_t lds = (size_t)WPB * assoc_per_wave_bytes(Shape<C>::M, Shape<C>::SWEEP_LDS, sizeof(EvalOut), pr.n_vals);
+        pr.reuse_depth = reuse_fit_depth(pr.reuse_req, Shape<C>::SLOTS,
+                                         assoc_per_wave_bytes(Shape<C>::M, Shape<C>::SWEEP_LDS, sizeof(EvalOut), pr.n_vals, reuse_bytes(Shape<C>::SLOTS, 0)));
+        const size_t lds = (size_t)WPB * assoc_per_wave_bytes(Shape<C>::M, Shape<C>::SWEEP_LDS, sizeof(EvalOut), pr.n_vals,
+                                                              reuse_bytes(Shape<C>::SLOTS, pr.reuse_depth));
         PG_REQUIRE(pr.n_vals >= 0 && lds <= 160 * 1024, "assoc_pheno: c = %d, n_vals = %d need %zu bytes of LDS per workgroup", C, pr.n_vals, lds);
         if (lds > 64 * 1024)
             PG_HIP(hipFuncSetAttribute(reinterpret_cast<const void *>(&assoc_kernel<C, false, true>), hipFuncAttributeMaxDynamicSharedMemorySize, (int)lds));
@@ -1564,7 +1736,7 @@
     __shared__ double tr[2];
     __shared__ EvalOut eo;
     const int lane = threadIdx.x;
-    const float root = newton_dev(ip.pr, ip.lam, ip.lam_min, ip.lam_max, [&](float lf, EvalOut &e) {
+    const float root = newton_dev(ip.pr, ip.lam, ip.lam_min, ip.lam_max, [&](float lf, EvalOut &e, bool) {
         for (int idx = lane; idx < 3 * IM * IM; idx += 64) (&G[0][0][0])[idx] = 0.0;
         wave_lds_sync();
         inspect_gram0(ip, lf, true, lane, G, tr);
@@ -1627,6 +1799,15 @@
     pr.leaf = ctx->plan.d_leaf; pr.node = ctx->plan.d_node; pr.level = ctx->plan.d_level; pr.chunk = ctx->plan.d_chunk;
     pr.n_leaf = ctx->plan.n_leaf; pr.n_level = ctx->plan.n_level; pr.n_chunk = ctx->plan.n_chunk;
     pr.n_vals = ctx->plan.n_leaf + ctx->plan.n_node;
+    static const int reuse_on = [] { const char *e = getenv("PG_ASSOC_REUSE"); return (e && *e) ? (atoi(e) != 0) : 1; }();
+    static const int reuse_depth = [] {
+        const char *e = getenv("PG_ASSOC_REUSE_DEPTH");
+        const int d = (e && *e) ? atoi(e) : REUSE_MAX_DEPTH;
+        return d < 1 ? 1 : (d > REUSE_MAX_DEPTH ? REUSE_MAX_DEPTH : d);
+    }();
+    pr.reuse = reuse_on;
+    pr.reuse_req = reuse_on ? reuse_depth : 0;
+    pr.reuse_depth = 0;
 }
 
 static int assoc_run(pg_ctx *ctx, int64_t n, int c, int64_t p, const float *d, const float *Wr, int64_t ldw, const float *yr,
@@ -1659,6 +1840,7 @@
     pr.beta = beta; pr.se = se; pr.tau = tau; pr.lam = lambda; pr.F = F;
     pr.stats = stats_dev;
     pr.trace = lrt ? nullptr : ctx->eval_trace;
+    pr.ptrace = lrt ? nullptr : ctx->pass_trace;
 
     build_fixed_kernel<<<(pr.npad + 255) / 256, 256, 0, ctx->stream>>>(pr.n, pr.npad, c, (int)ldw, pr.rowf, d, Wr, yr, (float *)ctx->fixed);
     PG_HIP(hipGetLastError());
@@ -1707,6 +1889,13 @@
 {
     PG_REQUIRE(ctx, "pg_assoc_set_eval_trace: NULL ctx");
     ctx->eval_trace = trace_dev;
+    return PG_OK;
+}
+
+extern "C" int pg_assoc_set_pass_trace(pg_ctx *ctx, unsigned *trace_dev)
+{
+    PG_REQUIRE(ctx, "pg_assoc_set_pass_trace: NULL ctx");
+    ctx->pass_trace = trace_dev;
     return PG_OK;
 }
 
@@ -1849,6 +2038,7 @@
     pr.ldHtab = (float *)((char *)ctx->tabs + off_ldh);
     pr.beta = beta; pr.se = se; pr.tau = tau; pr.lam = lambda; pr.F = F;
     pr.stats = stats_dev;
+    pr.ptrace = ctx->pass_trace;
     build_fixed_kernel<<<(pr.npad + 255) / 256, 256, 0, ctx->stream>>>(pr.n, pr.npad, c, c, pr.rowf, d, Wr, yr, (float *)ctx->fixed);
     PG_HIP(hipGetLastError());
     rc = launch_assoc_gxe(ctx, pr, xer, ldxe);
diff --git a/pygemma_amd/csrc/common.hpp b/pygemma_amd/csrc/common.hpp
--- a/pygemma_amd/csrc/common.hpp
+++ b/pygemma_amd/csrc/common.hpp
@@ -49,6 +49,7 @@
     void *tabs = nullptr;  size_t tabs_bytes = 0;
     unsigned long long *stats = nullptr;
     unsigned *eval_trace = nullptr;
+    unsigned *pass_trace = nullptr;
     pg::NpSumPlan plan;
     void *pheno = nullptr; size_t pheno_bytes = 0;
     void *score = nullptr; size_t score_bytes = 0;
diff --git a/pygemma_amd/ops.py b/pygemma_amd/ops.py
--- a/pygemma_amd/ops.py
+++ b/pygemma_amd/ops.py
@@ -9,7 +9,7 @@
     return np.ascontiguousarray(a, dtype=np.float32)
 
 
-def assoc(d, Wr, yr, Xr, grid=False, ctx=None, want_p=True, return_stats=False):
+def assoc(d, Wr, yr, Xr, grid=False, ctx=None, want_p=True, return_stats=False, return_pass_trace=False):
     L = _lib.load()
     own = ctx is None
     ctx = ctx or _lib.Context(0)
@@ -22,12 +22,27 @@
         F, pv = np.empty(p, np.float64), np.empty(p, np.float64)
         stats = np.zeros(2, np.uint64)
         vp = lambda a: a.ctypes.data_as(C.c_void_p)
-        _lib.check(L.pg_assoc(ctx.handle, n, c, p, vp(d), vp(Wr), vp(yr), vp(Xr), int(bool(grid)), vp(beta), vp(se),
-                              vp(tau), vp(lam), vp(F), vp(pv) if want_p else None, vp(stats)), "pg_assoc")
+        dpt = None
+        if return_pass_trace:
+            dpt = ctx.alloc(max(p, 1) * 4)
+            _lib.check(L.pg_memset(ctx.handle, dpt.ptr, 0, max(p, 1) * 4), "pg_memset")
+            _lib.check(L.pg_assoc_set_pass_trace(ctx.handle, dpt.ptr), "pg_assoc_set_pass_trace")
+        try:
+            _lib.check(L.pg_assoc(ctx.handle, n, c, p, vp(d), vp(Wr), vp(yr), vp(Xr), int(bool(grid)), vp(beta), vp(se),
+                                  vp(tau), vp(lam), vp(F), vp(pv) if want_p else None, vp(stats)), "pg_assoc")
+            if dpt is not None:
+                ctx.sync()
+                ptrace = dpt.download((p,), np.uint32)
+        finally:
+            if dpt is not None:
+                L.pg_assoc_set_pass_trace(ctx.handle, None)
+                dpt.free()
         out = {"beta": beta, "se_beta": se, "tau": tau, "lambda": lam.astype(np.float64), "F_wald": F,
                "p_wald": pv if want_p else None}
         if return_stats:
             out["n_evals"] = stats.astype(np.int64)
+        if return_pass_trace:
+            out["pass_trace"] = np.stack([(ptrace >> s) & 0xff for s in (0, 8, 16, 24)], axis=1).astype(np.uint8)
         return out
     finally:
         if own:
```

Measured after the change: 1.798 million, median of 6. 1.02x the previous value.
